# zhirui-gao/PoseProbe

Measured on AMD Instinct MI355X. Metric: rays_per_sec_train_step, higher is better.
Workload: dtype f32 (3xf16-split products); 1 GPU; DTU-scan1-like 3-view 400x400, object-branch train step (ray select, render, losses, backward, TV+Adam), 160^3 grid, 186 samples/ray, N_rand=1024/GPU; per-step ray permutation + jitter pre-generated on the host and resident in HBM (the reference draws randperm inside the step); grid=160, n_rand_per_gpu=1024, samples_in_bbox_last_step=57637, parallelism=single GPU

## Files before the change

include/poseprobe_hip.h:

```cpp
#ifndef POSEPROBE_HIP_H
#define POSEPROBE_HIP_H

#include <stdint.h>

#ifdef __cplusplus
extern "C" {
#endif

typedef enum {
  PP_OK = 0,
  PP_ERR_INVALID_ARG = -1,
  PP_ERR_LAUNCH = -2,
  PP_ERR_UNSUPPORTED = -3
} pp_status;

const char* pp_last_error(void);
#define PP_ABI_VERSION 4
int pp_abi_version(void);

typedef struct {
  float xyz_min[3];
  float xyz_max[3];
  int32_t size[3];
  float voxel_size;
// ... 49 lines not shown
                 const float* alphainv_last, const int32_t* ray_start, const int32_t* i_end, int32_t n_rays,
                 float bg, const float* rgb_pre, const float* g_rgb_marched, const float* g_cum_weights,
                 const float* g_alphainv_last, const float* g_depth_acc, const float* g_weights ,
                 float* grad_alpha, float* grad_rgb, void* stream);

int pp_geometry_fwd(const pp_scene* sc, const float* sdf_grid, const float* sdf_ab ,
                    const float* pts, const float* warp_out, const float* viewdirs, const int32_t* ray_id,
                    const int32_t* count, int32_t capacity, float inv_s, float* alpha, float* gradient,
                    float* sdf_final, float* sdf_deform, float* grad_deform, void* stream);
int pp_geometry_bwd(const pp_scene* sc, const float* sdf_grid, const float* sdf_ab, const float* pts,
                    const float* warp_out, const float* viewdirs, const int32_t* ray_id, const int32_t* count,
                    int32_t capacity, float inv_s, const float* g_alpha, const float* g_gradient,
                    const float* g_sdf_final, const float* g_sdf_deform, const float* g_grad_deform,
                    const float* g_correction, int32_t accumulate, float* warp_out_grad, float* pts_grad,
                    float* viewdir_grad_s, float* sdf_ab_grad, void* stream);

int pp_geometry_bwd_priors(const pp_scene* sc, const float* sdf_grid, const float* sdf_ab, const float* pts,
                           const float* warp_out, const float* viewdirs, const int32_t* ray_id, const int32_t* count,
                           int32_t capacity, float inv_s, const float* g_alpha, const float* g_gradient, float w_eikonal,
                           float w_deform, float loss_scale, int32_t accumulate, float* warp_out_grad, float* pts_grad,
                           float* viewdir_grad_s, float* sdf_ab_grad, float* loss_out, const float* batch_norm,
                           void* stream);

int pp_k0_pack_samples(const float* pts, const float* feat_grad, const int32_t* count, int32_t capacity, int32_t k0_dim,
                       float* packed, void* stream);
int pp_k0_scatter_packed(const pp_scene* sc, const float* packed, int32_t n_shards, int32_t capacity, float* k0_grad_cl,
                         uint8_t* touched , void* stream);
int pp_k0_scatter_samples(const pp_scene* sc, const float* pts, const int32_t* count, int32_t capacity,
                          const float* feat_grad, float* k0_grad_cl, uint8_t* touched , void* stream);

int pp_k0_scatter_sorted_workspace(int64_t n_samples, int64_t* bytes);
int pp_k0_scatter_samples_sorted(const pp_scene* sc, const float* pts, const int32_t* count, int32_t capacity,
                                 const float* feat_grad, float* k0_grad_cl, uint8_t* touched , void* work,
                                 int64_t work_bytes, void* stream);
int pp_k0_scatter_packed_sorted(const pp_scene* sc, const float* packed, int32_t n_shards, int32_t capacity, float* k0_grad_cl,
                                uint8_t* touched , void* work, int64_t work_bytes, void* stream);

int pp_color_feat_fwd(const pp_scene* sc, const float* k0_cl, const float* pts, const float* viewdirs,
                      const int32_t* ray_id, const float* gradient, const float* pe_w, const int32_t* count,
                      int32_t capacity, float* feat, void* stream);
int pp_color_feat_bwd(const pp_scene* sc, const float* k0_cl, const float* pts, const float* viewdirs,
                      const int32_t* ray_id, const float* gradient, const float* pe_w, const int32_t* count,
                      int32_t capacity, const float* feat_grad, float* k0_grad_cl, float* pts_grad,
                      float* gradient_grad, float* viewdir_grad_s, void* stream);

int pp_context_create(void** ctx);
int pp_context_destroy(void* ctx);
int pp_context_set_option(void* ctx, const char* name, int32_t value);
int pp_context_get_option(const void* ctx, const char* name, int32_t* value);

#define PP_RGBNET_PARAMS (128 * 64 + 128 + 2 * (128 * 128 + 128) + 3 * 128 + 3)
int pp_rgbnet_fwd(const float* params, const float* feat, const int32_t* count, int32_t capacity, float* acts,
                  float* rgb, void* ctx, void* stream);
int pp_rgbnet_bwd(const float* params, const float* feat, const float* acts, const float* rgb,
                  const float* rgb_grad, const int32_t* count, int32_t capacity, float* scratch ,
                  float* params_grad , float* feat_grad, void* ctx , void* stream);

#define PP_WARP_PARAMS (128 * 3 + 128 + 3 * (128 * 128 + 128) + 4 * 128 + 4)
int pp_warp_fwd(const float* params, const float* pts, const int32_t* count, int32_t capacity, float out_range,
                float* acts, float* out, void* ctx, void* stream);
int pp_warp_bwd(const float* params, const float* pts, const float* acts, const float* out_grad,
                const int32_t* count, int32_t capacity, float out_range, float* scratch ,
                float* params_grad , float* pts_grad , void* ctx ,
                void* stream);

int pp_rgbnet_workspace(int32_t capacity, int64_t* acts_floats, int64_t* scratch_floats);
int pp_warp_workspace(int32_t capacity, int64_t* acts_floats, int64_t* scratch_floats);
int pp_mlp_workspace(int32_t in_ld, int32_t n_gemm, int32_t capacity, int64_t* acts_floats, int64_t* scratch_floats);

int pp_warp_bwd_data(const float* params, const float* pts, const float* acts, const float* out_grad,
                     const int32_t* count, int32_t capacity, float out_range, float* scratch, float* params_grad,
                     float* pts_grad, int32_t* stage2_host, void* ctx, void* stream);
int pp_warp_bwd_weights(const float* acts, const float* scratch, const int32_t* count, int32_t capacity,
                        float* params_grad, int32_t stage2, void* ctx, void* stream);
int pp_rgbnet_bwd_data(const float* params, const float* acts, const float* rgb, const float* rgb_grad,
                       const int32_t* count, int32_t capacity, float* scratch, float* params_grad, float* feat_grad,
                       int32_t* stage2_host, void* ctx, void* stream);
int pp_rgbnet_bwd_weights(const float* feat, const float* acts, const float* scratch, const int32_t* count,
                          int32_t capacity, float* params_grad, int32_t stage2, void* ctx, void* stream);

int pp_mlp_pack_workspace(int64_t* pack_floats);
int pp_mlp_pack(const float* warp_params, const float* rgbnet_params, float* pack, void* ctx, void* stream);
int pp_mlp_pack_invalidate(void* ctx);

int pp_warp_lean_begin(const float* acts, const float* scratch, const float* params, void* ctx);
int pp_warp_lean_end(void* ctx);

int pp_ordered_workspace(int32_t work_groups, int32_t capacity, int32_t n_rays, int64_t* bytes);
int pp_ordered_attach(void* ctx, void* work, int64_t work_bytes, int32_t work_groups, int32_t capacity, int32_t n_rays);
int pp_geometry_color_feat_fwd(const pp_scene* sc, const float* sdf_grid, const float* sdf_ab, const float* pts,
                               const float* warp_out, const float* viewdirs, const int32_t* ray_id, const int32_t* count,
                               int32_t capacity, float inv_s, float* alpha, float* gradient, float* sdf_final,
                               float* sdf_deform, float* grad_deform, const float* k0_cl, const float* pe_w, float* feat,
                               void* stream);
int pp_geometry_bwd_priors_ordered(const pp_scene* sc, const float* sdf_grid, const float* sdf_ab, const float* pts,
                                   const float* warp_out, const float* viewdirs, const int32_t* ray_id, const int32_t* count,
                                   int32_t capacity, float inv_s, const float* g_alpha, const float* g_gradient, float w_eikonal,
                                   float w_deform, float loss_scale, int32_t accumulate, float* warp_out_grad, float* pts_grad,
                                   float* viewdir_grad_s, float* sdf_ab_grad, float* loss_out, const float* batch_norm,
                                   void* ctx, void* stream);
int pp_raygen_select_bwd_ordered(const pp_scene* sc, const int32_t* ray_idx, int32_t n_rays, const float* c2w,
                                 const float* intr, int32_t n_views, int32_t H, int32_t W, int32_t inverse_y,
                                 const float* rays_o, const float* rays_d, const float* t_min,
                                 const int32_t* ray_start, const float* pts_grad, const float* step,
                                 const float* viewdir_grad_s, const float* rays_o_grad, const float* rays_d_grad,
                                 const float* viewdirs_grad, const float* depth_grad, float* rays_o_grad_out,
                                 float* rays_d_grad_out, float* viewdirs_grad_out, float* c2w_grad, void* ctx, void* stream);

int pp_loss_rays(const float* rgb_marched, const float* alphainv_last, const float* cum_weights,
                 const float* target, const float* mask_px, float* mask_sum, int32_t n_rays, float w_main,
                 float w_entropy, float w_mask, float loss_scale, float* g_rgb_marched, float* g_alphainv_last,
                 float* g_cum_weights, float* loss_out, const float* batch_norm, void* stream);
int pp_loss_samples(const float* gradient, const float* grad_deform, const float* warp_out,
                    const float* sdf_deform, const int32_t* count, int32_t capacity, float w_eikonal,
                    float w_deform, float loss_scale, float* g_gradient, float* g_grad_deform,
                    float* g_correction, float* g_sdf_deform, float* loss_out, const float* batch_norm, void* stream);

int pp_grid_tv_adam_step(const float* p_in, float* p_out, float* grad, float* exp_avg, float* exp_avg_sq,
                         int32_t size_x, int32_t size_y, int32_t size_z, int32_t channels, int32_t x_begin,
                         int32_t x_end, float tv_scale, float grad_scale, float lr, float beta1, float beta2,
                         float eps, int32_t step, float* tv_out, void* ctx, void* stream);
int pp_grid_tv_adam_step_sparse(const float* p_in, float* p_out, float* grad, float* exp_avg, float* exp_avg_sq,
                                int32_t size_x, int32_t size_y, int32_t size_z, int32_t channels, int32_t x_begin,
                                int32_t x_end, float tv_scale, float grad_scale, float lr, float beta1, float beta2,
                                float eps, int32_t step, float* tv_out, const uint8_t* touched, uint8_t* touched_clear,
                                void* ctx, void* stream);
int pp_grid_tv_adam_step_tail(const float* p_in, float* p_out, float* grad, float* exp_avg, float* exp_avg_sq,
                              int32_t size_x, int32_t size_y, int32_t size_z, int32_t channels, int32_t x_begin,
                              int32_t x_end, float tv_scale, float grad_scale, float lr, float beta1, float beta2,
                              float eps, int32_t step, float* tv_out, const uint8_t* touched, uint8_t* touched_clear,
                              float* flat_p, float* flat_grad, float* flat_m, float* flat_v, int32_t flat_n,
                              const int32_t* flat_seg_end, const float* flat_seg_lr, int32_t flat_n_seg, float flat_beta1,
                              float flat_beta2, float flat_eps, float* se3, float* se3_grad, float* se3_m, float* se3_v,
                              int32_t n_views, const float* pose_lr, float pose_beta1, float pose_beta2, float pose_eps,
                              int32_t se3_update, const pp_scene* sc, const int32_t* ray_idx, int32_t n_rays,
                              const float* c2w, const float* intr, int32_t H, int32_t W, int32_t inverse_y,
                              const float* rays_o, const float* rays_d, const float* t_min, const int32_t* ray_start,
                              const float* pts_grad, const float* step_len, const float* viewdir_grad_s, const float* jac,
                              float* c2w_grad, int32_t* arrive, void* ctx, void* stream);
int pp_adam_flat(float* p, float* grad, float* exp_avg, float* exp_avg_sq, int32_t n, const int32_t* seg_end,
                 const float* seg_lr, int32_t n_seg, float grad_scale, float beta1, float beta2, float eps,
                 int32_t step, int32_t zero_grad, void* stream);
int pp_grid_tv_value(const float* p, int32_t size_x, int32_t size_y, int32_t size_z, int32_t channels, float* out,
                     void* stream);

int pp_grid_sample_fwd(const pp_scene* sc, const float* grid_cl, int32_t channels, const float* pts, int32_t n_pts,
                       int32_t border, float* out, void* stream);
int pp_grid_sample_bwd(const pp_scene* sc, const float* grid_cl, int32_t channels, const float* pts, int32_t n_pts,
                       int32_t border, const float* out_grad, float* grid_grad_cl, float* pts_grad, void* stream);
int pp_grid_tv_grad(const float* p, int32_t size_x, int32_t size_y, int32_t size_z, int32_t channels, float scale,
                    const float* g_scalar, float* grad, void* stream);

int pp_sdf_first_crossing(const float* sdf, const int32_t* ray_start, const int32_t* step_k, int32_t n_rays,
                          int32_t n_samples, float dist, const float* t_min, const float* rays_o,
                          const float* rays_d, float* sdf_dense, float* pts, uint8_t* mask, float* zval,
                          void* stream);

int pp_sdf_crossing_dense_bwd(const pp_scene* sc, const float* sdf_grid, const float* rays_o, const float* rays_d,
                              const float* t_min, const float* jitter, int32_t n_rays, int32_t n_samples, float dist,
                              const float* sdf_dense, const float* g_pts, const float* g_sdf_dense, float* g_rays_o,
                              float* g_rays_d, float* g_t_min, void* stream);

int pp_raw2alpha_fwd(const float* density, float shift, float interval, const float* interval_v, int32_t n,
                     float* exp_d, float* alpha, void* stream);
int pp_raw2alpha_bwd(const float* exp_d, const float* grad_back, float interval, const float* interval_v, int32_t n,
                     float* grad, void* stream);
int pp_maskcache_lookup(const uint8_t* world, const float* xyz, int32_t size_x, int32_t size_y, int32_t size_z,
                        float scale_x, float scale_y, float scale_z, float shift_x, float shift_y, float shift_z,
                        int32_t n, uint8_t* out, void* stream);
int pp_sample_ndc(const pp_scene* sc, const float* rays_o, const float* rays_d, int32_t n_rays, int32_t n_samples,
                  float* pts, uint8_t* mask_outbbox, void* stream);
int pp_sample_bg(const float* rays_o, const float* rays_d, const float* t_max, float bg_preserve, int32_t n_rays,
                 int32_t n_samples, float* pts, void* stream);
int pp_adam_upd(float* param, const float* grad, float* exp_avg, float* exp_avg_sq, const float* perlr, int32_t n,
                int32_t step, float beta1, float beta2, float lr, float eps, int32_t mode, void* stream);
int pp_adam_upd_multi(float* const* params_host, const float* const* grads_host, float* const* exp_avg_host,
                      float* const* exp_avg_sq_host, const int32_t* sizes_host, int32_t n_tensors, int32_t step, float beta1,
                      float beta2, float lr, float eps, void* stream);
int pp_tv_add_grad(const float* param_cl, float* grad_cl, const float* mask_cl, int32_t size_x, int32_t size_y,
                   int32_t size_z, int32_t channels, float wx, float wy, float wz, int32_t dense_mode, void* stream);
int pp_cumdist_thres(const float* dist, float thres, int32_t n_rays, int32_t n_pts, uint8_t* mask, void* stream);

int pp_feat_generic_fwd(const pp_scene* sc, const float* k0_cl, const float* pts, const float* viewdirs,
                        const int32_t* ray_id, const float* gradient, const float* pe_w, const uint8_t* sel,
                        int32_t k0_skip, int32_t ld, const int32_t* count, int32_t capacity, float* feat,
                        float* k0_raw, void* stream);
int pp_feat_generic_bwd_k0(const pp_scene* sc, const float* pts, const uint8_t* sel, int32_t k0_skip, int32_t ld,
                           const int32_t* count, int32_t capacity, const float* feat_grad,
                           const float* k0_raw_grad, float* k0_grad_cl, void* stream);
int pp_mlp_fwd(const float* params, const float* feat, int32_t in_ld, int32_t n_gemm, const int32_t* count,
               int32_t capacity, const float* logit_add, int32_t logit_add_ld, float* acts, float* out,
               void* ctx, void* stream);
int pp_mlp_bwd(const float* params, const float* feat, int32_t in_ld, int32_t n_gemm, const float* acts,
               const float* out, const float* out_grad, const int32_t* count, int32_t capacity, float* scratch,
               float* params_grad, float* feat_grad, float* logit_add_grad, int32_t logit_add_ld, void* ctx,
// ... 87 lines not shown
```

poseprobe_amd/csrc/pp_loss.hip:

```cpp
#include "pp_common.h"

__device__ __forceinline__ float block_sum256(float v, float* sm) {
  v = pp_wave_sum(v);
  int lane = threadIdx.x & 63, wid = threadIdx.x >> 6;
  __syncthreads();
  if (lane == 0) sm[wid] = v;
  __syncthreads();
  return sm[0] + sm[1] + sm[2] + sm[3];
}

__global__ __launch_bounds__(256) void k_loss_rays(const float* __restrict__ rgbm, const float* __restrict__ alast,
                                                   const float* __restrict__ cw, const float* __restrict__ target,
                                                   const float* __restrict__ mask_px, float* __restrict__ mask_sum,
                                                   int n_rays, float w_main, float w_ent, float w_mask, float ls,
                                                   float* __restrict__ g_rgbm, float* __restrict__ g_alast,
                                                   float* __restrict__ g_cw, float* __restrict__ loss_out,
                                                   const float* __restrict__ batch_norm) {
  __shared__ float sm[4];
  int r = blockIdx.x * blockDim.x + threadIdx.x;
  float l_mse = 0.f, l_ent = 0.f, l_bce = 0.f;
  float part = 0.f;
  for (int i = threadIdx.x; i < n_rays; i += 256) part += mask_px[i];
  const float msum_local = block_sum256(part, sm);
  if (blockIdx.x == 0 && threadIdx.x == 0) mask_sum[0] = msum_local;
  const float msum = batch_norm ? batch_norm[0] : msum_local;
  const float invN = 1.f / (float)n_rays;
  if (r < n_rays) {
    float y = mask_px[r];
    for (int k = 0; k < 3; ++k) {
      float d = rgbm[r * 3 + k] * y - target[r * 3 + k] * y;
      l_mse += d * d;
      g_rgbm[r * 3 + k] = ls * w_main * 2.f * d * y / (msum * 3.f);
    }
    float a = alast[r];
    float p = fminf(fmaxf(a, 1e-6f), 1.f - 1e-6f);
    float lp = logf(p), lq = logf(1.f - p);
    l_ent = -(p * lp + (1.f - p) * lq);
    g_alast[r] = (a >= 1e-6f && a <= 1.f - 1e-6f) ? ls * w_ent * (-(lp - lq)) * invN : 0.f;
    float c0 = cw[r];
    float c = fminf(fmaxf(c0, 1e-3f), 1.f - 1e-3f);
    l_bce = -(y * logf(c) + (1.f - y) * logf(1.f - c));
    g_cw[r] = (c0 >= 1e-3f && c0 <= 1.f - 1e-3f) ? ls * w_mask * (-(y / c) + (1.f - y) / (1.f - c)) * invN : 0.f;
  }
  l_mse = block_sum256(l_mse, sm);
  l_ent = block_sum256(l_ent, sm);
  l_bce = block_sum256(l_bce, sm);
  if (threadIdx.x == 0 && loss_out) {
    atomicAdd(&loss_out[0], l_mse / (msum * 3.f));
    atomicAdd(&loss_out[1], l_ent * invN);
    atomicAdd(&loss_out[6], l_bce * invN);
    atomicAdd(&loss_out[7], w_main * (l_mse / (msum * 3.f)) + w_ent * (l_ent * invN) + w_mask * (l_bce * invN));
  }
}

__global__ __launch_bounds__(256) void k_loss_samples(const float* __restrict__ gradient, const float* __restrict__ gdef,
                                                      const float* __restrict__ warp_out, const float* __restrict__ sdef,
                                                      const int32_t* __restrict__ count, int capacity, float w_eik,
                                                      float w_dyn, float ls, float* __restrict__ g_gradient,
                                                      float* __restrict__ g_gdef, float* __restrict__ g_corr,
                                                      float* __restrict__ g_sdef, float* __restrict__ loss_out,
                                                      const float* __restrict__ batch_norm) {
  __shared__ float sm[4];
  int m = blockIdx.x * blockDim.x + threadIdx.x;
  int M = min(count[0], capacity);
  float invM = M > 0 ? 1.f / (float)M : 0.f;
  if (batch_norm) invM = batch_norm[1] > 0.f ? 1.f / batch_norm[1] : 0.f;
  float l_eik = 0.f, l_gd = 0.f, l_c = 0.f, l_sd = 0.f;
  if (m < M) {
    float g[3] = {gradient[m * 3], gradient[m * 3 + 1], gradient[m * 3 + 2]};
    float gn = sqrtf(g[0] * g[0] + g[1] * g[1] + g[2] * g[2]);
    float e = gn - 1.f;
    l_eik = fabsf(e);
    float sg = (e > 0.f) ? 1.f : (e < 0.f ? -1.f : 0.f);
    for (int k = 0; k < 3; ++k) g_gradient[m * 3 + k] += (gn > 0.f) ? ls * w_eik * sg * g[k] / gn * invM : 0.f;
    for (int i = 0; i < 3; ++i) {
      float a0 = gdef[m * 9 + i * 3], a1 = gdef[m * 9 + i * 3 + 1], a2 = gdef[m * 9 + i * 3 + 2];
      float an = sqrtf(a0 * a0 + a1 * a1 + a2 * a2);
      l_gd += an;
      float s = (an > 0.f) ? ls * w_dyn * invM / (3.f * an) : 0.f;
      g_gdef[m * 9 + i * 3] = a0 * s; g_gdef[m * 9 + i * 3 + 1] = a1 * s; g_gdef[m * 9 + i * 3 + 2] = a2 * s;
    }
    float c = warp_out[(size_t)m * 16 + 3];
    l_c = fabsf(c);
    g_corr[m] = ls * w_dyn * invM * ((c > 0.f) ? 1.f : (c < 0.f ? -1.f : 0.f));
    float sd = sdef[m];
    l_sd = fabsf(sd);
    g_sdef[m] = ls * w_dyn * invM * ((sd > 0.f) ? 1.f : (sd < 0.f ? -1.f : 0.f));
  }
  l_eik = block_sum256(l_eik, sm);
  l_gd = block_sum256(l_gd, sm);
  l_c = block_sum256(l_c, sm);
  l_sd = block_sum256(l_sd, sm);
  if (threadIdx.x == 0 && loss_out && m - (int)threadIdx.x < M) {
    atomicAdd(&loss_out[2], l_eik * invM);
    atomicAdd(&loss_out[3], l_gd * invM / 3.f);
    atomicAdd(&loss_out[4], l_c * invM);
    atomicAdd(&loss_out[5], l_sd * invM);
    atomicAdd(&loss_out[7], w_eik * (l_eik * invM) + w_dyn * ((l_gd * invM / 3.f + l_c * invM) + l_sd * invM));
  }
}

extern "C" int pp_loss_rays(const float* rgb_marched, const float* alphainv_last, const float* cum_weights,
                            const float* target, const float* mask_px, float* mask_sum, int32_t n_rays, float w_main,
                            float w_entropy, float w_mask, float loss_scale, float* g_rgb_marched,
                            float* g_alphainv_last, float* g_cum_weights, float* loss_out, const float* batch_norm,
                            void* stream) {
  PP_REQUIRE(rgb_marched && alphainv_last && cum_weights && target && mask_px && mask_sum && g_rgb_marched &&
                 g_alphainv_last && g_cum_weights,
             "null pointer");
  PP_REQUIRE(n_rays > 0, "n_rays<=0");
  hipStream_t st = pp_stream(stream);
  hipLaunchKernelGGL(k_loss_rays, dim3(pp_div_up(n_rays, 256)), dim3(256), 0, st, rgb_marched, alphainv_last,
                     cum_weights, target, mask_px, mask_sum, n_rays, w_main, w_entropy, w_mask, loss_scale,
                     g_rgb_marched, g_alphainv_last, g_cum_weights, loss_out, batch_norm);
  PP_CHECK_LAUNCH();
  return PP_OK;
}

extern "C" int pp_loss_samples(const float* gradient, const float* grad_deform, const float* warp_out,
                               const float* sdf_deform, const int32_t* count, int32_t capacity, float w_eikonal,
                               float w_deform, float loss_scale, float* g_gradient, float* g_grad_deform,
                               float* g_correction, float* g_sdf_deform, float* loss_out, const float* batch_norm,
                               void* stream) {
  PP_REQUIRE(gradient && grad_deform && warp_out && sdf_deform && count && g_gradient && g_grad_deform &&
                 g_correction && g_sdf_deform,
             "null pointer");
  PP_REQUIRE(capacity > 0, "capacity<=0");
  hipLaunchKernelGGL(k_loss_samples, dim3(pp_div_up(capacity, 256)), dim3(256), 0, pp_stream(stream), gradient,
                     grad_deform, warp_out, sdf_deform, count, capacity, w_eikonal, w_deform, loss_scale, g_gradient,
                     g_grad_deform, g_correction, g_sdf_deform, loss_out, batch_norm);
  PP_CHECK_LAUNCH();
  return PP_OK;
}
```

poseprobe_amd/csrc/pp_march.hip:

```cpp
#include "pp_common.h"

__device__ __forceinline__ float lane_value(float v, int j) {
  return __int_as_float(__builtin_amdgcn_readlane(__float_as_int(v), j));
}
__device__ __forceinline__ double lane_value(double v, int j) {
  return __hiloint2double(__builtin_amdgcn_readlane(__double2hiint(v), j), __builtin_amdgcn_readlane(__double2loint(v), j));
}

template <bool FUSED, bool DVGO>
__global__ __launch_bounds__(256) void k_march_fwd(const float* __restrict__ alpha, const float* __restrict__ rgb,
                                                   const float* __restrict__ step_w, const float* __restrict__ nrm_in,
                                                   const int32_t* __restrict__ ray_start, int n_rays, float bg,
                                                   float* __restrict__ weights, float* __restrict__ Tout,
                                                   float* __restrict__ alphainv_last, int32_t* __restrict__ i_end,
                                                   float* __restrict__ rgb_marched, float* __restrict__ rgb_pre,
                                                   float* __restrict__ cum_weights, float* __restrict__ depth_acc,
                                                   float* __restrict__ normal_marched) {
  const int r = blockIdx.x * 4 + __builtin_amdgcn_readfirstlane(threadIdx.x >> 6);
  int lane = threadIdx.x & 63;
  if (r >= n_rays) return;
  const int b = ray_start[r], e = ray_start[r + 1];
  float Tc = 1.f;
  int stop = e;
  bool stopped = false;
  float acc_rgb[3] = {0, 0, 0}, acc_w = 0.f, acc_d = 0.f, acc_n[3] = {0, 0, 0};
  float a_next = (b + lane < e) ? alpha[b + lane] : 0.f;
  for (int c0 = b; c0 < e; c0 += 64) {
    int i = c0 + lane;
    const float a = a_next;
    a_next = (i + 64 < e) ? alpha[i + 64] : 0.f;
    float cr[3] = {0.f, 0.f, 0.f}, cs = 0.f, cn[3] = {0.f, 0.f, 0.f};
    if (FUSED && i < e) {
      if (rgb) for (int k = 0; k < 3; ++k) cr[k] = rgb[i * 3 + k];
      if (step_w) cs = step_w[i];
      if (nrm_in) for (int k = 0; k < 3; ++k) cn[k] = nrm_in[i * 3 + k];
    }
    float myT = 1.f, myw = 0.f;
    if (!stopped) {
      int n = e - c0 < 64 ? e - c0 : 64;
      const double omd = 1.0 - (double)a;
      const float omf = fmaxf(1.f - a, 1e-10f);
      bool reached = false;
      for (int j = 0; j < n; ++j) {
        if (lane == j) { myT = Tc; reached = true; }
        if (DVGO) {
          Tc = Tc * lane_value(omf, j);
        } else {
          Tc = (float)((double)Tc * lane_value(omd, j));
          if (Tc < 1e-3f) { stop = c0 + j + 1; stopped = true; break; }
        }
      }
      if (reached) myw = myT * a;
    }
    if (i < e) {
      weights[i] = myw;
      if (Tout) Tout[i] = myT;
      if (FUSED) {
        acc_w += myw;
        if (rgb) for (int k = 0; k < 3; ++k) acc_rgb[k] += myw * cr[k];
        if (step_w) acc_d += myw * cs;
        if (nrm_in) for (int k = 0; k < 3; ++k) acc_n[k] += myw * cn[k];
      }
    }
  }
  if (FUSED) {
    acc_w = pp_wave_sum(acc_w);
    acc_d = pp_wave_sum(acc_d);
    for (int k = 0; k < 3; ++k) { acc_rgb[k] = pp_wave_sum(acc_rgb[k]); acc_n[k] = pp_wave_sum(acc_n[k]); }
  }
  if (lane == 0) {
    alphainv_last[r] = Tc;
    i_end[r] = stop;
    if (FUSED) {
      cum_weights[r] = acc_w;
      if (depth_acc) depth_acc[r] = acc_d;
      for (int k = 0; k < 3; ++k) {
        float pre = acc_rgb[k] + (1.f - acc_w) * bg;
        if (rgb_pre) rgb_pre[r * 3 + k] = pre;
        if (rgb_marched) rgb_marched[r * 3 + k] = fminf(fmaxf(pre, 0.f), 1.f);
        if (normal_marched) normal_marched[r * 3 + k] = acc_n[k];
      }
    }
  }
}

template <bool FUSED>
__global__ __launch_bounds__(256) void k_march_bwd(const float* __restrict__ alpha, const float* __restrict__ rgb,
                                                   const float* __restrict__ step_w, const float* __restrict__ weights,
                                                   const float* __restrict__ Tin, const float* __restrict__ alphainv_last,
                                                   const int32_t* __restrict__ ray_start, const int32_t* __restrict__ i_end,
                                                   int n_rays, float bg, const float* __restrict__ rgb_pre,
                                                   const float* __restrict__ g_rgbm, const float* __restrict__ g_cw,
                                                   const float* __restrict__ g_last, const float* __restrict__ g_depth,
                                                   const float* __restrict__ g_w_in, float* __restrict__ g_alpha,
                                                   float* __restrict__ g_rgb) {
  const int r = blockIdx.x * 4 + __builtin_amdgcn_readfirstlane(threadIdx.x >> 6);
  int lane = threadIdx.x & 63;
  if (r >= n_rays) return;
  const int b = ray_start[r], e = ray_start[r + 1], stop = i_end[r];
  float gm[3] = {0, 0, 0}, gcw = 0.f, gd = 0.f;
  if (FUSED) {
    for (int k = 0; k < 3; ++k) {
      float pre = rgb_pre ? rgb_pre[r * 3 + k] : 0.5f;
      float g = g_rgbm ? g_rgbm[r * 3 + k] : 0.f;
      gm[k] = (pre >= 0.f && pre <= 1.f) ? g : 0.f;
    }
    gcw = (g_cw ? g_cw[r] : 0.f) - bg * (gm[0] + gm[1] + gm[2]);
    gd = g_depth ? g_depth[r] : 0.f;
  }
  float back = (g_last ? g_last[r] : 0.f) * alphainv_last[r];
  int nchunk = (e - b + 63) / 64;
  struct Chunk { float a, w, T, gw, v[3], sw; };
  auto fetch = [&](int c) {
    Chunk k;
    const int i = b + c * 64 + lane;
    const bool live = i < e;
    k.a = live ? alpha[i] : 0.f;
    k.w = live ? weights[i] : 0.f;
    k.T = live ? Tin[i] : 1.f;
    k.gw = (live && g_w_in) ? g_w_in[i] : 0.f;
    k.v[0] = k.v[1] = k.v[2] = 0.f; k.sw = 0.f;
    if (FUSED && live) {
      if (rgb) for (int q = 0; q < 3; ++q) k.v[q] = rgb[i * 3 + q];
      if (step_w) k.sw = step_w[i];
    }
    return k;
  };
  Chunk nx = fetch(nchunk > 0 ? nchunk - 1 : 0);
  for (int c = nchunk - 1; c >= 0; --c) {
    int c0 = b + c * 64;
    int i = c0 + lane;
    bool live = i < e;
    const Chunk ck = nx;
    if (c > 0) nx = fetch(c - 1);
    const float a = ck.a, w = ck.w, T = ck.T;
    float gw = ck.gw;
    if (FUSED && live) {
      float wr = 0.f;
      if (rgb) for (int k = 0; k < 3; ++k) { wr += gm[k] * ck.v[k]; if (g_rgb) g_rgb[i * 3 + k] = w * gm[k]; }
      gw += wr + gcw + (step_w ? gd * ck.sw : 0.f);
    }
    int hi = stop - c0;
    if (hi > 64) hi = 64;
    const float gww = gw * w;
    float myback = 0.f;
    for (int j = hi - 1; j >= 0; --j) {
      if (lane == j) myback = back;
      back += lane_value(gww, j);
    }
    float ga = 0.f;
    if (lane < hi) {
      const float gwT = gw * T;
      const double denom = (double)(1.f - a) + 1e-10;
      ga = (float)((double)gwT - (double)myback / denom);
    }
    if (live) g_alpha[i] = ga;
  }
}

extern "C" int pp_alpha2weight_fwd(const float* alpha, const int32_t* ray_start, int32_t n_rays, float* weights,
                                   float* T, float* alphainv_last, int32_t* i_end, void* stream) {
  PP_REQUIRE(alpha && ray_start && weights && T && alphainv_last && i_end, "null pointer");
  PP_REQUIRE(n_rays > 0, "n_rays<=0");
  hipLaunchKernelGGL((k_march_fwd<false, false>), dim3(pp_div_up(n_rays, 4)), dim3(256), 0, pp_stream(stream), alpha, nullptr,
                     nullptr, nullptr, ray_start, n_rays, 0.f, weights, T, alphainv_last, i_end, nullptr, nullptr,
                     nullptr, nullptr, nullptr);
  PP_CHECK_LAUNCH();
  return PP_OK;
}

extern "C" int pp_alpha2weight_bwd(const float* alpha, const float* weights, const float* T, const float* alphainv_last,
                                   const int32_t* ray_start, const int32_t* i_end, int32_t n_rays,
                                   const float* grad_weights, const float* grad_last, float* grad_alpha, void* stream) {
  PP_REQUIRE(alpha && weights && T && alphainv_last && ray_start && i_end && grad_weights && grad_last && grad_alpha,
             "null pointer");
  PP_REQUIRE(n_rays > 0, "n_rays<=0");
  hipLaunchKernelGGL((k_march_bwd<false>), dim3(pp_div_up(n_rays, 4)), dim3(256), 0, pp_stream(stream), alpha, nullptr,
                     nullptr, weights, T, alphainv_last, ray_start, i_end, n_rays, 0.f, nullptr, nullptr, nullptr,
                     grad_last, nullptr, grad_weights, grad_alpha, nullptr);
  PP_CHECK_LAUNCH();
  return PP_OK;
}

extern "C" int pp_march_fwd(const float* alpha, const float* rgb, const float* step_w, const float* nrm_in,
                            const int32_t* ray_start, int32_t n_rays, float bg, float* weights, float* T,
                            float* alphainv_last, int32_t* i_end, float* rgb_marched, float* rgb_pre,
                            float* cum_weights, float* depth_acc, float* normal_marched, void* stream) {
  PP_REQUIRE(alpha && rgb && ray_start && weights && T && alphainv_last && i_end && cum_weights, "null pointer");
  PP_REQUIRE(n_rays > 0, "n_rays<=0");
  hipLaunchKernelGGL((k_march_fwd<true, false>), dim3(pp_div_up(n_rays, 4)), dim3(256), 0, pp_stream(stream), alpha, rgb,
                     step_w, nrm_in, ray_start, n_rays, bg, weights, T, alphainv_last, i_end, rgb_marched, rgb_pre,
                     cum_weights, depth_acc, normal_marched);
  PP_CHECK_LAUNCH();
  return PP_OK;
}

extern "C" int pp_march_bwd(const float* alpha, const float* rgb, const float* step_w, const float* weights,
                            const float* T, const float* alphainv_last, const int32_t* ray_start,
                            const int32_t* i_end, int32_t n_rays, float bg, const float* rgb_pre,
                            const float* g_rgb_marched, const float* g_cum_weights, const float* g_alphainv_last,
                            const float* g_depth_acc, const float* g_weights, float* grad_alpha, float* grad_rgb,
                            void* stream) {
  PP_REQUIRE(alpha && rgb && weights && T && alphainv_last && ray_start && i_end && grad_alpha, "null pointer");
  PP_REQUIRE(n_rays > 0, "n_rays<=0");
  hipLaunchKernelGGL((k_march_bwd<true>), dim3(pp_div_up(n_rays, 4)), dim3(256), 0, pp_stream(stream), alpha, rgb,
                     step_w, weights, T, alphainv_last, ray_start, i_end, n_rays, bg, rgb_pre, g_rgb_marched,
                     g_cum_weights, g_alphainv_last, g_depth_acc, g_weights, grad_alpha, grad_rgb);
  PP_CHECK_LAUNCH();
  return PP_OK;
}

#define PP_MAX_S 1024
__global__ __launch_bounds__(256) void k_first_crossing(const float* __restrict__ sdf, const int32_t* __restrict__ ray_start,
                                                        const int32_t* __restrict__ step_k, int n_rays, int S, float dist,
                                                        const float* __restrict__ t_min, const float* __restrict__ rays_o,
                                                        const float* __restrict__ rays_d, float* __restrict__ sdf_dense,
                                                        float* __restrict__ pts, uint8_t* __restrict__ mask,
                                                        float* __restrict__ zval) {
  __shared__ float rows[4][PP_MAX_S];
  int wid = threadIdx.x >> 6, lane = threadIdx.x & 63;
  int r = blockIdx.x * 4 + wid;
  if (r >= n_rays) return;
  float* row = rows[wid];
  if (ray_start) {
    for (int k = lane; k < S; k += 64) row[k] = 1.f;
    __builtin_amdgcn_wave_barrier();
    for (int i = ray_start[r] + lane; i < ray_start[r + 1]; i += 64) row[step_k[i]] = sdf[i];
  } else {
    for (int k = lane; k < S; k += 64) row[k] = sdf[(size_t)r * S + k];
  }
  __builtin_amdgcn_wave_barrier();
  if (sdf_dense) for (int k = lane; k < S; k += 64) sdf_dense[(size_t)r * S + k] = row[k];
  int prev = 0;
  for (int k0 = 0; k0 < S - 1; k0 += 64) {
    int k = k0 + lane;
    bool hit = (k < S - 1) && (row[k] * row[k + 1] <= 0.f);
    unsigned long long bal = __ballot(hit);
    if (bal) { prev = k0 + __ffsll((long long)bal) - 1; break; }
  }
  if (lane == 0) {
    float s1 = row[prev], s2 = row[prev + 1];
    float z1 = (float)prev * dist + dist * 0.5f, z2 = (float)(prev + 1) * dist + dist * 0.5f;
    float z0 = (s1 * z2 - s2 * z1) / (s1 - s2 + 1e-10f);
    if (z0 < z1) z0 = 0.f;
    if (z0 > z2) z0 = 0.f;
    bool ok = (z0 > 1e-10f) && (s1 * s2 < 0.f);
    float dx = rays_d[r * 3], dy = rays_d[r * 3 + 1], dz = rays_d[r * 3 + 2];
    float nrm = sqrtf(fmaf(dz, dz, fmaf(dy, dy, dx * dx)));
    float interpx = t_min[r] + z0 / nrm;
    pts[r * 3] = rays_o[r * 3] + dx * interpx;
    pts[r * 3 + 1] = rays_o[r * 3 + 1] + dy * interpx;
    pts[r * 3 + 2] = rays_o[r * 3 + 2] + dz * interpx;
    mask[r] = ok ? 1 : 0;
    if (zval) zval[r] = z0;
  }
}

extern "C" int pp_sdf_first_crossing(const float* sdf, const int32_t* ray_start, const int32_t* step_k, int32_t n_rays,
                                     int32_t n_samples, float dist, const float* t_min, const float* rays_o,
                                     const float* rays_d, float* sdf_dense, float* pts, uint8_t* mask, float* zval,
                                     void* stream) {
  PP_REQUIRE(sdf && t_min && rays_o && rays_d && pts && mask, "null pointer");
  PP_REQUIRE((ray_start == nullptr) == (step_k == nullptr), "ray_start and step_k go together");
  PP_REQUIRE(n_rays > 0 && n_samples >= 2 && n_samples <= PP_MAX_S, "need n_rays>0 and 2<=n_samples<=1024");
  hipLaunchKernelGGL(k_first_crossing, dim3(pp_div_up(n_rays, 4)), dim3(256), 0, pp_stream(stream), sdf, ray_start, step_k,
                     n_rays, n_samples, dist, t_min, rays_o, rays_d, sdf_dense, pts, mask, zval);
  PP_CHECK_LAUNCH();
  return PP_OK;
}

extern "C" int pp_march_dvgo_fwd(const float* alpha, const float* rgb, const float* step_w, const int32_t* ray_start,
                                 int32_t n_rays, float* weights, float* T, float* alphainv_last, int32_t* i_end,
                                 float* rgb_acc, float* cum_weights, float* depth_acc, void* stream) {
  PP_REQUIRE(alpha && ray_start && weights && T && alphainv_last && i_end && cum_weights, "null pointer");
  PP_REQUIRE(n_rays > 0, "n_rays<=0");
  hipLaunchKernelGGL((k_march_fwd<true, true>), dim3(pp_div_up(n_rays, 4)), dim3(256), 0, pp_stream(stream), alpha, rgb,
                     step_w, nullptr, ray_start, n_rays, 0.f, weights, T, alphainv_last, i_end, nullptr, rgb_acc,
                     cum_weights, depth_acc, nullptr);
  PP_CHECK_LAUNCH();
  return PP_OK;
}
```

poseprobe_amd/csrc/pp_mlp.hip:

```cpp
#include "pp_common.h"
#include "pp_mlp_fused.h"
#include "pp_mlp_pack.h"
#include "pp_ordered.h"
#include <stdlib.h>

struct MlpRoute {
  const PPContext* c;
  bool fused;
  int split;
  bool pack;
  int wgs;
  explicit MlpRoute(const void* ctx) : c(static_cast<const PPContext*>(ctx)) {
    const int* o = pp_options(ctx);
    fused = o[PP_OPT_MLP_FUSED] == 1; split = o[PP_OPT_MLP_SPLIT]; pack = o[PP_OPT_MLP_PACK] == 1;
    wgs = o[PP_OPT_MLP_WGS] > 0 ? (o[PP_OPT_MLP_WGS] < 16 ? 16 : o[PP_OPT_MLP_WGS]) : pp_num_cus();
  }
  bool runs_split(int bits) const { return fused && (split & bits) == bits; }
};

static const float* mlp_pack_for(const MlpRoute& rt, const float* params, int net) {
  if (!rt.c || !rt.pack || !rt.c->pack || rt.c->pack_params[net] != params) return nullptr;
  return rt.c->pack;
}

static const float* warp_lean_for(const MlpRoute& rt, const float* acts, const float* scratch) {
  const PPContext* c = rt.c;
  if (!c || !c->lean_acts || c->lean_acts != acts || (scratch && c->lean_scratch != scratch) || !rt.runs_split(1 | 2 | 16)) return nullptr;
  return c->lean_params;
}

extern "C" int pp_warp_lean_end(void* ctx) {
  PP_REQUIRE(ctx, "null context");
  PPContext* c = static_cast<PPContext*>(ctx);
  c->lean_acts = c->lean_scratch = c->lean_params = nullptr;
  return PP_OK;
}

extern "C" int pp_warp_lean_begin(const float* acts, const float* scratch, const float* params, void* ctx) {
  PP_REQUIRE(ctx, "null context (the scope is recorded in a context: create one)");
  PP_REQUIRE(acts && scratch && params, "null pointer");
  pp_warp_lean_end(ctx);
  if (pp_options(ctx)[PP_OPT_WARP_LEAN] != 1 || !MlpRoute(ctx).runs_split(1 | 2 | 16)) return PP_OK;
  PPContext* c = static_cast<PPContext*>(ctx);
  c->lean_acts = acts;
  c->lean_scratch = scratch;
  c->lean_params = params;
  return PP_OK;
}

static const char* ordered_refusal(const MlpRoute& rt, int capacity, int bits, bool fused_shape = true) {
  const PPContext* c = rt.c;
  if (!c || !c->ord) return nullptr;
  if (!fused_shape || !rt.runs_split(bits))
    return "an ordered-flush workspace is attached to the context: only the split-precision layer-fused kernels have ordered "
           "flushes (options mlp_fused = 1, mlp_split bits 2, 8 and 16; the Voxurf network shapes)";
  if (capacity > c->ord_cap || rt.wgs > c->ord_wgs)
    return "the attached ordered-flush workspace is too small for this capacity / work-group count";
  return nullptr;
}
#define PP_REQUIRE_ORDERED(rt, capacity, ...)                                   \
  do {                                                                          \
    const char* why__ = ordered_refusal(rt, capacity, __VA_ARGS__);             \
    PP_REQUIRE(why__ == nullptr, why__);                                        \
  } while (0)
static float* ordered_part(const MlpRoute& rt, int region) {
  const PPContext* c = rt.c;
  if (!c || !c->ord) return nullptr;
  const OrdLayout L = pp_ord_layout(c->ord_wgs, c->ord_cap, c->ord_rays);
  return c->ord + (region < 2 ? L.wgrad[region] : L.thin[region - 2]);
}

extern "C" int pp_mlp_pack_workspace(int64_t* pack_floats) {
  PP_REQUIRE(pack_floats, "null pointer");
  *pack_floats = PK_FLOATS;
  return PP_OK;
}

extern "C" int pp_mlp_pack_invalidate(void* ctx) {
  PP_REQUIRE(ctx, "null context");
  PPContext* c = static_cast<PPContext*>(ctx);
  c->pack = nullptr;
  c->pack_params[0] = c->pack_params[1] = nullptr;
  return PP_OK;
}

extern "C" int pp_mlp_pack(const float* warp_params, const float* rgbnet_params, float* pack, void* ctx, void* stream) {
  PP_REQUIRE(ctx, "null context (the pack is recorded in a context: create one)");
  PP_REQUIRE(pack && (warp_params || rgbnet_params), "null pointer");
  PP_REQUIRE((reinterpret_cast<uintptr_t>(pack) & 15) == 0, "pack must be 16-byte aligned");
  pp_mlp_pack_invalidate(ctx);
  const MlpRoute rt(ctx);
  if (!rt.pack || !rt.fused || (rt.split & 15) == 0) return PP_OK;
  pp_launch_mlp_pack(warp_params, rgbnet_params, pack, pp_stream(stream));
  PP_CHECK_LAUNCH();
  PPContext* c = static_cast<PPContext*>(ctx);
  c->pack = pack;
  c->pack_params[0] = warp_params;
  c->pack_params[1] = rgbnet_params;
  return PP_OK;
}

extern "C" int pp_mlp_fwd(const float* params, const float* feat, int32_t in_ld, int32_t n_gemm, const int32_t* count,
                          int32_t capacity, const float* logit_add, int32_t logit_add_ld, float* acts, float* out,
                          void* ctx, void* stream) {
  const MlpRoute rt(ctx);
  PP_REQUIRE(params && feat && count && out, "null pointer");
  PP_REQUIRE(capacity > 0 && in_ld % 32 == 0 && in_ld <= 128 && n_gemm >= 1 && n_gemm <= 8, "bad sizes");
  PP_REQUIRE(acts || (in_ld == 64 && n_gemm == 3 && rt.runs_split(4)),
             "acts may be NULL only for the rgbnet shape with the split-precision forward kernel (option mlp_split bit 4)");
  hipStream_t st = pp_stream(stream);
  if (in_ld == 64 && n_gemm == 3 && rt.fused) {
    if (rt.runs_split(4)) pp_launch_rgb_fused_fwd_s(params, feat, count, capacity, logit_add, logit_add_ld, acts, out, st, rt.wgs, mlp_pack_for(rt, params, 1));
    else pp_launch_rgb_fused_fwd(params, feat, count, capacity, logit_add, logit_add_ld, acts, out, st, rt.wgs);
  } else
    pp_launch_mlp_layered_fwd(params, feat, in_ld, n_gemm, count, capacity, logit_add, logit_add_ld, acts, out, st);
  PP_CHECK_LAUNCH();
  return PP_OK;
}

static bool warp_bwd_stage1(const MlpRoute& rt, const float* params, const float* pts, const float* acts, const float* out_grad,
                            const int32_t* count, int capacity, float out_range, float* scratch, float* params_grad, float* pts_grad,
                            hipStream_t st) {
  const bool sb = rt.runs_split(2);
  if (sb) pp_launch_warp_fused_bwd_s(params, pts, acts, out_grad, count, capacity, out_range, scratch, params_grad, pts_grad, st, rt.wgs,
                                     mlp_pack_for(rt, params, 0), ordered_part(rt, 2), warp_lean_for(rt, acts, scratch) != nullptr);
  else pp_launch_warp_fused_bwd(params, pts, acts, out_grad, count, capacity, out_range, scratch, params_grad, pts_grad, st, rt.wgs);
  return sb;
}
static void warp_bwd_stage2(const MlpRoute& rt, const float* acts, const float* scratch, const int32_t* count, int capacity,
                            float* params_grad, bool sb, hipStream_t st) {
  const int rcap = capacity * 4;
  const size_t LS = (size_t)rcap * 128;
  float *pg = params_grad, *b3 = sb ? pg + WPF_B3 : nullptr, *b2 = sb ? pg + WPF_B2 : nullptr, *b1 = sb ? pg + WPF_B1 : nullptr;
  const float* lp = warp_lean_for(rt, acts, scratch);
  const WgradLean lean{acts + 3 * LS, lp ? lp + WPF_W4 : nullptr, lp ? lp + WPF_W0 : nullptr};
  if (rt.runs_split(16))
    pp_launch_wgrad_chain_s(scratch, acts + 2 * LS, pg + WPF_W3, scratch + LS, acts + LS, pg + WPF_W2, scratch + 2 * LS, acts, pg + WPF_W1,
                            128, count, 4, rcap, st, rt.wgs, b3, b2, b1, ordered_part(rt, 0), lp ? &lean : nullptr);
  else
    pp_launch_wgrad_chain(scratch, acts + 2 * LS, pg + WPF_W3, scratch + LS, acts + LS, pg + WPF_W2, scratch + 2 * LS, acts, pg + WPF_W1,
                          128, count, 4, rcap, st, rt.wgs, b3, b2, b1);
}
static bool rgb_bwd_stage1(const MlpRoute& rt, const float* params, const float* acts, const float* rgb, const float* rgb_grad,
                           const int32_t* count, int capacity, float* scratch, float* params_grad, float* feat_grad, float* logit_grad,
                           int lg_ld, hipStream_t st) {
  const bool sb = rt.runs_split(8);
  if (sb) pp_launch_rgb_fused_bwd_s(params, acts, rgb, rgb_grad, count, capacity, scratch, params_grad, feat_grad, logit_grad, lg_ld,
                                    st, rt.wgs, mlp_pack_for(rt, params, 1), ordered_part(rt, 3));
  else pp_launch_rgb_fused_bwd(params, acts, rgb, rgb_grad, count, capacity, scratch, params_grad, feat_grad, logit_grad, lg_ld, st, rt.wgs);
  return sb;
}
static void rgb_bwd_stage2(const MlpRoute& rt, const float* feat, const float* acts, const float* scratch, const int32_t* count,
                           int capacity, float* params_grad, bool sb, hipStream_t st) {
  const size_t FLS = (size_t)capacity * 128;
  float *pg = params_grad, *b2 = sb ? pg + RGF_B2 : nullptr, *b1 = sb ? pg + RGF_B1 : nullptr, *b0 = sb ? pg + RGF_B0 : nullptr;
  if (rt.runs_split(16))
    pp_launch_wgrad_chain_s(scratch, acts + FLS, pg + RGF_W2, scratch + FLS, acts, pg + RGF_W1, scratch + 2 * FLS, feat, pg + RGF_W0,
                            64, count, 1, capacity, st, rt.wgs, b2, b1, b0, ordered_part(rt, 1), nullptr);
  else
    pp_launch_wgrad_chain(scratch, acts + FLS, pg + RGF_W2, scratch + FLS, acts, pg + RGF_W1, scratch + 2 * FLS, feat, pg + RGF_W0,
                          64, count, 1, capacity, st, rt.wgs, b2, b1, b0);
}

extern "C" int pp_mlp_bwd(const float* params, const float* feat, int32_t in_ld, int32_t n_gemm, const float* acts,
                          const float* out, const float* out_grad, const int32_t* count, int32_t capacity,
                          float* scratch, float* params_grad, float* feat_grad, float* logit_add_grad,
                          int32_t logit_add_ld, void* ctx, void* stream) {
  const MlpRoute rt(ctx);
  PP_REQUIRE(params && feat && acts && out && out_grad && count && scratch && params_grad, "null pointer");
  PP_REQUIRE(capacity > 0 && in_ld % 32 == 0 && in_ld <= 128 && n_gemm >= 1 && n_gemm <= 8, "bad sizes");
  PP_REQUIRE_ORDERED(rt, capacity, 8 | 16, in_ld == 64 && n_gemm == 3 && feat_grad != nullptr);
  hipStream_t st = pp_stream(stream);
  if (in_ld == 64 && n_gemm == 3 && feat_grad && rt.fused) {
    const bool sb = rgb_bwd_stage1(rt, params, acts, out, out_grad, count, capacity, scratch, params_grad, feat_grad, logit_add_grad,
                                   logit_add_ld, st);
    rgb_bwd_stage2(rt, feat, acts, scratch, count, capacity, params_grad, sb, st);
  } else
    pp_launch_mlp_layered_bwd(params, feat, in_ld, n_gemm, acts, out, out_grad, count, capacity, scratch, params_grad, feat_grad,
                              logit_add_grad, logit_add_ld, st);
  PP_CHECK_LAUNCH();
  return PP_OK;
}

extern "C" int pp_rgbnet_fwd(const float* params, const float* feat, const int32_t* count, int32_t capacity,
// ... 120 lines not shown
```

poseprobe_amd/csrc/pp_mlp_fused.h:

```cpp
#pragma once
#include <hip/hip_runtime.h>
#include <stdint.h>

#define WPF_W0 0
#define WPF_B0 (128 * 3)
#define WPF_W1 (WPF_B0 + 128)
#define WPF_B1 (WPF_W1 + 128 * 128)
#define WPF_W2 (WPF_B1 + 128)
#define WPF_B2 (WPF_W2 + 128 * 128)
#define WPF_W3 (WPF_B2 + 128)
#define WPF_B3 (WPF_W3 + 128 * 128)
#define WPF_W4 (WPF_B3 + 128)
#define WPF_B4 (WPF_W4 + 4 * 128)

static inline int pp_fused_grid(int units, int wgs) { return units < wgs ? units : wgs; }

int pp_launch_warp_fused_fwd(const float* params, const float* pts, const int32_t* count, int capacity, float out_range,
                             float* acts, float* out, hipStream_t st, int wgs);
int pp_launch_warp_fused_bwd(const float* params, const float* pts, const float* acts, const float* out_grad,
                             const int32_t* count, int capacity, float out_range, float* ybar, float* params_grad,
                             float* pts_grad, hipStream_t st, int wgs);
struct WgradOperands {
  const float* Y;
  const float* X;
  float* Wbar;
  float* bbar;
};
struct WgradLean {
  const float* gate3;
  const float* w4;
  const float* w0;
};
int pp_launch_wgrad_chain_s(const float* YA, const float* XA, float* WA, const float* YB, const float* XB, float* WB,
                            const float* YC, const float* XC, float* WC, int kxc, const int32_t* count, int rmul, int rcap,
                            hipStream_t st, int wgs, float* bA, float* bB, float* bC, float* part, const WgradLean* lean);
int pp_launch_warp_fused_fwd_s(const float* params, const float* pts, const int32_t* count, int capacity, float out_range,
                               float* acts, float* out, hipStream_t st, int wgs, const float* pack, bool lean);
int pp_launch_warp_fused_bwd_s(const float* params, const float* pts, const float* acts, const float* out_grad,
                               const int32_t* count, int capacity, float out_range, float* ybar, float* params_grad,
                               float* pts_grad, hipStream_t st, int wgs, const float* pack, float* part, bool lean);
int pp_launch_mlp_pack(const float* warp_params, const float* rgbnet_params, float* pack, hipStream_t st);
int pp_launch_wgrad_chain(const float* YA, const float* XA, float* WA, const float* YB, const float* XB, float* WB,
                          const float* YC, const float* XC, float* WC, int kxc, const int32_t* count, int rmul, int rcap,
                          hipStream_t st, int wgs, float* bA, float* bB, float* bC);

#define RGF_W0 0
#define RGF_B0 (128 * 64)
#define RGF_W1 (RGF_B0 + 128)
#define RGF_B1 (RGF_W1 + 128 * 128)
#define RGF_W2 (RGF_B1 + 128)
#define RGF_B2 (RGF_W2 + 128 * 128)
#define RGF_W3 (RGF_B2 + 128)
#define RGF_B3 (RGF_W3 + 3 * 128)

int pp_launch_rgb_fused_fwd(const float* params, const float* feat, const int32_t* count, int capacity,
                            const float* logit_add, int add_ld, float* acts, float* rgb, hipStream_t st, int wgs);
int pp_launch_rgb_fused_fwd_s(const float* params, const float* feat, const int32_t* count, int capacity,
                              const float* logit_add, int add_ld, float* acts, float* rgb, hipStream_t st, int wgs, const float* pack);
int pp_launch_rgb_fused_bwd_s(const float* params, const float* acts, const float* rgb, const float* rgb_grad,
                              const int32_t* count, int capacity, float* ybar, float* params_grad, float* feat_grad,
                              float* logit_grad, int lg_ld, hipStream_t st, int wgs, const float* pack, float* part);
int pp_launch_rgb_fused_bwd(const float* params, const float* acts, const float* rgb, const float* rgb_grad,
                            const int32_t* count, int capacity, float* ybar, float* params_grad, float* feat_grad,
                            float* logit_grad, int lg_ld, hipStream_t st, int wgs);

void pp_launch_mlp_layered_fwd(const float* params, const float* feat, int in_ld, int n_gemm, const int32_t* count, int capacity,
                               const float* logit_add, int logit_add_ld, float* acts, float* out, hipStream_t st);
void pp_launch_mlp_layered_bwd(const float* params, const float* feat, int in_ld, int n_gemm, const float* acts, const float* out,
                               const float* out_grad, const int32_t* count, int capacity, float* scratch, float* params_grad,
                               float* feat_grad, float* logit_add_grad, int logit_add_ld, hipStream_t st);
void pp_launch_warp_layered_fwd(const float* params, const float* pts, const int32_t* count, int capacity, float out_range,
                                float* acts, float* out, hipStream_t st);
void pp_launch_warp_layered_bwd(const float* params, const float* pts, const float* acts, const float* out_grad, const int32_t* count,
                                int capacity, float out_range, float* scratch, float* params_grad, float* pts_grad, hipStream_t st);
```

poseprobe_amd/csrc/pp_mlp_split.hip:

```cpp
#include "pp_common.h"
#include "pp_mlp_fused.h"
#include "pp_gemm_split.h"
#include "pp_split_image.h"
#include "pp_mlp_pack.h"
#include "pp_ordered.h"

typedef float f32x4 __attribute__((ext_vector_type(4)));

#define LDA 132
#define TILE_ROWS 64
#define LDH2 136
#define PLANE (TILE_ROWS * LDH2)
#define PP_WAIT_VMEM() do { __builtin_amdgcn_s_waitcnt(0x0F70); asm volatile("" ::: "memory"); } while (0)

namespace {

struct SplitW { pp_half8 h[8], l[8]; };

__device__ __forceinline__ float wave_max(float v) {
#pragma unroll
  for (int o = 32; o > 0; o >>= 1) v = fmaxf(v, __shfl_xor(v, o, 64));
  return v;
}
template <int CTRL>
__device__ __forceinline__ float dpp_f(float v) {
  return __int_as_float(__builtin_amdgcn_update_dpp(0, __float_as_int(v), CTRL, 0xf, 0xf, true));
}
__device__ __forceinline__ float row_max16(float v) {
  v = fmaxf(v, dpp_f<0xB1>(v));
  v = fmaxf(v, dpp_f<0x4E>(v));
  v = fmaxf(v, dpp_f<0x141>(v));
  v = fmaxf(v, dpp_f<0x140>(v));
  return v;
}
__device__ __forceinline__ float block_max(float v, float* red, int tid, int& phase) {
  float* set = red + 16 * (phase & 1);
  ++phase;
  v = row_max16(v);
  if ((tid & 15) == 0) set[tid >> 4] = v;
  __syncthreads();
  const float4 a = *reinterpret_cast<const float4*>(set), b = *reinterpret_cast<const float4*>(set + 4),
               c = *reinterpret_cast<const float4*>(set + 8), d = *reinterpret_cast<const float4*>(set + 12);
  return fmaxf(fmaxf(fmaxf(fmaxf(a.x, a.y), fmaxf(a.z, a.w)), fmaxf(fmaxf(b.x, b.y), fmaxf(b.z, b.w))),
               fmaxf(fmaxf(fmaxf(c.x, c.y), fmaxf(c.z, c.w)), fmaxf(fmaxf(d.x, d.y), fmaxf(d.z, d.w))));
}
__device__ __forceinline__ int scale_exp(float mx) {
  if (!(mx > 0.f) || !(mx < 3.0e38f)) return 0;
  int e;
  frexpf(mx, &e);
  return min(max(15 - e, -60), 60);
}
__device__ __forceinline__ float pow2(int e) { return ldexpf(1.f, e); }
__device__ __forceinline__ float tile_scale(float mx) { return pow2(scale_exp(mx)); }
__device__ __forceinline__ void split1(float x, _Float16& h, _Float16& l) {
  h = (_Float16)x;
  l = (_Float16)(x - (float)h);
}
__device__ __forceinline__ void split8(const float4& a, const float4& b, float s, pp_half8& h, pp_half8& l) {
  const float v[8] = {a.x * s, a.y * s, a.z * s, a.w * s, b.x * s, b.y * s, b.z * s, b.w * s};
#pragma unroll
  for (int i = 0; i < 8; ++i) {
    _Float16 hh, ll;
    split1(v[i], hh, ll);
    h[i] = hh; l[i] = ll;
  }
}
__device__ __forceinline__ float amax4(const float4& v) { return fmaxf(fmaxf(fabsf(v.x), fabsf(v.y)), fmaxf(fabsf(v.z), fabsf(v.w))); }
__device__ __forceinline__ float asum4(const float4& v) { return (fabsf(v.x) + fabsf(v.y)) + (fabsf(v.z) + fabsf(v.w)); }

__device__ __forceinline__ int load_w_rows_split(SplitW& w, float& l1, const float* __restrict__ W, int n, int lh, float* red,
                                                   int tid, int& phase) {
  float4 v[16];
  float mx = 0.f, sum = 0.f;
#pragma unroll
  for (int ks = 0; ks < 8; ++ks) {
    v[2 * ks] = *reinterpret_cast<const float4*>(W + (size_t)n * 128 + 16 * ks + 8 * lh);
    v[2 * ks + 1] = *reinterpret_cast<const float4*>(W + (size_t)n * 128 + 16 * ks + 8 * lh + 4);
    mx = fmaxf(mx, fmaxf(amax4(v[2 * ks]), amax4(v[2 * ks + 1])));
    sum += asum4(v[2 * ks]) + asum4(v[2 * ks + 1]);
  }
  sum += __shfl_xor(sum, 32, 64);
  const int e = scale_exp(block_max(mx, red, tid, phase));
  const float s = pow2(e);
  l1 = block_max(sum, red, tid, phase) * 1.0001f;
#pragma unroll
  for (int ks = 0; ks < 8; ++ks) split8(v[2 * ks], v[2 * ks + 1], s, w.h[ks], w.l[ks]);
  return e;
// ... 1095 lines not shown
    mma_half(Aa, w2, acc0, l31, lh);
    PP_WAIT_VMEM();
    __syncthreads();
    const int e10 = scale_exp(slot_get(&Mx[par][0]) * l1_2), e11 = scale_exp(slot_get(&Mx[par][1]) * l1_2);
    zero16(acc1);
    eb.begin(&GT[l31 * 128 + fb]);
    mma_half(Aa + 32 * LDH2, w2, acc1, l31, lh, [&](int ks) {
      eb.step(ks, acc0, pow2(-(e2 + ew2)), pow2(e10), ok0, crow + LS, Ab + l31 * LDH2 + fb);
    });
    slot_max(&Mx[par][2], eb.vmax(pow2(-e10)), lane);
    __syncthreads();
    zero16(acc0);
    eb.begin(&GT[(32 + l31) * 128 + fb]);
    mma_half(Ab, w1, acc0, l31, lh, [&](int ks) {
      eb.step(ks, acc1, pow2(-(e2 + ew2)), pow2(e11), ok1, crow + LS + 32 * 128, Ab + (32 + l31) * LDH2 + fb);
    });
    slot_max(&Mx[par][3], eb.vmax(pow2(-e11)), lane);
    __syncthreads();
    stage_tile(H0, r0, GT);
    zero16(acc1);
    mma_half(Ab + 32 * LDH2, w1, acc1, l31, lh);
    PP_WAIT_VMEM();
    __syncthreads();
    const int e00 = scale_exp(slot_get(&Mx[par][2]) * l1_1), e01 = scale_exp(slot_get(&Mx[par][3]) * l1_1);
    eb.begin(&GT[l31 * 128 + fb]);
    eb.all(acc0, pow2(-(e10 + ew1)), pow2(e00), ok0, crow + 2 * LS, Aa + l31 * LDH2 + fb);
    eb.begin(&GT[(32 + l31) * 128 + fb]);
    eb.all(acc1, pow2(-(e11 + ew1)), pow2(e01), ok1, crow + 2 * LS + 32 * 128, Aa + (32 + l31) * LDH2 + fb);
    if (more) logit_grads(tnext, par ^ 1);
    __syncthreads();
    {
      f32x16 fa;
      zero16(fa);
      mma_half(Aa + rb * 32 * LDH2, w0, fa, l31, lh);
      const float inv = pow2(-((rb ? e01 : e00) + ew0));
      const int row = r0 + rb * 32 + l31;
      if (row < R) {
        float* __restrict__ ft = feat_grad + (size_t)row * 64 + (wid & 1) * 32 + 4 * lh;
#pragma unroll
        for (int q = 0; q < 4; ++q)
          *reinterpret_cast<float4*>(ft + 8 * q) = make_float4(fa[4 * q] * inv, fa[4 * q + 1] * inv, fa[4 * q + 2] * inv, fa[4 * q + 3] * inv);
      }
    }
    if (more) {
      w3_accumulate();
      out_layer_bwd(tnext, par ^ 1, Ab);
    }
    __syncthreads();
  }

  float* red = reinterpret_cast<float*>(At[0]);
  __syncthreads();
  if (h0 == 1) {
#pragma unroll
    for (int o = 0; o < 3; ++o) red[o * 128 + j0] = wacc3[o];
    if (j0 < 3) red[4 * 128 + j0] = bacc3;
  }
  __syncthreads();
  if (h0 == 0 && part != nullptr) {
    float* __restrict__ row = part + (size_t)blockIdx.x * ORD_RGB_THIN;
#pragma unroll
    for (int o = 0; o < 3; ++o) row[o * 128 + j0] = wacc3[o] + red[o * 128 + j0];
    if (j0 < 3) row[384 + j0] = bacc3 + red[4 * 128 + j0];
  } else if (h0 == 0) {
#pragma unroll
    for (int o = 0; o < 3; ++o) atomicAdd(&params_grad[RGF_W3 + o * 128 + j0], wacc3[o] + red[o * 128 + j0]);
    if (j0 < 3) atomicAdd(&params_grad[RGF_B3 + j0], bacc3 + red[4 * 128 + j0]);
  }
}

int pp_launch_rgb_fused_bwd_s(const float* params, const float* acts, const float* rgb, const float* rgb_grad,
                              const int32_t* count, int capacity, float* ybar, float* params_grad, float* feat_grad,
                              float* logit_grad, int lg_ld, hipStream_t st, int wgs, const float* pack, float* part) {
  const int grid = pp_fused_grid(pp_div_up(capacity, TILE_ROWS), wgs);
  launch_pack_variant(k_rgb_fused_bwd_s<true>, k_rgb_fused_bwd_s<false>, grid, st, pack, params, acts, rgb, rgb_grad, count, capacity, ybar,
                      params_grad, feat_grad, logit_grad, lg_ld, part);
  if (part) {
    const OrdSegs segs{2, {384, ORD_RGB_THIN_N, 0, 0}, {RGF_W3, RGF_B3, 0, 0}};
    pp_launch_ordered_flush(part, ORD_RGB_THIN, grid, count, capacity, TILE_ROWS, segs, params_grad, st);
  }
  return 0;
}

__global__ __launch_bounds__(256) void k_mlp_pack(const float* __restrict__ warp, const float* __restrict__ rgb, float* __restrict__ pack) {
  __shared__ __attribute__((aligned(16))) float red4[32];
  const int task = blockIdx.x;
  const float* __restrict__ params = task < PK_TASKS_WARP ? warp : rgb;
  if (params == nullptr) return;
  const int tid = threadIdx.x, lane = tid & 63, wid = tid >> 6;
  const int l31 = lane & 31, lh = lane >> 5;
  const int col = wid * 32 + l31;
  int phase = 0;
  SplitW w;
  float l1 = 0.f;
  float* __restrict__ S = pack + PK_SCAL;
  auto put = [&](int se, int e, int sl, float v) {
    if (tid == 0) { S[se] = __int_as_float(e); if (sl >= 0) S[sl] = v; }
  };
  if (task < 3) {
    const int off = task == 0 ? WPF_W1 : (task == 1 ? WPF_W2 : WPF_W3);
    const int e = load_w_rows_split(w, l1, params + off, col, lh, red4, tid, phase);
    store_w_packed<8>(pack + PK_WARP + task * PK_IMG, w, tid);
    put(PKW_EW1 + 2 * task, e, PKW_L1_1 + 2 * task, l1);
  } else if (task < 6) {
    const int t = task - 3;
    const int off = t == 0 ? WPF_W3 : (t == 1 ? WPF_W2 : WPF_W1);
    const int e = load_w_cols_split(w, l1, params + off, col, lh, red4, tid, phase);
    store_w_packed<8>(pack + PK_WARP + task * PK_IMG, w, tid);
    put(PKW_EW3C + 2 * t, e, PKW_L1_3C + 2 * t, l1);
  } else if (task == 6) {
    const float b1mx = block_max(fabsf(params[WPF_B1 + col]), red4, tid, phase), b2mx = block_max(fabsf(params[WPF_B2 + col]), red4, tid, phase);
    const float w0x = params[WPF_W0 + col * 3], w0y = params[WPF_W0 + col * 3 + 1], w0z = params[WPF_W0 + col * 3 + 2];
    const float b0 = params[WPF_B0 + col];
    const float w0l1 = block_max((fabsf(w0x) + fabsf(w0y)) + fabsf(w0z), red4, tid, phase) * 1.0001f;
    const float w0mx = block_max(fmaxf(fmaxf(fabsf(w0x), fabsf(w0y)), fabsf(w0z)), red4, tid, phase);
    const float b0mx = block_max(fabsf(b0), red4, tid, phase);
    if (tid == 0) { S[PKW_B1MX] = b1mx; S[PKW_B2MX] = b2mx; S[PKW_W0L1] = w0l1; S[PKW_W0MX] = w0mx; S[PKW_B0MX] = b0mx; }
    put(PKW_EW0, scale_exp(fmaxf(w0mx, b0mx)), -1, 0.f);
  } else if (task == 7) {
    const int e = load_w0_rows_split(w, l1, params + RGF_W0, col, lh, red4, tid, phase);
    store_w_packed<4>(pack + PK_RGB, w, tid);
    put(PKR_EW0, e, PKR_L1_0, l1);
  } else if (task < 10) {
    const int t = task - 8;
    const int e = load_w_rows_split(w, l1, params + (t == 0 ? RGF_W1 : RGF_W2), col, lh, red4, tid, phase);
    store_w_packed<8>(pack + PK_RGB_W1 + t * PK_IMG, w, tid);
    put(PKR_EW1 + 2 * t, e, PKR_L1_1 + 2 * t, l1);
  } else if (task < 12) {
    const int t = task - 10;
    const int e = load_w_cols_split(w, l1, params + (t == 0 ? RGF_W2 : RGF_W1), col, lh, red4, tid, phase);
    store_w_packed<8>(pack + PK_RGB_W1 + (2 + t) * PK_IMG, w, tid);
    put(PKR_EW2C + 2 * t, e, PKR_L1_2C + 2 * t, l1);
  } else if (task == 12) {
    const int e = load_w0_cols_split(w, params + RGF_W0, (wid & 1) * 32 + l31, lh, red4, tid, phase);
    store_w_packed<8>(pack + PK_RGB_W1 + 4 * PK_IMG, w, tid);
    put(PKR_EW0T, e, -1, 0.f);
  } else {
    const float b0mx = block_max(fabsf(params[RGF_B0 + col]), red4, tid, phase), b1mx = block_max(fabsf(params[RGF_B1 + col]), red4, tid, phase);
    const float w3a = params[RGF_W3 + col], w3b = params[RGF_W3 + 128 + col], w3c = params[RGF_W3 + 256 + col];
    const float w3l1 = block_max((fabsf(w3a) + fabsf(w3b)) + fabsf(w3c), red4, tid, phase) * 1.0001f;
    const int ew3 = scale_exp(block_max(fmaxf(fmaxf(fabsf(w3a), fabsf(w3b)), fabsf(w3c)), red4, tid, phase));
    if (tid == 0) { S[PKR_B0MX] = b0mx; S[PKR_B1MX] = b1mx; }
    put(PKR_EW3, ew3, PKR_W3L1, w3l1);
  }
}

int pp_launch_mlp_pack(const float* warp_params, const float* rgbnet_params, float* pack, hipStream_t st) {
  hipLaunchKernelGGL(k_mlp_pack, dim3(PK_TASKS), dim3(256), 0, st, warp_params, rgbnet_params, pack);
  return 0;
}

namespace {

struct WgsUnit { int r0, rend; };

__device__ __forceinline__ WgsUnit wgs_unit(int k, int full, int wg, int nwg, int ntiles, int R, int rem_rows, int q) {
  if (k < full) {
    const int t = ntiles - 1 - wg - k * nwg;
    return {t * TILE_ROWS, R};
  }
  const int hi = rem_rows - wg * q;
  return {max(hi - q, 0), hi};
}

__device__ __forceinline__ void wgs_active(int ntiles, int& nwg_ab, int& nwg_c) {
  if (ntiles < 8 * nwg_ab) {
    nwg_ab = max(nwg_ab / 2, 1);
    nwg_c = max(nwg_c / 2, 1);
  }
}

template <int KX, int CSTEP, bool LEAN>
__device__ __forceinline__ void wgs_layer(const WgradOperands& L, const float* __restrict__ gate3, const float* __restrict__ wls,
                                          int layer, int R, int ntiles, int wg, int nwg, unsigned char* __restrict__ img,
                                          float2* __restrict__ flags, float* __restrict__ slot) {
  static_assert(!LEAN || KX == 128, "the lean form is the warp net's");
  constexpr int NB = KX / 64;
  constexpr int XR = KX / 16;
  constexpr int XC = KX / 4;
  const int full = ntiles / nwg;
  const int rem_rows = min((ntiles - full * nwg) * TILE_ROWS, R);
  const int q = ((rem_rows + nwg - 1) / nwg + 15) & ~15;
  const int nunits = full + (rem_rows - wg * q > 0 ? 1 : 0);
  if (nunits == 0) {
    if (slot != nullptr)
      for (int i = threadIdx.x; i < ORD_WGRAD_SLOT / 4; i += 256) reinterpret_cast<float4*>(slot)[i] = make_float4(0.f, 0.f, 0.f, 0.f);
    return;
  }
  unsigned char* const Yh = img;
  unsigned char* const Yl = img + TILE_ROWS * 256;
  unsigned char* const Xh = img + 2 * TILE_ROWS * 256;
  unsigned char* const Xl = img + 3 * TILE_ROWS * 256;
  const int tid = threadIdx.x, lane = tid & 63, wid = tid >> 6;
  const int wr = wid >> 1, wc = wid & 1, l31 = lane & 31, lh = lane >> 5;
  const int c4 = tid & 31, rblk = tid >> 5;
  const int xc4 = c4 % XC, xrow = 8 * rblk + (c4 / XC) * XR;
  const bool bias = L.bbar != nullptr;
  const bool lean_y = LEAN && layer == 0, lean_x = LEAN && layer == 2;
  float4 rg[2];
  f32x16 acc[2][NB];
#pragma unroll
  for (int t = 0; t < 2; ++t)
#pragma unroll
    for (int u = 0; u < NB; ++u) zero16(acc[t][u]);
  float bsum[4] = {0.f, 0.f, 0.f, 0.f};
  int eY = 60, eX = 60;
  float sY = pow2(eY), sX = pow2(eX), limY = pow2(15 - eY), limX = pow2(15 - eX);

  float4 ry[8], rx[XR];
  auto load_rows = [&](int r0, int i0, int i1) {
#pragma unroll
    for (int i = 0; i < 8; ++i) {
      if (i < i0 || i >= i1) continue;
      if (lean_y) {
        const size_t row = (size_t)min(r0 + 8 * rblk + i, R - 1);
        ry[i] = *reinterpret_cast<const float4*>(L.Y + row * 4);
        if ((i & 3) == 0) rg[i >> 2] = *reinterpret_cast<const float4*>(gate3 + row * 128 + c4 * 4);
      } else {
        ry[i] = *reinterpret_cast<const float4*>(L.Y + (size_t)min(r0 + 8 * rblk + i, R - 1) * 128 + c4 * 4);
      }
      if (i < XR && !(lean_x && (i & 3) != 0))
        rx[i] = *reinterpret_cast<const float4*>(L.X + (size_t)min(r0 + xrow + i, R - 1) * KX + xc4 * 4);
    }
  };
  auto rebuild = [&]() {
    if (lean_y) {
      const float4 w0 = *reinterpret_cast<const float4*>(wls + c4 * 4), w1 = *reinterpret_cast<const float4*>(wls + 128 + c4 * 4),
                   w2 = *reinterpret_cast<const float4*>(wls + 256 + c4 * 4), w3 = *reinterpret_cast<const float4*>(wls + 384 + c4 * 4);
#pragma unroll
// ... 258 lines not shown
```

poseprobe_amd/csrc/pp_rays.hip:

```cpp
#include "pp_common.h"
#include "pp_ordered.h"
#include "pp_ray_bwd.h"

struct D6 {
  float v;
  float d;
};
__device__ __forceinline__ D6 d6c(float c) { D6 r; r.v = c; r.d = 0.f; return r; }
__device__ __forceinline__ D6 operator+(const D6& a, const D6& b) { D6 r; r.v = a.v + b.v; r.d = a.d + b.d; return r; }
__device__ __forceinline__ D6 operator-(const D6& a, const D6& b) { D6 r; r.v = a.v - b.v; r.d = a.d - b.d; return r; }
__device__ __forceinline__ D6 operator-(const D6& a) { D6 r; r.v = -a.v; r.d = -a.d; return r; }
__device__ __forceinline__ D6 operator*(const D6& a, const D6& b) { D6 r; r.v = a.v * b.v; r.d = a.d * b.v + a.v * b.d; return r; }
__device__ __forceinline__ D6 operator*(const D6& a, float s) { D6 r; r.v = a.v * s; r.d = a.d * s; return r; }

__device__ D6 taylor_t(const D6& t, int kind) {
  D6 ans = d6c(0.f);
  D6 pw = d6c(1.f);
  double denom = 1.0;
  for (int i = 0; i <= 10; ++i) {
    if (kind == 0) { if (i > 0) denom *= (double)((2 * i) * (2 * i + 1)); }
    else if (kind == 1) denom *= (double)((2 * i + 1) * (2 * i + 2));
    else denom *= (double)((2 * i + 2) * (2 * i + 3));
    float c = (float)(((i & 1) ? -1.0 : 1.0) / denom);
    ans = ans + pw * c;
    pw = pw * t;
  }
  return ans;
}

__global__ void k_pose_fwd(const float* __restrict__ se3, const float* __restrict__ w2c_init,
                           const int32_t* __restrict__ refine_mask, int n_views, float* __restrict__ w2c,
                           float* __restrict__ c2w, float* __restrict__ jac) {
  int tidx = blockIdx.x * blockDim.x + threadIdx.x;
  int v = tidx / 6, kd = tidx - (tidx / 6) * 6;
  if (v >= n_views) return;
  const float* P0 = w2c_init + v * 12;
  D6 Rn[3][3], tn[3];
  bool refine = (refine_mask == nullptr) || refine_mask[v] != 0;
  if (!refine) {
    for (int i = 0; i < 3; ++i) { for (int j = 0; j < 3; ++j) Rn[i][j] = d6c(P0[i * 4 + j]); tn[i] = d6c(P0[i * 4 + 3]); }
  } else {
    D6 w[3], u[3];
    for (int k = 0; k < 3; ++k) {
      w[k] = d6c(se3[v * 6 + k]); w[k].d = (kd == k) ? 1.f : 0.f;
      u[k] = d6c(se3[v * 6 + 3 + k]); u[k].d = (kd == 3 + k) ? 1.f : 0.f;
    }
    D6 t = w[0] * w[0] + w[1] * w[1] + w[2] * w[2];
    D6 A = taylor_t(t, 0), B = taylor_t(t, 1), C = taylor_t(t, 2);
    D6 z = d6c(0.f);
    D6 wx[3][3] = {{z, -w[2], w[1]}, {w[2], z, -w[0]}, {-w[1], w[0], z}};
    D6 wx2[3][3];
    for (int i = 0; i < 3; ++i) for (int j = 0; j < 3; ++j) wx2[i][j] = wx[i][0] * wx[0][j] + wx[i][1] * wx[1][j] + wx[i][2] * wx[2][j];
    D6 R[3][3], Vm[3][3], tr[3];
    for (int i = 0; i < 3; ++i) for (int j = 0; j < 3; ++j) {
      D6 eye = d6c(i == j ? 1.f : 0.f);
      R[i][j] = eye + A * wx[i][j] + B * wx2[i][j];
      Vm[i][j] = eye + B * wx[i][j] + C * wx2[i][j];
    }
    for (int i = 0; i < 3; ++i) tr[i] = Vm[i][0] * u[0] + Vm[i][1] * u[1] + Vm[i][2] * u[2];
    for (int i = 0; i < 3; ++i) {
      for (int j = 0; j < 3; ++j) Rn[i][j] = R[0][j] * P0[i * 4 + 0] + R[1][j] * P0[i * 4 + 1] + R[2][j] * P0[i * 4 + 2];
      tn[i] = tr[0] * P0[i * 4 + 0] + tr[1] * P0[i * 4 + 1] + tr[2] * P0[i * 4 + 2] + d6c(P0[i * 4 + 3]);
    }
  }
  for (int i = 0; i < 3; ++i) {
    for (int j = 0; j < 3; ++j) {
      if (kd == 0) { w2c[v * 12 + i * 4 + j] = Rn[i][j].v; c2w[v * 12 + i * 4 + j] = Rn[j][i].v; }
      jac[(v * 12 + i * 4 + j) * 6 + kd] = Rn[j][i].d;
    }
    D6 ti = -(Rn[0][i] * tn[0] + Rn[1][i] * tn[1] + Rn[2][i] * tn[2]);
    if (kd == 0) { w2c[v * 12 + i * 4 + 3] = tn[i].v; c2w[v * 12 + i * 4 + 3] = ti.v; }
    jac[(v * 12 + i * 4 + 3) * 6 + kd] = ti.d;
  }
}

__global__ void k_pose_bwd(const float* __restrict__ jac, const float* __restrict__ c2w_grad, int n_views,
                           float* __restrict__ se3_grad) {
  int t = blockIdx.x * blockDim.x + threadIdx.x;
  if (t >= n_views * 6) return;
  se3_grad[t] = pose_bwd_elem<false>(jac, c2w_grad, t);
}

extern "C" int pp_pose_fwd(const float* se3, const float* w2c_init, const int32_t* refine_mask, int32_t n_views,
                           float* w2c, float* c2w, float* jac, void* stream) {
  PP_REQUIRE(se3 && w2c_init && w2c && c2w && jac && n_views > 0, "null pointer or n_views<=0");
  hipLaunchKernelGGL(k_pose_fwd, dim3(pp_div_up(n_views * 6, 64)), dim3(64), 0, pp_stream(stream), se3, w2c_init,
                     refine_mask, n_views, w2c, c2w, jac);
  PP_CHECK_LAUNCH();
  return PP_OK;
}
extern "C" int pp_pose_bwd(const float* jac, const float* c2w_grad, int32_t n_views, float* se3_grad, void* stream) {
  PP_REQUIRE(jac && c2w_grad && se3_grad && n_views > 0, "null pointer or n_views<=0");
  hipLaunchKernelGGL(k_pose_bwd, dim3(pp_div_up(n_views * 6, 64)), dim3(64), 0, pp_stream(stream), jac, c2w_grad,
                     n_views, se3_grad);
  PP_CHECK_LAUNCH();
  return PP_OK;
}


__global__ void k_raygen_fwd(const int32_t* __restrict__ ray_idx, int n_rays, const float* __restrict__ c2w,
                             const float* __restrict__ intr, int H, int W, int inverse_y, int normalize,
                             const float* __restrict__ images, const float* __restrict__ masks,
                             float* __restrict__ rays_o, float* __restrict__ rays_d, float* __restrict__ viewdirs,
                             float* __restrict__ target, float* __restrict__ mask_px) {
  int r = blockIdx.x * blockDim.x + threadIdx.x;
  if (r >= n_rays) return;
  int idx = ray_idx[r], view;
  float dirs[3];
  pixel_dir(idx, H, W, intr, inverse_y, view, dirs);
  const float* P = c2w + view * 12;
  float d[3];
  for (int k = 0; k < 3; ++k)
    d[k] = pp_add(pp_add(pp_mul(dirs[0], P[k * 4 + 0]), pp_mul(dirs[1], P[k * 4 + 1])), pp_mul(dirs[2], P[k * 4 + 2]));
  float nrm = pp_norm3(d[0], d[1], d[2]);
  for (int k = 0; k < 3; ++k) {
    float vd = pp_div(d[k], nrm);
    rays_o[r * 3 + k] = P[k * 4 + 3];
    rays_d[r * 3 + k] = normalize ? vd : d[k];
    viewdirs[r * 3 + k] = vd;
  }
  if (target) for (int k = 0; k < 3; ++k) target[r * 3 + k] = images[(size_t)idx * 3 + k];
  if (mask_px) mask_px[r] = masks[idx];
}

extern "C" int pp_raygen_select_fwd(const pp_scene* sc, const int32_t* ray_idx, int32_t n_rays, const float* c2w,
                                    const float* intr, int32_t n_views, int32_t H, int32_t W, int32_t inverse_y,
                                    int32_t normalize, const float* images, const float* masks, float* rays_o,
                                    float* rays_d, float* viewdirs, float* target, float* mask_px, void* stream) {
  (void)sc; (void)n_views;
  PP_REQUIRE(ray_idx && c2w && intr && rays_o && rays_d && viewdirs && n_rays > 0, "null pointer or n_rays<=0");
  PP_REQUIRE((!target || images) && (!mask_px || masks), "target/mask requested without images/masks");
  hipLaunchKernelGGL(k_raygen_fwd, dim3(pp_div_up(n_rays, 256)), dim3(256), 0, pp_stream(stream), ray_idx, n_rays,
                     c2w, intr, H, W, inverse_y, normalize, images, masks, rays_o, rays_d, viewdirs, target, mask_px);
  PP_CHECK_LAUNCH();
  return PP_OK;
}

struct RaySlab {
  float o[3], d[3], t_min, t_max, nrm;
  bool miss;
};

__device__ __forceinline__ RaySlab ray_slab(const SceneDev& sc, const float* __restrict__ rays_o,
                                            const float* __restrict__ rays_d, int r) {
  RaySlab s;
  float lo = -INFINITY, hi = INFINITY;
  for (int k = 0; k < 3; ++k) {
    s.o[k] = rays_o[r * 3 + k];
    s.d[k] = rays_d[r * 3 + k];
    float vec = (s.d[k] == 0.f) ? 1e-6f : s.d[k];
    float a = pp_div(pp_sub(sc.mx[k], s.o[k]), vec);
    float b = pp_div(pp_sub(sc.mn[k], s.o[k]), vec);
    lo = fmaxf(lo, fminf(a, b));
    hi = fminf(hi, fmaxf(a, b));
  }
  s.t_min = fminf(fmaxf(lo, sc.near_), sc.far_);
// ... 339 lines not shown
```

poseprobe_amd/engine.py:

```python
import contextlib
import math
from dataclasses import dataclass

import numpy as np
import torch

from . import ops

PAD = 64


def _pad(n):
    return (n + PAD - 1) // PAD * PAD


@dataclass
class SceneConfig:
    xyz_min: np.ndarray
    xyz_max: np.ndarray
    num_voxels: int
    stepsize: float = 1.5
    near: float = 0.24
    far: float = 4.8
    bg: float = 0.0
    N_iters: int = 10000
    s_ratio: float = 50.0
    s_start: float = 0.2
    step_start: float = 0.0
    barf_c2f: tuple = (0.6, 1.0)
    posbase_pe: int = 5
    viewbase_pe: int = 1
    k0_dim: int = 12
    out_range: float = 1.0
    inverse_y: bool = True
    sdf_index_exact: bool = False

    def __post_init__(self):
        lo = torch.tensor(np.asarray(self.xyz_min, dtype=np.float32))
        hi = torch.tensor(np.asarray(self.xyz_max, dtype=np.float32))
        vs = ((hi - lo).prod() / self.num_voxels).pow(1 / 3)
        self.voxel_size = float(vs)
        self.world_size = [int(v) for v in ((hi - lo) / vs).long().tolist()]
        self.pp = ops.make_scene(lo.tolist(), hi.tolist(), self.world_size, self.voxel_size, self.stepsize, self.near,
                                 self.far, self.bg, self.out_range, self.k0_dim, self.posbase_pe, self.viewbase_pe,
                                 sdf_index_exact=True if self.sdf_index_exact else None)
        self.n_samples = self.pp.n_samples

    def s_val(self, global_step):
        return 1. / (global_step + self.s_ratio / self.s_start - self.step_start) * self.s_ratio

    def inv_s(self, global_step):
        return float(np.float32(1.0) / np.float32(self.s_val(global_step)))

    @property
    def step_dist(self):
        return float(np.float32(self.stepsize) * np.float32(self.voxel_size))

    def pe_weights(self, progress):
        out = []
        for L in (self.posbase_pe, self.viewbase_pe):
            if self.barf_c2f is None:
                out.append(np.ones(L, dtype=np.float32))
                continue
            start, end = self.barf_c2f
            alpha = (torch.tensor(progress, dtype=torch.float32) - start) / (end - start) * L
            k = torch.arange(L, dtype=torch.float32)
            w = (1 - (alpha - k).clamp_(min=0, max=1).mul_(np.pi).cos_()) / 2
            out.append(w.numpy())
        return np.concatenate(out).astype(np.float32)


def dynamic_weight(w0, w1, it, total):
    return w0 * math.exp(math.log(w1 / w0) / total * it)


class Workspace:
    SAMPLER = ('t_min', 't_max', 'ray_start', 'count', 'pts', 'ray_id', 'step_k', 'step')

    def __init__(self, N, capacity, device, sample_capacity=None, backward=True, keep_activations=True, ctx=None, samples=None):
        f = dict(dtype=torch.float32, device=device)
        i = dict(dtype=torch.int32, device=device)
        self.N, self.cap, self.device = N, capacity, device
        e = torch.empty
        self.rays_o, self.rays_d, self.viewdirs = e(N, 3, **f), e(N, 3, **f), e(N, 3, **f)
# ... 49 lines not shown

    def __init__(self, device, moments=True):
        self.off, o = {}, 0
        for name, n in self.SEG:
            self.off[name] = (o, n)
            o += _pad(n)
        self.n = o
        z = lambda: torch.zeros(o, dtype=torch.float32, device=device)
        self.data, self.grad = z(), z()
        self.m, self.v = (z(), z()) if moments else (None, None)

    def view(self, name, which='data'):
        o, n = self.off[name]
        return getattr(self, which)[o:o + n]

    def load_reference(self, sdf_alpha, sdf_beta, rgbnet, warp):
        with torch.no_grad():
            self.view('sdf_ab').copy_(torch.cat([sdf_alpha.reshape(1), sdf_beta.reshape(1)]))
            self.view('rgbnet').copy_(pack_rgbnet(rgbnet).to(self.data.device))
            self.view('warp').copy_(pack_warp(warp).to(self.data.device))

    def export_grads(self):
        g = {'sdf_alpha': self.view('sdf_ab', 'grad')[0:1].clone(), 'sdf_beta': self.view('sdf_ab', 'grad')[1:2].clone()}
        g['rgbnet'] = unpack_rgbnet(self.view('rgbnet', 'grad'))
        g['warp'] = unpack_warp(self.view('warp', 'grad'))
        return g


_WARP_PREFIX = 'warp_network.deform_net.net.net.{}.0'
MLP_LAYOUT = {
    'rgbnet': ((128, 57, 64, 'rgbnet.0'), (128, 128, 128, 'rgbnet.2.0'), (128, 128, 128, 'rgbnet.3.0'), (3, 128, 128, 'rgbnet.4')),
    'warp': tuple((o, i, i, _WARP_PREFIX.format(l)) for l, (o, i) in enumerate(((128, 3), (128, 128), (128, 128), (128, 128), (4, 128)))),
}


def _pack(net, layers):
    parts = []
    for (o, i, ld, _), (W, b) in zip(MLP_LAYOUT[net], layers):
        if ld != i:
            Wp = torch.zeros(o, ld, dtype=torch.float32, device=W.device)
            Wp[:, :W.shape[1]] = W
            W = Wp
        parts += [W.reshape(-1), b]
    return torch.cat([p.detach().float() for p in parts])


def _unpack(net, flat):
    at, out = 0, []
    for o, i, ld, _ in MLP_LAYOUT[net]:
        W = flat[at:at + o * ld].reshape(o, ld)[:, :i]; at += o * ld
        b = flat[at:at + o]; at += o
        out.append((W, b))
    return out


def pack_rgbnet(layers, in_dim=57):
    assert in_dim == MLP_LAYOUT['rgbnet'][0][1]
    return _pack('rgbnet', layers)


def unpack_rgbnet(flat, in_dim=57):
    assert in_dim == MLP_LAYOUT['rgbnet'][0][1]
    return _unpack('rgbnet', flat)


def pack_warp(layers):
    return _pack('warp', layers)


def unpack_warp(flat):
    return _unpack('warp', flat)


class RenderCore:

    def __init__(self, cfg: SceneConfig, ctx=None, ordered=False):
        self.cfg = cfg
        self.ctx = ctx
        self.ordered = bool(ordered)
        if self.ordered and ctx is None:
            raise ValueError('an ordered RenderCore needs its own context (the workspace is attached to it)')

    @contextlib.contextmanager
    def pass_scope(self, flat, pack, lean_ws=None):
        lean = lean_ws is not None and lean_ws.warp_acts is not None
        try:
            ops.mlp_pack(flat.view('warp'), flat.view('rgbnet'), pack, self.ctx)
            if lean:
                ops.warp_lean_begin(lean_ws.warp_acts, lean_ws.scratch, flat.view('warp'), self.ctx)
            yield
        finally:
            ops.mlp_pack_invalidate(self.ctx)
            if lean:
                ops.warp_lean_end(self.ctx)

    def sample(self, ws, jitter):
        ops.sample_dense(self.cfg.pp, ws.rays_o, ws.rays_d, jitter, ws.sample_cap, ws.t_min, ws.t_max, ws.ray_start, ws.count,
                         ws.pts, ws.ray_id, ws.step_k, ws.step)

    def forward(self, ws, k0_cl, sdf, sdf_ab, rgbnet_p, warp_p, inv_s, pe_w, step_w=None, before_k0_use=None, normals=None,
                side_by_side=False):
        cfg, sc = self.cfg, self.cfg.pp
        nrm, normal_marched = (None, None) if normals is None else normals
        ops.warp_fwd(warp_p, ws.pts, ws.count, ws.cap, cfg.out_range, ws.warp_acts, ws.warp_out, self.ctx)
        if side_by_side and before_k0_use is None and (sc.k0_dim, sc.pos_pe, sc.view_pe) == (12, 5, 1):
            ops.geometry_color_feat_fwd(sc, sdf, sdf_ab, ws.pts, ws.warp_out, ws.viewdirs, ws.ray_id, ws.count, ws.cap, inv_s,
                                        ws.alpha, ws.gradient, ws.sdf_final, ws.sdf_deform, ws.grad_deform, k0_cl, pe_w, ws.feat)
        else:
            ops.geometry_fwd(sc, sdf, sdf_ab, ws.pts, ws.warp_out, ws.viewdirs, ws.ray_id, ws.count, ws.cap, inv_s,
                             ws.alpha, ws.gradient, ws.sdf_final, ws.sdf_deform, ws.grad_deform)
            if before_k0_use is not None:
                before_k0_use()
            ops.color_feat_fwd(sc, k0_cl, ws.pts, ws.viewdirs, ws.ray_id, ws.gradient, pe_w, ws.count, ws.cap, ws.feat)
        ops.rgbnet_fwd(rgbnet_p, ws.feat, ws.count, ws.cap, ws.rgb_acts, ws.rgb, self.ctx)
        if nrm is not None:
            torch.div(ws.gradient, ws.gradient.norm(2, -1, keepdim=True) + 1e-6, out=nrm)
        ops.march_fwd(ws.alpha, ws.rgb, ws.step if step_w is None else step_w, nrm, ws.ray_start, ws.N, cfg.bg,
                      ws.weights, ws.T, ws.alphainv_last, ws.i_end, ws.rgb_marched, ws.rgb_pre, ws.cum_weights,
                      ws.depth_acc, normal_marched)

    def backward(self, ws, k0_cl, sdf, sdf_ab, rgbnet_p, warp_p, inv_s, pe_w, k0_grad_cl, sdf_ab_grad, rgbnet_grad,
                 warp_grad, g_depth=None, g_weights=None, g_gradient_ext=None, g_sdf_deform=None, g_grad_deform=None,
                 g_correction=None, g_alpha_ext=None, g_rgb_ext=None, after_k0_grad=None, priors=None):
        cfg, sc = self.cfg, self.cfg.pp
        ops.march_bwd(ws.alpha, ws.rgb, ws.step, ws.weights, ws.T, ws.alphainv_last, ws.ray_start, ws.i_end, ws.N, cfg.bg,
                      ws.rgb_pre, ws.g_rgbm, ws.g_cw, ws.g_last, g_depth, g_weights, ws.g_alpha, ws.g_rgb)
        if g_alpha_ext is not None:
            ws.g_alpha.add_(g_alpha_ext)
        if g_rgb_ext is not None:
            ws.g_rgb.add_(g_rgb_ext)
        ctx = self.ctx
        ops.rgbnet_bwd(rgbnet_p, ws.feat, ws.rgb_acts, ws.rgb, ws.g_rgb, ws.count, ws.cap, ws.scratch_rgb,
                       rgbnet_grad, ws.g_feat, ctx)
        ops.color_feat_bwd(sc, k0_cl, ws.pts, ws.viewdirs, ws.ray_id, ws.gradient, pe_w, ws.count, ws.cap, ws.g_feat,
                           k0_grad_cl, ws.g_pts, ws.g_gradient, ws.g_view_s)
        if after_k0_grad is not None:
            after_k0_grad()
        if priors is not None:
            w_eik, w_dyn, ls, loss_out, batch_norm = priors
            if self.ordered:
                ops.geometry_bwd_priors_ordered(sc, sdf, sdf_ab, ws.pts, ws.warp_out, ws.viewdirs, ws.ray_id, ws.count, ws.cap,
                                                inv_s, ws.g_alpha, ws.g_gradient, w_eik, w_dyn, ls, 1, ws.g_warp_out, ws.g_pts,
                                                ws.g_view_s, sdf_ab_grad, loss_out, batch_norm, self.ctx)
            else:
                ops.geometry_bwd_priors(sc, sdf, sdf_ab, ws.pts, ws.warp_out, ws.viewdirs, ws.ray_id, ws.count, ws.cap, inv_s,
                                        ws.g_alpha, ws.g_gradient, w_eik, w_dyn, ls, 1, ws.g_warp_out, ws.g_pts, ws.g_view_s,
                                        sdf_ab_grad, loss_out, batch_norm)
        else:
            if self.ordered:
                raise ValueError('an ordered RenderCore differentiates the fused step only (priors=...): the separate '
                                 'geometry backward keeps its float atomics')
            if g_gradient_ext is not None:
                g_gradient_ext(ws)
            ops.geometry_bwd(sc, sdf, sdf_ab, ws.pts, ws.warp_out, ws.viewdirs, ws.ray_id, ws.count, ws.cap, inv_s,
                             ws.g_alpha, ws.g_gradient, None, g_sdf_deform, g_grad_deform, g_correction, 1, ws.g_warp_out,
                             ws.g_pts, ws.g_view_s, sdf_ab_grad)
        ops.warp_bwd(warp_p, ws.pts, ws.warp_acts, ws.g_warp_out, ws.count, ws.cap, cfg.out_range, ws.scratch, warp_grad,
                     ws.g_pts, ctx)


class TrainEngine:

    LR = {'k0': 1e-1, 'rgbnet': 1e-3, 'warp': 1e-3, 'sdf_ab': 1e-2}

    def __init__(self, cfg: SceneConfig, n_views, H, W, n_rand, device='cuda', lr_pose=1e-3, lr_pose_end=1e-4,
                 pose_iters=1, lrate_decay=10, loss_scale=0.1, weight_main=1.0, weight_tv_k0=0.01, weight_mask=0.1,
                 fix_first=True, capacity=None, x_slab=None, dist_ctx=None, deterministic_scatter=False, options=None,
                 deterministic=False, reproj_rows=0):
        self.cfg, self.dev = cfg, torch.device(device)
        self.deterministic = bool(deterministic)
        if self.deterministic:
            from . import _lib
            opts = dict(_lib.default_context().options(), **(options or {}))
            refused = [('mlp_fused = 0: the layer-by-layer kernels', opts['mlp_fused'] != 1),
                       (f"mlp_split = {opts['mlp_split']} (bits 2, 8 and 16 are needed): the fp32-instruction kernels",
                        opts['mlp_split'] & 26 != 26)]
            for what, bad in refused:
                if bad:
                    raise ValueError(f'deterministic=True with {what} have no ordered gradient flush (they keep float atomics)')
            options = opts
            deterministic_scatter = True
        self.ctx = ops.Context(**options) if options else None
        self.deterministic_scatter = bool(deterministic_scatter)
        self._scatter_work = None
        self._ordered_work = None
        self.V, self.H, self.W, self.N = n_views, H, W, n_rand
        cap = capacity or n_rand * cfg.n_samples
        self.ws = Workspace(n_rand, cap, self.dev, ctx=self.ctx)
        self.core = RenderCore(cfg, ctx=self.ctx, ordered=self.deterministic)
        X, Y, Z = cfg.world_size
        f = dict(dtype=torch.float32, device=self.dev)
        self.k0 = [torch.zeros(X, Y, Z, cfg.k0_dim, **f), torch.zeros(X, Y, Z, cfg.k0_dim, **f)]
        self.k0_cur = 0
        self.k0_grad, self.k0_m, self.k0_v = (torch.zeros(X, Y, Z, cfg.k0_dim, **f) for _ in range(3))
        self.sdf = torch.zeros(X, Y, Z, **f)
        self.k0_touched = torch.zeros(2, X * Y * Z, dtype=torch.uint8, device=self.dev)
        self.touch_par = 0
        self._k0_marked = False
        self.flat = FlatParams(self.dev)
        self.mlp_pack = torch.empty(ops.mlp_pack_workspace(), **f)
        self.se3 = torch.zeros(n_views, 6, **f)
        self.se3_grad, self.se3_m, self.se3_v = (torch.zeros(n_views, 6, **f) for _ in range(3))
        self.w2c_init = torch.zeros(n_views, 3, 4, **f)
        self.w2c, self.c2w = torch.zeros(n_views, 3, 4, **f), torch.zeros(n_views, 3, 4, **f)
        self.jac = torch.zeros(n_views, 12, 6, **f)
        self.c2w_grad = torch.zeros(n_views, 3, 4, **f)
        self.tail_arrive = torch.zeros(1, dtype=torch.int32, device=self.dev)
        self._c2w_clean = True
        self._deferred_rays = None
        mask = torch.ones(n_views, dtype=torch.int32)
        if fix_first:
            mask[0] = 0
        self.refine_mask = mask.to(self.dev)
        self.intr = torch.zeros(n_views, 4, **f)
        self.images = self.masks = None
        self.lr = dict(self.LR)
        self.lr_pose = lr_pose
        self.pose_gamma = (lr_pose_end / (1e-10 + lr_pose)) ** (1. / pose_iters)
        self.decay = 0.1 ** (1 / (lrate_decay * 1000))
        self.loss_scale, self.w_main, self.w_tv, self.w_mask = loss_scale, weight_main, weight_tv_k0, weight_mask
        self.n_step = 0
        self.x_slab = x_slab or (0, X)
        self.dist = dist_ctx
        segs = [self.flat.off[n][0] + _pad(self.flat.off[n][1]) for n, _ in FlatParams.SEG]
        self.seg_end = torch.tensor(segs, dtype=torch.int32, device=self.dev)
        self.pose_seg_end = torch.tensor([n_views * 6], dtype=torch.int32, device=self.dev)
        self.npe = cfg.posbase_pe + cfg.viewbase_pe
        self.step_host = torch.zeros(256, self.npe + 4, dtype=torch.float32)
        if self.dev.type == 'cuda':
            self.step_host = self.step_host.pin_memory()
        self._slot = 0
        self.step_dev = torch.zeros(self.npe + 4, **f)
        self.pe_w = self.step_dev[:self.npe]
        self.seg_lr = self.step_dev[self.npe:self.npe + 3]
        self.pose_seg_lr = self.step_dev[self.npe + 3:self.npe + 4]
        self.reproj_rows = int(reproj_rows)
        self.ws_reproj = None
        self.last_reproj_terms = None
        if self.reproj_rows > 0:
            self._alloc_reproj()

    def _alloc_reproj(self):
        R, S, cfg = self.reproj_rows, self.cfg.n_samples, self.cfg
        f = dict(dtype=torch.float32, device=self.dev)
        ws = self.ws_reproj = Workspace(R, R * S, self.dev, ctx=self.ctx)
        for t in (ws.g_rgbm, ws.g_last, ws.g_cw):
            t.zero_()
        z = lambda *shape: torch.zeros(*shape, **f)
        self._rp = dict(g_p=z(R, 3), g_depth=z(R), g_o=z(R, 3), g_d=z(R, 3), go=z(R, 3), gd=z(R, 3), gv=z(R, 3), g_t=z(R),
                        p=z(R, 3), hit=torch.zeros(R, dtype=torch.uint8, device=self.dev), terms=z(3),
                        g_w2c=z(self.V, 3, 4), g_c2w=z(self.V, 3, 4), se3=z(self.V, 6))
        lo, hi = (torch.tensor(np.asarray(a, dtype=np.float32)) for a in (cfg.xyz_min, cfg.xyz_max))
        self._rp_centre = [float(x) for x in (lo + hi)]
        self._rp_half_diag = float(torch.sqrt(torch.sum(hi - lo ** 2)) / 2.)
        if not math.isfinite(self._rp_half_diag):
            raise ValueError('reproj_rows > 0: Voxurf.diagonal_length is not finite for this box (sum(xyz_max - xyz_min ** 2) < 0)')

    def set_views(self, images, masks, Ks, w2c_init):
        t = lambda a: torch.as_tensor(np.asarray(a), dtype=torch.float32).to(self.dev).contiguous()
        self.images, self.masks = t(images), t(masks).reshape(self.V, self.H, self.W).contiguous()
        K = torch.as_tensor(np.asarray(Ks), dtype=torch.float32)
        self.intr.copy_(torch.stack([K[:, 0, 0], K[:, 1, 1], K[:, 0, 2], K[:, 1, 2]], -1))
        self.w2c_init.copy_(t(w2c_init))

    @property
    def k0_cl(self):
        return self.k0[self.k0_cur]

    def load_reference_params(self, k0, sdf, sdf_alpha, sdf_beta, rgbnet, warp, se3=None):
        with torch.no_grad():
            self.k0_cl.copy_(k0[0].permute(1, 2, 3, 0).to(self.dev))
            self.sdf.copy_(sdf[0, 0].to(self.dev))
            d = lambda x: x.detach().to(self.dev)
            self.flat.load_reference(d(sdf_alpha), d(sdf_beta), [(d(W), d(b)) for W, b in rgbnet],
                                     [(d(W), d(b)) for W, b in warp])
            if se3 is not None:
                self.se3.copy_(se3.to(self.dev))

    def k0_reference_layout(self, t=None):
        t = self.k0_cl if t is None else t
        return t.permute(3, 0, 1, 2)[None]

    def scatter_work(self, n_samples):
        need = ops.k0_scatter_sorted_workspace(n_samples)
        if self._scatter_work is None or self._scatter_work.numel() < need:
            self._scatter_work = torch.empty(need, dtype=torch.uint8, device=self.dev)
        return self._scatter_work

    def ordered_work(self):
        mlp_wgs = self.ctx.get('mlp_wgs')
        wgs = max(16, mlp_wgs) if mlp_wgs > 0 else torch.cuda.get_device_properties(self.dev).multi_processor_count
        need = ops.ordered_workspace(wgs, self.ws.cap, self.N)
        if self._ordered_work is None or self._ordered_work.numel() < need:
            self._ordered_work = torch.empty(need, dtype=torch.uint8, device=self.dev)
            ops.ordered_attach(self.ctx, self._ordered_work, wgs, self.ws.cap, self.N)
        return self._ordered_work

    def zero_grads(self):
        self.k0_grad.zero_()
        self.k0_touched.zero_()
        self._k0_marked = False
        self.flat.grad.zero_()
        self.se3_grad.zero_()
        self.c2w_grad.zero_()
        self.tail_arrive.zero_()
        self._c2w_clean = True
        self._deferred_rays = None

    @property
    def side_by_side(self):
        return self.dist is None and not self.deterministic

    def render_and_grads(self, ray_idx, jitter, global_step, defer_pose_bwd=False):
        defer_pose_bwd = defer_pose_bwd and self.side_by_side
        self._deferred_rays = None
        cfg, ws, sc = self.cfg, self.ws, self.cfg.pp
        if self.deterministic:
            self.ordered_work()
        ops.pose_fwd(self.se3, self.w2c_init, self.refine_mask, self.w2c, self.c2w, self.jac)
        ops.raygen_select_fwd(sc, ray_idx, self.c2w, self.intr, self.H, self.W, cfg.inverse_y, True, self.images, self.masks,
                              ws.rays_o, ws.rays_d, ws.viewdirs, ws.target, ws.mask_px)
        self.core.sample(ws, jitter)
        if self.dist is not None:
            self.dist.start_batch_stats(ws.count, ws.mask_px)
        progress = global_step / cfg.N_iters
        self._upload_step_scalars(progress)
        s_val, inv_s = cfg.s_val(global_step), cfg.inv_s(global_step)
        P = self.flat
        with self.core.pass_scope(P, self.mlp_pack, ws):
            self.core.forward(ws, self.k0_cl, self.sdf, P.view('sdf_ab'), P.view('rgbnet'), P.view('warp'), inv_s, self.pe_w,
                              before_k0_use=None if self.dist is None else (lambda: self.dist.wait_parameters(self)),
                              side_by_side=self.side_by_side)
            ws.zero_block.zero_()
            w_dyn = dynamic_weight(1e-1, 1e-3, global_step, cfg.N_iters)
            ls = self.loss_scale
            batch_norm = None if self.dist is None else self.dist.wait_batch_stats()
            ops.loss_rays(ws.rgb_marched, ws.alphainv_last, ws.cum_weights, ws.target, ws.mask_px, ws.mask_sum, self.w_main,
                          0.01, self.w_mask, ls, ws.g_rgbm, ws.g_last, ws.g_cw, ws.loss_out, batch_norm)

            dense_exchange = self.dist is not None and self.dist.local_scatter
            k0_grad = self.k0_grad if dense_exchange else None
            self._k0_marked = not dense_exchange
            touched = self.k0_touched[self.touch_par]

            def after_k0():
                if self.dist is None:
                    if self.deterministic_scatter:
                        ops.k0_scatter_samples_sorted(sc, ws.pts, ws.count, ws.cap, ws.g_feat, self.k0_grad, self.scatter_work(ws.cap), touched)
                    else:
                        ops.k0_scatter_samples(sc, ws.pts, ws.count, ws.cap, ws.g_feat, self.k0_grad, touched)
                else:
                    self.dist.start_grid_reduce(self)
            self.core.backward(ws, self.k0_cl, self.sdf, P.view('sdf_ab'), P.view('rgbnet'), P.view('warp'), inv_s, self.pe_w,
                               k0_grad, P.view('sdf_ab', 'grad'), P.view('rgbnet', 'grad'), P.view('warp', 'grad'),
                               priors=(1.0, w_dyn, ls, ws.loss_out, batch_norm),
                               after_k0_grad=after_k0)
            if defer_pose_bwd:
                self._deferred_rays = ray_idx
            elif self.deterministic:
                ops.raygen_select_bwd_ordered(sc, ray_idx, self.c2w, self.intr, self.H, self.W, cfg.inverse_y, ws.rays_o, ws.rays_d,
                                              ws.t_min, ws.ray_start, ws.g_pts, ws.step, ws.g_view_s, None, None, None, None, None,
                                              None, None, self.c2w_grad, self.ctx)
            else:
                ops.raygen_select_bwd(sc, ray_idx, self.c2w, self.intr, self.H, self.W, cfg.inverse_y, ws.rays_o, ws.rays_d,
                                      ws.t_min, ws.ray_start, ws.g_pts, ws.step, ws.g_view_s, None, None, None, None, None, None,
                                      None, self.c2w_grad)
            if not defer_pose_bwd:
                self._c2w_clean = False
                ops.pose_bwd(self.jac, self.c2w_grad, self.se3_grad)
        return s_val, w_dyn

    def reprojection_grads(self, rows, mode, global_step, jitter=None, weight_projection=1.0, weight_near_surface=1.0, nl=0.0,
                           pixel_thre=None, scale=None):
        if self.ws_reproj is None:
            raise ValueError('reprojection_grads needs an engine built with reproj_rows > 0')
        if self.deterministic:
            raise ValueError('the reprojection pass is out of the scope of deterministic=True: its render backward uses the separate '
                             'geometry backward, which keeps float atomics')
        if self.dist is not None:
            raise NotImplementedError('the reprojection pass is not sharded across ranks')
        if not self.cfg.inverse_y:
            raise NotImplementedError('the reprojection pass implements inverse_y=True without flips (the DTU setting)')
        if mode not in ('crossing', 'render'):
            raise ValueError(f"mode must be 'crossing' or 'render', got {mode!r}")
        cfg, ws, sc, rp, P = self.cfg, self.ws_reproj, self.cfg.pp, self._rp, self.flat
        R = rows['own'].shape[0]
        n = int(rows.get('n_rows', R))
        if not 0 < n <= R <= self.reproj_rows:
            raise ValueError(f'{n} of {R} rows with reproj_rows = {self.reproj_rows}')
        cap = self.reproj_rows
        if jitter is None:
            jitter = torch.rand(cap, device=self.dev)
        elif jitter.shape[0] < cap:
            jitter = torch.cat([jitter, jitter.new_zeros(cap - jitter.shape[0])])
        render = mode == 'render'
        scale = self.loss_scale if scale is None else scale
        ops.reproj_rays(sc, rows['own'], rows['pix'], n, self.intr, self.c2w, ws.rays_o, ws.rays_d, ws.viewdirs)
        self.core.sample(ws, jitter)
        loss_args = (self.intr, self.w2c, self._rp_centre, self._rp_half_diag, nl, pixel_thre, weight_near_surface,
                     weight_projection, scale, rp['terms'], rp['g_p'], rp['g_depth'], rp['g_o'], rp['g_d'], rp['g_w2c'])
        if render:
            par = (self.k0_cl, self.sdf, P.view('sdf_ab'), P.view('rgbnet'), P.view('warp'), cfg.inv_s(global_step), self.pe_w)
            with self.core.pass_scope(P, self.mlp_pack, ws):
                self.core.forward(ws, *par)
                ops.reproj_loss(True, n, rows['other'], rows['match'], rows['conf'], ws.rays_o, ws.rays_d, None, None, ws.t_min,
                                ws.depth_acc, *loss_args)
                self.core.backward(ws, *par, None, P.view('sdf_ab', 'grad'), P.view('rgbnet', 'grad'), P.view('warp', 'grad'),
                                   g_depth=rp['g_depth'])
                ops.raygen_select_bwd(sc, None, None, None, 0, 0, True, ws.rays_o, ws.rays_d, ws.t_min, ws.ray_start, ws.g_pts,
                                      ws.step, ws.g_view_s, rp['g_o'], rp['g_d'], None, rp['g_depth'], rp['go'], rp['gd'], rp['gv'],
                                      None)
            g_o, g_d, g_v, g_t = rp['go'], rp['gd'], rp['gv'], None
        else:
            S = cfg.n_samples
            dist = cfg.step_dist
            dense, sdf_d = ws.alpha, ws.sdf_final
            ops.reproj_dense_pts(sc, ws.rays_o, ws.rays_d, ws.t_min, jitter, ws.pts)
            ops.grid_sample_fwd(sc, self.sdf, 1, ws.pts, 1, dense)
            ops.sdf_first_crossing(dense, None, None, cap, S, dist, ws.t_min, ws.rays_o, ws.rays_d, sdf_d, rp['p'], rp['hit'], None)
            ops.reproj_loss(False, n, rows['other'], rows['match'], rows['conf'], ws.rays_o, ws.rays_d, rp['p'], rp['hit'], None,
                            None, *loss_args)
            ops.sdf_crossing_dense_bwd(sc, self.sdf, ws.rays_o, ws.rays_d, ws.t_min, jitter, cap, S, dist, sdf_d, rp['g_p'], None,
                                       rp['go'], rp['gd'], rp['g_t'])
            rp['go'].add_(rp['g_o'])
            rp['gd'].add_(rp['g_d'])
            g_o, g_d, g_v, g_t = rp['go'], rp['gd'], None, rp['g_t']
        ops.reproj_pose_fold(sc, rows['own'], rows['pix'], n, self.intr, self.c2w, self.w2c, ws.rays_o, ws.rays_d, g_o, g_d, g_v,
                             g_t, rp['g_w2c'], rp['g_c2w'])
        ops.pose_bwd(self.jac, rp['g_c2w'], rp['se3'])
        self.se3_grad += rp['se3']
        t = rp['terms']
        self.last_reproj_terms = dict(err=t[0], near=t[1], n_valid=t[2])
        return self.last_reproj_terms

    def _upload_step_scalars(self, progress):
        h = self.step_host[self._slot]
        self._slot = (self._slot + 1) % self.step_host.shape[0]
        h[:self.npe] = torch.from_numpy(self.cfg.pe_weights(progress))
        d = self.decay
        h[self.npe + 0], h[self.npe + 1], h[self.npe + 2] = self.lr['sdf_ab'] * d, self.lr['rgbnet'] * d, self.lr['warp'] * d
        h[self.npe + 3] = self.lr_pose
        self.step_dev.copy_(h, non_blocking=True)

    def optimizer_step(self, optimize_pose=True, grad_scale=1.0):
        cfg = self.cfg
        self.n_step += 1
        for k in self.lr:
            self.lr[k] *= self.decay
        if self.side_by_side:
            self._k0_step(self.lr['k0'], self.n_step, grad_scale, tail=self._optimizer_tail(optimize_pose))
            if optimize_pose:
                self.lr_pose *= self.pose_gamma
            return
        self._k0_step(self.lr['k0'], self.n_step, grad_scale)
        if self.dist is not None:
            self.dist.wait_small()
        ops.adam_flat(self.flat.data, self.flat.grad, self.flat.m, self.flat.v, self.seg_end, self.seg_lr, grad_scale, 0.9,
                      0.99, 1e-8, self.n_step, 1)
        if optimize_pose:
            ops.adam_flat(self.se3.view(-1), self.se3_grad.view(-1), self.se3_m.view(-1), self.se3_v.view(-1),
                          self.pose_seg_end, self.pose_seg_lr, grad_scale, 0.9, 0.999, 1e-8, self.n_step, 1)
            self.lr_pose *= self.pose_gamma

    def _optimizer_tail(self, optimize_pose):
        ws, cfg, rays = self.ws, self.cfg, None
        if self._deferred_rays is not None:
            if not self._c2w_clean:
                self.c2w_grad.zero_()
                self.tail_arrive.zero_()
                self._c2w_clean = True
            rays = (cfg.pp, self._deferred_rays, self.c2w, self.intr, self.H, self.W, cfg.inverse_y, ws.rays_o, ws.rays_d, ws.t_min,
                    ws.ray_start, ws.g_pts, ws.step, ws.g_view_s, self.jac, self.c2w_grad, self.tail_arrive)
            self._deferred_rays = None
        pose = None
        if optimize_pose or rays is not None:
            pose = (self.se3.view(-1), self.se3_grad.view(-1), self.se3_m.view(-1), self.se3_v.view(-1), self.pose_seg_lr, 0.9, 0.999,
                    1e-8, optimize_pose)
        return dict(flat=(self.flat.data, self.flat.grad, self.flat.m, self.flat.v, self.seg_end, self.seg_lr, 0.9, 0.99, 1e-8),
                    pose=pose, rays=rays)

    def _k0_step(self, lr_k0, n_step, grad_scale, tail=None):
        kw = {} if tail is None else dict(tail=tail)
        cfg = self.cfg
        X, Y, Z = cfg.world_size
        tv_scale = self.loss_scale * self.w_tv / (3.0 * X * Y * Z * cfg.k0_dim)
        src, dst = self.k0[self.k0_cur], self.k0[1 - self.k0_cur]
        xb, xe = self.x_slab
        if self._k0_marked and (xb, xe) == (0, X):
            cur = self.touch_par
            ops.grid_tv_adam_step_sparse(src, dst, self.k0_grad, self.k0_m, self.k0_v, cfg.world_size, cfg.k0_dim, xb, xe,
                                         tv_scale, grad_scale, lr_k0, 0.9, 0.99, 1e-8, n_step, self.ws.tv_out,
                                         self.k0_touched[cur], self.k0_touched[1 - cur], self.ctx, **kw)
            self.touch_par = 1 - cur
            self._k0_marked = False
        else:
            ops.grid_tv_adam_step(src, dst, self.k0_grad, self.k0_m, self.k0_v, cfg.world_size, cfg.k0_dim, xb, xe, tv_scale,
                                  grad_scale, lr_k0, 0.9, 0.99, 1e-8, n_step, self.ws.tv_out, self.ctx, **kw)
        self.k0_cur = 1 - self.k0_cur

    def train_step(self, ray_idx, jitter, global_step, optimize_pose=True):
        out = self.render_and_grads(ray_idx, jitter, global_step, defer_pose_bwd=True)
        self.grad_scale = 1.0
        if self.dist is not None:
            self.dist.reduce_gradients(self)
        self.optimizer_step(optimize_pose, grad_scale=self.grad_scale)
        if self.dist is not None:
            self.dist.gather_parameters(self)
        return out

    def _mlp_state(self, which='data'):
        for net in ('rgbnet', 'warp'):
            for (*_, key), (W, b) in zip(MLP_LAYOUT[net], _unpack(net, self.flat.view(net, which))):
                yield key, W, b

    def model_state_dict(self):
        c = lambda t: t.detach().clone().cpu()
        cfg, P = self.cfg, self.flat
        sd = {'sdf_alpha': c(P.view('sdf_ab')[0:1]), 'sdf_beta': c(P.view('sdf_ab')[1:2]),
              'xyz_min': torch.tensor(np.asarray(cfg.xyz_min, dtype=np.float32)),
              'xyz_max': torch.tensor(np.asarray(cfg.xyz_max, dtype=np.float32)),
              'sdf.grid': c(self.sdf)[None, None], 'k0.grid': c(self.k0_reference_layout()).contiguous()}
        for name in ('sdf', 'k0'):
            sd[name + '.xyz_min'], sd[name + '.xyz_max'] = sd['xyz_min'].clone(), sd['xyz_max'].clone()
        for key, W, b in self._mlp_state():
            sd[key + '.weight'], sd[key + '.bias'] = c(W).contiguous(), c(b)
# ... 175 lines not shown
```

poseprobe_amd/ops.py:

```python
import ctypes

import numpy as np
import torch

from . import _lib
from ._lib import pp_scene


def _ptr(t, dtype=None, name='tensor'):
    if t is None:
        return None
    if not isinstance(t, torch.Tensor):
        raise TypeError(f'{name} must be a torch.Tensor')
    if not t.is_cuda:
        raise RuntimeError(f'{name} must be a CUDA tensor')
    if not t.is_contiguous():
        raise RuntimeError(f'{name} must be contiguous')
    if dtype is not None and t.dtype != dtype:
        raise RuntimeError(f'{name} must be {dtype}, got {t.dtype}')
    return ctypes.c_void_p(t.data_ptr())


def _f(t, name='tensor'):
    return _ptr(t, torch.float32, name)


def _i(t, name='tensor'):
    return _ptr(t, torch.int32, name)


def _u8(t, name='tensor'):
    return _ptr(t, torch.uint8, name)


def _stream():
    return ctypes.c_void_p(torch.cuda.current_stream().cuda_stream)


def make_scene(xyz_min, xyz_max, world_size, voxel_size, stepsize, near, far, bg, out_range=1.0, k0_dim=12,
               pos_pe=5, view_pe=1, sdf_index_exact=None):
    sc = pp_scene()
    for i in range(3):
        sc.xyz_min[i] = float(xyz_min[i])
        sc.xyz_max[i] = float(xyz_max[i])
        sc.size[i] = int(world_size[i])
    sc.voxel_size = float(np.float32(voxel_size))
    sc.stepsize = float(stepsize)
    sc.near_clip = float(near)
    sc.far_clip = float(far)
    sc.bg = float(bg)
    sc.n_samples = int(np.linalg.norm(np.array([int(w) for w in world_size]) + 1) / stepsize) + 1
    sc.out_range = float(out_range)
    sc.k0_dim, sc.pos_pe, sc.view_pe = int(k0_dim), int(pos_pe), int(view_pe)
    if sdf_index_exact is None:
        import os
        sdf_index_exact = os.environ.get('PP_SDF_INDEX_EXACT') == '1'
    sc.sdf_index_exact = int(bool(sdf_index_exact))
    return sc


RGBNET_PARAMS = 128 * 64 + 128 + 2 * (128 * 128 + 128) + 3 * 128 + 3
WARP_PARAMS = 128 * 3 + 128 + 3 * (128 * 128 + 128) + 4 * 128 + 4
FEAT_LD = 64


def pose_fwd(se3, w2c_init, refine_mask, w2c, c2w, jac):
    V = se3.shape[0]
    _lib.call('pp_pose_fwd', _f(se3), _f(w2c_init), _i(refine_mask), V, _f(w2c), _f(c2w), _f(jac), _stream())


def pose_bwd(jac, c2w_grad, se3_grad):
    _lib.call('pp_pose_bwd', _f(jac), _f(c2w_grad), se3_grad.shape[0], _f(se3_grad), _stream())


def raygen_select_fwd(sc, ray_idx, c2w, intr, H, W, inverse_y, normalize, images, masks, rays_o, rays_d, viewdirs,
                      target, mask_px):
    _lib.call('pp_raygen_select_fwd', ctypes.byref(sc), _i(ray_idx), ray_idx.shape[0], _f(c2w), _f(intr),
              c2w.shape[0], H, W, int(inverse_y), int(normalize), _f(images), _f(masks), _f(rays_o), _f(rays_d),
              _f(viewdirs), _f(target), _f(mask_px), _stream())


def raygen_select_bwd(sc, ray_idx, c2w, intr, H, W, inverse_y, rays_o, rays_d, t_min, ray_start, pts_grad, step,
                      vgrad_s, g_o, g_d, g_v, g_depth, g_o_out, g_d_out, g_v_out, c2w_grad):
    n_views = c2w.shape[0] if c2w is not None else 0
    _lib.call('pp_raygen_select_bwd', ctypes.byref(sc), _i(ray_idx), rays_o.shape[0], _f(c2w), _f(intr), n_views,
              H, W, int(inverse_y), _f(rays_o), _f(rays_d), _f(t_min), _i(ray_start), _f(pts_grad), _f(step),
              _f(vgrad_s), _f(g_o), _f(g_d), _f(g_v), _f(g_depth), _f(g_o_out), _f(g_d_out), _f(g_v_out),
              _f(c2w_grad), _stream())


def sample_dense(sc, rays_o, rays_d, jitter, capacity, t_min, t_max, ray_start, count, pts, ray_id, step_k, step,
                 mask_keep=None):
    _lib.call('pp_sample_dense', ctypes.byref(sc), _f(rays_o), _f(rays_d), _f(jitter), rays_o.shape[0], capacity,
              _f(t_min), _f(t_max), _i(ray_start), _i(count), _f(pts), _i(ray_id), _i(step_k), _f(step),
              _ptr(mask_keep, torch.uint8), _stream())


def sample_var(sc, rays_o, rays_d, capacity, t_min, t_max, n_steps, ray_start, count, pts, ray_id, step_id):
    _lib.call('pp_sample_var', ctypes.byref(sc), _f(rays_o), _f(rays_d), rays_o.shape[0], capacity, _f(t_min),
              _f(t_max), _i(n_steps), _i(ray_start), _i(count), _f(pts), _i(ray_id), _i(step_id), _stream())


def alpha2weight_fwd(alpha, ray_start, n_rays, weights, T, alphainv_last, i_end):
    _lib.call('pp_alpha2weight_fwd', _f(alpha), _i(ray_start), n_rays, _f(weights), _f(T), _f(alphainv_last),
              _i(i_end), _stream())


def alpha2weight_bwd(alpha, weights, T, alphainv_last, ray_start, i_end, n_rays, grad_weights, grad_last, grad_alpha):
    _lib.call('pp_alpha2weight_bwd', _f(alpha), _f(weights), _f(T), _f(alphainv_last), _i(ray_start), _i(i_end),
              n_rays, _f(grad_weights), _f(grad_last), _f(grad_alpha), _stream())


def march_fwd(alpha, rgb, step_w, nrm_in, ray_start, n_rays, bg, weights, T, alphainv_last, i_end, rgb_marched,
              rgb_pre, cum_weights, depth_acc, normal_marched):
    _lib.call('pp_march_fwd', _f(alpha), _f(rgb), _f(step_w), _f(nrm_in), _i(ray_start), n_rays, float(bg),
              _f(weights), _f(T), _f(alphainv_last), _i(i_end), _f(rgb_marched), _f(rgb_pre), _f(cum_weights),
              _f(depth_acc), _f(normal_marched), _stream())


def march_bwd(alpha, rgb, step_w, weights, T, alphainv_last, ray_start, i_end, n_rays, bg, rgb_pre, g_rgbm, g_cw,
              g_last, g_depth, g_weights, grad_alpha, grad_rgb):
    _lib.call('pp_march_bwd', _f(alpha), _f(rgb), _f(step_w), _f(weights), _f(T), _f(alphainv_last), _i(ray_start),
              _i(i_end), n_rays, float(bg), _f(rgb_pre), _f(g_rgbm), _f(g_cw), _f(g_last), _f(g_depth),
              _f(g_weights), _f(grad_alpha), _f(grad_rgb), _stream())


def geometry_fwd(sc, sdf_grid, sdf_ab, pts, warp_out, viewdirs, ray_id, count, capacity, inv_s, alpha, gradient,
                 sdf_final, sdf_deform, grad_deform):
    _lib.call('pp_geometry_fwd', ctypes.byref(sc), _f(sdf_grid), _f(sdf_ab), _f(pts), _f(warp_out), _f(viewdirs),
              _i(ray_id), _i(count), capacity, float(inv_s), _f(alpha), _f(gradient), _f(sdf_final), _f(sdf_deform),
              _f(grad_deform), _stream())


def geometry_bwd(sc, sdf_grid, sdf_ab, pts, warp_out, viewdirs, ray_id, count, capacity, inv_s, g_alpha, g_gradient,
                 g_sdf_final, g_sdf_deform, g_grad_deform, g_correction, accumulate, warp_out_grad, pts_grad, vgrad_s,
                 sdf_ab_grad):
    _lib.call('pp_geometry_bwd', ctypes.byref(sc), _f(sdf_grid), _f(sdf_ab), _f(pts), _f(warp_out), _f(viewdirs),
              _i(ray_id), _i(count), capacity, float(inv_s), _f(g_alpha), _f(g_gradient), _f(g_sdf_final),
              _f(g_sdf_deform), _f(g_grad_deform), _f(g_correction), int(accumulate), _f(warp_out_grad),
              _f(pts_grad), _f(vgrad_s), _f(sdf_ab_grad), _stream())


def color_feat_fwd(sc, k0_cl, pts, viewdirs, ray_id, gradient, pe_w, count, capacity, feat):
    _lib.call('pp_color_feat_fwd', ctypes.byref(sc), _f(k0_cl), _f(pts), _f(viewdirs), _i(ray_id), _f(gradient),
              _f(pe_w), _i(count), capacity, _f(feat), _stream())


def color_feat_bwd(sc, k0_cl, pts, viewdirs, ray_id, gradient, pe_w, count, capacity, feat_grad, k0_grad_cl, pts_grad,
                   gradient_grad, vgrad_s):
    _lib.call('pp_color_feat_bwd', ctypes.byref(sc), _f(k0_cl), _f(pts), _f(viewdirs), _i(ray_id), _f(gradient),
              _f(pe_w), _i(count), capacity, _f(feat_grad), _f(k0_grad_cl), _f(pts_grad), _f(gradient_grad),
              _f(vgrad_s), _stream())


def geometry_bwd_priors(sc, sdf_grid, sdf_ab, pts, warp_out, viewdirs, ray_id, count, capacity, inv_s, g_alpha, g_gradient,
                        w_eikonal, w_deform, loss_scale, accumulate, warp_out_grad, pts_grad, vgrad_s, sdf_ab_grad, loss_out,
                        batch_norm=None):
    _lib.call('pp_geometry_bwd_priors', ctypes.byref(sc), _f(sdf_grid), _f(sdf_ab), _f(pts), _f(warp_out), _f(viewdirs),
              _i(ray_id), _i(count), capacity, float(inv_s), _f(g_alpha), _f(g_gradient), float(w_eikonal), float(w_deform),
              float(loss_scale), int(accumulate), _f(warp_out_grad), _f(pts_grad), _f(vgrad_s), _f(sdf_ab_grad),
              _f(loss_out), _f(batch_norm), _stream())


def geometry_color_feat_fwd(sc, sdf_grid, sdf_ab, pts, warp_out, viewdirs, ray_id, count, capacity, inv_s, alpha, gradient,
                           sdf_final, sdf_deform, grad_deform, k0_cl, pe_w, feat):
    _lib.call('pp_geometry_color_feat_fwd', ctypes.byref(sc), _f(sdf_grid), _f(sdf_ab), _f(pts), _f(warp_out), _f(viewdirs),
              _i(ray_id), _i(count), capacity, float(inv_s), _f(alpha), _f(gradient), _f(sdf_final), _f(sdf_deform),
              _f(grad_deform), _f(k0_cl), _f(pe_w), _f(feat), _stream())


def ordered_workspace(work_groups, capacity, n_rays):
    b = ctypes.c_int64()
    _lib.call('pp_ordered_workspace', int(work_groups), int(capacity), int(n_rays), ctypes.byref(b))
    return b.value


def ordered_attach(ctx, work, work_groups, capacity, n_rays):
    if ctx is None:
        raise ValueError('ordered_attach needs a context of its own (the default context is shared by everybody)')
    _lib.call('pp_ordered_attach', ctx.handle, _u8(work), 0 if work is None else int(work.numel()), int(work_groups),
              int(capacity), int(n_rays))


def geometry_bwd_priors_ordered(sc, sdf_grid, sdf_ab, pts, warp_out, viewdirs, ray_id, count, capacity, inv_s, g_alpha, g_gradient,
                                w_eikonal, w_deform, loss_scale, accumulate, warp_out_grad, pts_grad, vgrad_s, sdf_ab_grad, loss_out,
                                batch_norm, ctx):
    _lib.call('pp_geometry_bwd_priors_ordered', ctypes.byref(sc), _f(sdf_grid), _f(sdf_ab), _f(pts), _f(warp_out), _f(viewdirs),
              _i(ray_id), _i(count), capacity, float(inv_s), _f(g_alpha), _f(g_gradient), float(w_eikonal), float(w_deform),
              float(loss_scale), int(accumulate), _f(warp_out_grad), _f(pts_grad), _f(vgrad_s), _f(sdf_ab_grad),
              _f(loss_out), _f(batch_norm), ctx.handle, _stream())


def raygen_select_bwd_ordered(sc, ray_idx, c2w, intr, H, W, inverse_y, rays_o, rays_d, t_min, ray_start, pts_grad, step,
                              vgrad_s, g_o, g_d, g_v, g_depth, g_o_out, g_d_out, g_v_out, c2w_grad, ctx):
    _lib.call('pp_raygen_select_bwd_ordered', ctypes.byref(sc), _i(ray_idx), rays_o.shape[0], _f(c2w), _f(intr), c2w.shape[0],
              H, W, int(inverse_y), _f(rays_o), _f(rays_d), _f(t_min), _i(ray_start), _f(pts_grad), _f(step),
              _f(vgrad_s), _f(g_o), _f(g_d), _f(g_v), _f(g_depth), _f(g_o_out), _f(g_d_out), _f(g_v_out),
              _f(c2w_grad), ctx.handle, _stream())


def k0_pack_samples(pts, feat_grad, count, capacity, k0_dim, packed):
    _lib.call('pp_k0_pack_samples', _f(pts), _f(feat_grad), _i(count), capacity, int(k0_dim), _f(packed), _stream())


def k0_scatter_packed(sc, packed, n_shards, capacity, k0_grad_cl, touched=None):
    _lib.call('pp_k0_scatter_packed', ctypes.byref(sc), _f(packed), int(n_shards), capacity, _f(k0_grad_cl), _u8(touched),
              _stream())


# ... 15 lines not shown

def k0_scatter_packed_sorted(sc, packed, n_shards, capacity, k0_grad_cl, work, touched=None):
    _lib.call('pp_k0_scatter_packed_sorted', ctypes.byref(sc), _f(packed), int(n_shards), capacity, _f(k0_grad_cl), _u8(touched),
              _u8(work), int(work.numel()), _stream())


Context = _lib.Context
_h = _lib.handle


def mlp_pack_workspace():
    n = ctypes.c_int64()
    _lib.call('pp_mlp_pack_workspace', ctypes.byref(n))
    return n.value


def mlp_pack(warp_params, rgbnet_params, pack, ctx=None):
    _lib.call('pp_mlp_pack', _f(warp_params), _f(rgbnet_params), _f(pack), _h(ctx), _stream())


def mlp_pack_invalidate(ctx=None):
    _lib.call('pp_mlp_pack_invalidate', _h(ctx))


def warp_lean_begin(acts, scratch, params, ctx=None):
    _lib.call('pp_warp_lean_begin', _f(acts), _f(scratch), _f(params), _h(ctx))


def warp_lean_end(ctx=None):
    _lib.call('pp_warp_lean_end', _h(ctx))


def rgbnet_fwd(params, feat, count, capacity, acts, rgb, ctx=None):
    _lib.call('pp_rgbnet_fwd', _f(params), _f(feat), _i(count), capacity, _f(acts), _f(rgb), _h(ctx), _stream())


def rgbnet_bwd(params, feat, acts, rgb, rgb_grad, count, capacity, scratch, params_grad, feat_grad, ctx=None):
    _lib.call('pp_rgbnet_bwd', _f(params), _f(feat), _f(acts), _f(rgb), _f(rgb_grad), _i(count), capacity,
              _f(scratch), _f(params_grad), _f(feat_grad), _h(ctx), _stream())


def warp_fwd(params, pts, count, capacity, out_range, acts, out, ctx=None):
    _lib.call('pp_warp_fwd', _f(params), _f(pts), _i(count), capacity, float(out_range), _f(acts), _f(out), _h(ctx), _stream())


def warp_bwd(params, pts, acts, out_grad, count, capacity, out_range, scratch, params_grad, pts_grad, ctx=None):
    _lib.call('pp_warp_bwd', _f(params), _f(pts), _f(acts), _f(out_grad), _i(count), capacity, float(out_range),
              _f(scratch), _f(params_grad), _f(pts_grad), _h(ctx), _stream())


def mlp_workspaces(capacity):
    out = {}
    for name in ('rgbnet', 'warp'):
        a, s = ctypes.c_int64(), ctypes.c_int64()
        _lib.call(f'pp_{name}_workspace', int(capacity), ctypes.byref(a), ctypes.byref(s))
        out[name] = (a.value, s.value)
    return out


def warp_bwd_data(params, pts, acts, out_grad, count, capacity, out_range, scratch, params_grad, pts_grad, ctx=None):
    stage2 = ctypes.c_int32()
    _lib.call('pp_warp_bwd_data', _f(params), _f(pts), _f(acts), _f(out_grad), _i(count), capacity, float(out_range),
              _f(scratch), _f(params_grad), _f(pts_grad), ctypes.byref(stage2), _h(ctx), _stream())
    return stage2.value


def warp_bwd_weights(acts, scratch, count, capacity, params_grad, stage2, ctx=None):
    _lib.call('pp_warp_bwd_weights', _f(acts), _f(scratch), _i(count), capacity, _f(params_grad), int(stage2), _h(ctx), _stream())


def rgbnet_bwd_data(params, acts, rgb, rgb_grad, count, capacity, scratch, params_grad, feat_grad, ctx=None):
    stage2 = ctypes.c_int32()
    _lib.call('pp_rgbnet_bwd_data', _f(params), _f(acts), _f(rgb), _f(rgb_grad), _i(count), capacity, _f(scratch),
              _f(params_grad), _f(feat_grad), ctypes.byref(stage2), _h(ctx), _stream())
    return stage2.value


def rgbnet_bwd_weights(feat, acts, scratch, count, capacity, params_grad, stage2, ctx=None):
    _lib.call('pp_rgbnet_bwd_weights', _f(feat), _f(acts), _f(scratch), _i(count), capacity, _f(params_grad), int(stage2),
              _h(ctx), _stream())


def loss_rays(rgb_marched, alphainv_last, cum_weights, target, mask_px, mask_sum, w_main, w_entropy, w_mask,
              loss_scale, g_rgbm, g_last, g_cw, loss_out, batch_norm=None):
    _lib.call('pp_loss_rays', _f(rgb_marched), _f(alphainv_last), _f(cum_weights), _f(target), _f(mask_px),
              _f(mask_sum), rgb_marched.shape[0], float(w_main), float(w_entropy), float(w_mask), float(loss_scale),
              _f(g_rgbm), _f(g_last), _f(g_cw), _f(loss_out), _f(batch_norm), _stream())


def loss_samples(gradient, grad_deform, warp_out, sdf_deform, count, capacity, w_eik, w_deform, loss_scale, g_gradient,
                 g_grad_deform, g_correction, g_sdf_deform, loss_out, batch_norm=None):
    _lib.call('pp_loss_samples', _f(gradient), _f(grad_deform), _f(warp_out), _f(sdf_deform), _i(count), capacity,
              float(w_eik), float(w_deform), float(loss_scale), _f(g_gradient), _f(g_grad_deform), _f(g_correction),
              _f(g_sdf_deform), _f(loss_out), _f(batch_norm), _stream())


def _tail_args(tail):
    fp, fg, fm, fv, seg_end, seg_lr, b1, b2, eps = tail['flat']
    out = [_f(fp), _f(fg), _f(fm), _f(fv), fp.numel(), _i(seg_end), _f(seg_lr), seg_end.numel(), float(b1), float(b2), float(eps)]
    pose, rays = tail.get('pose'), tail.get('rays')
    if pose is None:
        out += [None, None, None, None, 0, None, 0., 0., 0., 0]
    else:
        se3, g, m, v, lr, b1, b2, eps, update = pose
        out += [_f(se3), _f(g), _f(m), _f(v), se3.numel() // 6, _f(lr), float(b1), float(b2), float(eps), int(bool(update))]
    if rays is None:
        out += [None, None, 0, None, None, 0, 0, 0] + [None] * 10
    else:
        sc, ray_idx, c2w, intr, H, W, inverse_y, rays_o, rays_d, t_min, ray_start, pts_grad, step, vgrad_s, jac, c2w_grad, arrive = rays
        out += [ctypes.byref(sc), _i(ray_idx), rays_o.shape[0], _f(c2w), _f(intr), H, W, int(inverse_y), _f(rays_o), _f(rays_d),
                _f(t_min), _i(ray_start), _f(pts_grad), _f(step), _f(vgrad_s), _f(jac), _f(c2w_grad), _i(arrive)]
    return out


def grid_tv_adam_step(p_in, p_out, grad, exp_avg, exp_avg_sq, size, channels, x_begin, x_end, tv_scale, grad_scale, lr,
                      beta1, beta2, eps, step, tv_out, ctx=None, tail=None):
    if tail is not None:
        _lib.call('pp_grid_tv_adam_step_tail', _f(p_in), _f(p_out), _f(grad), _f(exp_avg), _f(exp_avg_sq),
                  int(size[0]), int(size[1]), int(size[2]), channels, x_begin, x_end, float(tv_scale), float(grad_scale),
                  float(lr), float(beta1), float(beta2), float(eps), int(step), _f(tv_out), None, None, *_tail_args(tail),
                  _h(ctx), _stream())
        return
    _lib.call('pp_grid_tv_adam_step', _f(p_in), _f(p_out), _f(grad), _f(exp_avg), _f(exp_avg_sq),
              int(size[0]), int(size[1]), int(size[2]), channels, x_begin, x_end, float(tv_scale), float(grad_scale),
              float(lr), float(beta1), float(beta2), float(eps), int(step), _f(tv_out), _h(ctx), _stream())


def grid_tv_adam_step_sparse(p_in, p_out, grad, exp_avg, exp_avg_sq, size, channels, x_begin, x_end, tv_scale, grad_scale,
                             lr, beta1, beta2, eps, step, tv_out, touched, touched_clear, ctx=None, tail=None):
    grid = (_f(p_in), _f(p_out), _f(grad), _f(exp_avg), _f(exp_avg_sq),
            int(size[0]), int(size[1]), int(size[2]), channels, x_begin, x_end, float(tv_scale), float(grad_scale),
            float(lr), float(beta1), float(beta2), float(eps), int(step), _f(tv_out), _u8(touched), _u8(touched_clear))
    if tail is None:
        _lib.call('pp_grid_tv_adam_step_sparse', *grid, _h(ctx), _stream())
    else:
        _lib.call('pp_grid_tv_adam_step_tail', *grid, *_tail_args(tail), _h(ctx), _stream())


def grid_tv_value(p, size, channels, out):
    _lib.call('pp_grid_tv_value', _f(p), int(size[0]), int(size[1]), int(size[2]), channels, _f(out), _stream())


def adam_flat(p, grad, exp_avg, exp_avg_sq, seg_end, seg_lr, grad_scale, beta1, beta2, eps, step, zero_grad):
    _lib.call('pp_adam_flat', _f(p), _f(grad), _f(exp_avg), _f(exp_avg_sq), p.numel(), _i(seg_end), _f(seg_lr),
              seg_end.numel(), float(grad_scale), float(beta1), float(beta2), float(eps), int(step), int(zero_grad),
              _stream())


def grid_sample_fwd(sc, grid_cl, channels, pts, border, out):
    _lib.call('pp_grid_sample_fwd', ctypes.byref(sc), _f(grid_cl), channels, _f(pts), pts.shape[0], int(border), _f(out),
              _stream())


def grid_sample_bwd(sc, grid_cl, channels, pts, border, out_grad, grid_grad_cl, pts_grad):
    _lib.call('pp_grid_sample_bwd', ctypes.byref(sc), _f(grid_cl), channels, _f(pts), pts.shape[0], int(border),
              _f(out_grad), _f(grid_grad_cl), _f(pts_grad), _stream())


def grid_tv_grad(p, size, channels, scale, g_scalar, grad):
    _lib.call('pp_grid_tv_grad', _f(p), int(size[0]), int(size[1]), int(size[2]), channels, float(scale), _f(g_scalar),
              _f(grad), _stream())


def sdf_first_crossing(sdf, ray_start, step_k, n_rays, n_samples, dist, t_min, rays_o, rays_d, sdf_dense, pts, mask, zval):
    _lib.call('pp_sdf_first_crossing', _f(sdf), _i(ray_start), _i(step_k), n_rays, n_samples, float(dist), _f(t_min),
              _f(rays_o), _f(rays_d), _f(sdf_dense), _f(pts), _ptr(mask, torch.uint8), _f(zval), _stream())

# ... 321 lines not shown
```

Baseline: 1.056 million rays/s.

## Fuse ray compositing, ray losses and march backward; fuse step head launches

Adds a fused march+loss+backward kernel that composites each ray, computes the ray losses and their gradients, and runs the march backward in one launch with a workspace. This replaces the separate composite, loss_rays and march_bwd kernels and their intermediate global round-trips. It also adds a pp_step_begin entry that combines pose forward, step-scalar upload, zeroing and the MLP pack into one call. The loss and march math is moved into shared device helpers. The fused path requires a sample cap and is refused when batch normalisation across devices is used.

```diff
diff --git a/include/poseprobe_hip.h b/include/poseprobe_hip.h
--- a/include/poseprobe_hip.h
+++ b/include/poseprobe_hip.h
@@ -155,6 +155,10 @@
 int pp_mlp_pack_workspace(int64_t* pack_floats);
 int pp_mlp_pack(const float* warp_params, const float* rgbnet_params, float* pack, void* ctx, void* stream);
 int pp_mlp_pack_invalidate(void* ctx);
+int pp_step_begin(const float* se3, const float* w2c_init, const int32_t* refine_mask, int32_t n_views, float* w2c,
+                  float* c2w, float* jac, const float* step_scalars, int32_t n_scalars, float* step_dev,
+                  float* zero_block, int32_t n_zero, const float* warp_params, const float* rgbnet_params, float* pack,
+                  void* ctx, void* stream);
 
 int pp_warp_lean_begin(const float* acts, const float* scratch, const float* params, void* ctx);
 int pp_warp_lean_end(void* ctx);
@@ -184,6 +188,14 @@
                  const float* target, const float* mask_px, float* mask_sum, int32_t n_rays, float w_main,
                  float w_entropy, float w_mask, float loss_scale, float* g_rgb_marched, float* g_alphainv_last,
                  float* g_cum_weights, float* loss_out, const float* batch_norm, void* stream);
+int pp_march_loss_workspace(int32_t n_rays, int32_t sample_cap, int64_t* bytes);
+int pp_march_loss_bwd(const float* alpha, const float* rgb, const float* step_w, const int32_t* ray_start,
+                      int32_t n_rays, int32_t sample_cap, float bg, float* weights, float* T, float* alphainv_last,
+                      int32_t* i_end, float* rgb_marched, float* rgb_pre, float* cum_weights, float* depth_acc,
+                      const float* target, const float* mask_px, float* mask_sum, float w_main, float w_entropy,
+                      float w_mask, float loss_scale, float* g_rgb_marched, float* g_alphainv_last,
+                      float* g_cum_weights, float* loss_out, const float* g_depth_acc, const float* g_weights,
+                      float* grad_alpha, float* grad_rgb, void* work, int64_t work_bytes, void* stream);
 int pp_loss_samples(const float* gradient, const float* grad_deform, const float* warp_out,
                     const float* sdf_deform, const int32_t* count, int32_t capacity, float w_eikonal,
                     float w_deform, float loss_scale, float* g_gradient, float* g_grad_deform,
diff --git a/poseprobe_amd/csrc/pp_loss.hip b/poseprobe_amd/csrc/pp_loss.hip
--- a/poseprobe_amd/csrc/pp_loss.hip
+++ b/poseprobe_amd/csrc/pp_loss.hip
@@ -1,13 +1,5 @@
 #include "pp_common.h"
-
-__device__ __forceinline__ float block_sum256(float v, float* sm) {
-  v = pp_wave_sum(v);
-  int lane = threadIdx.x & 63, wid = threadIdx.x >> 6;
-  __syncthreads();
-  if (lane == 0) sm[wid] = v;
-  __syncthreads();
-  return sm[0] + sm[1] + sm[2] + sm[3];
-}
+#include "pp_loss_body.h"
 
 __global__ __launch_bounds__(256) void k_loss_rays(const float* __restrict__ rgbm, const float* __restrict__ alast,
                                                    const float* __restrict__ cw, const float* __restrict__ target,
@@ -19,38 +11,23 @@
   __shared__ float sm[4];
   int r = blockIdx.x * blockDim.x + threadIdx.x;
   float l_mse = 0.f, l_ent = 0.f, l_bce = 0.f;
-  float part = 0.f;
-  for (int i = threadIdx.x; i < n_rays; i += 256) part += mask_px[i];
-  const float msum_local = block_sum256(part, sm);
+  const float msum_local = loss_mask_sum(mask_px, n_rays, sm);
   if (blockIdx.x == 0 && threadIdx.x == 0) mask_sum[0] = msum_local;
   const float msum = batch_norm ? batch_norm[0] : msum_local;
   const float invN = 1.f / (float)n_rays;
   if (r < n_rays) {
-    float y = mask_px[r];
-    for (int k = 0; k < 3; ++k) {
-      float d = rgbm[r * 3 + k] * y - target[r * 3 + k] * y;
-      l_mse += d * d;
-      g_rgbm[r * 3 + k] = ls * w_main * 2.f * d * y / (msum * 3.f);
-    }
-    float a = alast[r];
-    float p = fminf(fmaxf(a, 1e-6f), 1.f - 1e-6f);
-    float lp = logf(p), lq = logf(1.f - p);
-    l_ent = -(p * lp + (1.f - p) * lq);
-    g_alast[r] = (a >= 1e-6f && a <= 1.f - 1e-6f) ? ls * w_ent * (-(lp - lq)) * invN : 0.f;
-    float c0 = cw[r];
-    float c = fminf(fmaxf(c0, 1e-3f), 1.f - 1e-3f);
-    l_bce = -(y * logf(c) + (1.f - y) * logf(1.f - c));
-    g_cw[r] = (c0 >= 1e-3f && c0 <= 1.f - 1e-3f) ? ls * w_mask * (-(y / c) + (1.f - y) / (1.f - c)) * invN : 0.f;
+    const float pix[3] = {rgbm[r * 3], rgbm[r * 3 + 1], rgbm[r * 3 + 2]};
+    const float tgt[3] = {target[r * 3], target[r * 3 + 1], target[r * 3 + 2]};
+    const RayLoss L = loss_ray_terms(pix, alast[r], cw[r], tgt, mask_px[r], msum, invN, w_main, w_ent, w_mask, ls);
+    for (int k = 0; k < 3; ++k) g_rgbm[r * 3 + k] = L.g_rgbm[k];
+    g_alast[r] = L.g_last;
+    g_cw[r] = L.g_cw;
+    l_mse = L.l_mse; l_ent = L.l_ent; l_bce = L.l_bce;
   }
   l_mse = block_sum256(l_mse, sm);
   l_ent = block_sum256(l_ent, sm);
   l_bce = block_sum256(l_bce, sm);
-  if (threadIdx.x == 0 && loss_out) {
-    atomicAdd(&loss_out[0], l_mse / (msum * 3.f));
-    atomicAdd(&loss_out[1], l_ent * invN);
-    atomicAdd(&loss_out[6], l_bce * invN);
-    atomicAdd(&loss_out[7], w_main * (l_mse / (msum * 3.f)) + w_ent * (l_ent * invN) + w_mask * (l_bce * invN));
-  }
+  if (threadIdx.x == 0 && loss_out) loss_rays_add(loss_out, l_mse, l_ent, l_bce, msum, invN, w_main, w_ent, w_mask);
 }
 
 __global__ __launch_bounds__(256) void k_loss_samples(const float* __restrict__ gradient, const float* __restrict__ gdef,
diff --git a/poseprobe_amd/csrc/pp_loss_body.h b/poseprobe_amd/csrc/pp_loss_body.h
--- /dev/null
+++ b/poseprobe_amd/csrc/pp_loss_body.h
@@ -0,0 +1,48 @@
+#pragma once
+#include "pp_common.h"
+
+__device__ __forceinline__ float block_sum256(float v, float* sm) {
+  v = pp_wave_sum(v);
+  int lane = threadIdx.x & 63, wid = threadIdx.x >> 6;
+  __syncthreads();
+  if (lane == 0) sm[wid] = v;
+  __syncthreads();
+  return sm[0] + sm[1] + sm[2] + sm[3];
+}
+
+__device__ __forceinline__ float loss_mask_sum(const float* __restrict__ mask_px, int n_rays, float* sm) {
+  float part = 0.f;
+  for (int i = threadIdx.x; i < n_rays; i += 256) part += mask_px[i];
+  return block_sum256(part, sm);
+}
+
+struct RayLoss { float g_rgbm[3], g_last, g_cw, l_mse, l_ent, l_bce; };
+
+__device__ __forceinline__ RayLoss loss_ray_terms(const float (&rgbm)[3], const float a, const float c0, const float (&target)[3],
+                                                  const float y, const float msum, const float invN, const float w_main,
+                                                  const float w_ent, const float w_mask, const float ls) {
+  RayLoss L;
+  L.l_mse = 0.f;
+  for (int k = 0; k < 3; ++k) {
+    float d = rgbm[k] * y - target[k] * y;
+    L.l_mse += d * d;
+    L.g_rgbm[k] = ls * w_main * 2.f * d * y / (msum * 3.f);
+  }
+  float p = fminf(fmaxf(a, 1e-6f), 1.f - 1e-6f);
+  float lp = logf(p), lq = logf(1.f - p);
+  L.l_ent = -(p * lp + (1.f - p) * lq);
+  L.g_last = (a >= 1e-6f && a <= 1.f - 1e-6f) ? ls * w_ent * (-(lp - lq)) * invN : 0.f;
+  float c = fminf(fmaxf(c0, 1e-3f), 1.f - 1e-3f);
+  L.l_bce = -(y * logf(c) + (1.f - y) * logf(1.f - c));
+  L.g_cw = (c0 >= 1e-3f && c0 <= 1.f - 1e-3f) ? ls * w_mask * (-(y / c) + (1.f - y) / (1.f - c)) * invN : 0.f;
+  return L;
+}
+
+__device__ __forceinline__ void loss_rays_add(float* __restrict__ loss_out, const float l_mse, const float l_ent, const float l_bce,
+                                              const float msum, const float invN, const float w_main, const float w_ent,
+                                              const float w_mask) {
+  atomicAdd(&loss_out[0], l_mse / (msum * 3.f));
+  atomicAdd(&loss_out[1], l_ent * invN);
+  atomicAdd(&loss_out[6], l_bce * invN);
+  atomicAdd(&loss_out[7], w_main * (l_mse / (msum * 3.f)) + w_ent * (l_ent * invN) + w_mask * (l_bce * invN));
+}
diff --git a/poseprobe_amd/csrc/pp_march.hip b/poseprobe_amd/csrc/pp_march.hip
--- a/poseprobe_amd/csrc/pp_march.hip
+++ b/poseprobe_amd/csrc/pp_march.hip
@@ -1,10 +1,114 @@
 #include "pp_common.h"
+#include "pp_loss_body.h"
 
 __device__ __forceinline__ float lane_value(float v, int j) {
   return __int_as_float(__builtin_amdgcn_readlane(__float_as_int(v), j));
 }
 __device__ __forceinline__ double lane_value(double v, int j) {
   return __hiloint2double(__builtin_amdgcn_readlane(__double2hiint(v), j), __builtin_amdgcn_readlane(__double2loint(v), j));
+}
+
+struct MarchAcc {
+  float Tc = 1.f;
+  int stop;
+  bool stopped = false;
+  float rgb[3] = {0, 0, 0}, w = 0.f, d = 0.f, n[3] = {0, 0, 0};
+};
+
+template <bool FUSED, bool DVGO>
+__device__ __forceinline__ void march_fwd_chunk(MarchAcc& s, const int c0, const int e, const int lane, const float a,
+                                                const bool has_rgb, const float (&cr)[3], const bool has_sw, const float cs,
+                                                const bool has_n, const float (&cn)[3], float& myT, float& myw) {
+  myT = 1.f; myw = 0.f;
+  if (!s.stopped) {
+    int n = e - c0 < 64 ? e - c0 : 64;
+    const double omd = 1.0 - (double)a;
+    const float omf = fmaxf(1.f - a, 1e-10f);
+    bool reached = false;
+    for (int j = 0; j < n; ++j) {
+      if (lane == j) { myT = s.Tc; reached = true; }
+      if (DVGO) {
+        s.Tc = s.Tc * lane_value(omf, j);
+      } else {
+        s.Tc = (float)((double)s.Tc * lane_value(omd, j));
+        if (s.Tc < 1e-3f) { s.stop = c0 + j + 1; s.stopped = true; break; }
+      }
+    }
+    if (reached) myw = myT * a;
+  }
+  if (FUSED && c0 + lane < e) {
+    s.w += myw;
+    if (has_rgb) for (int k = 0; k < 3; ++k) s.rgb[k] += myw * cr[k];
+    if (has_sw) s.d += myw * cs;
+    if (has_n) for (int k = 0; k < 3; ++k) s.n[k] += myw * cn[k];
+  }
+}
+
+template <bool FUSED>
+__device__ __forceinline__ void march_fwd_finish(MarchAcc& s, const int r, const int lane, const float bg,
+                                                 float* __restrict__ alphainv_last, int32_t* __restrict__ i_end,
+                                                 float* __restrict__ rgb_marched, float* __restrict__ rgb_pre,
+                                                 float* __restrict__ cum_weights, float* __restrict__ depth_acc,
+                                                 float* __restrict__ normal_marched, float (&pre)[3], float (&rgbm)[3]) {
+  if (FUSED) {
+    s.w = pp_wave_sum(s.w);
+    s.d = pp_wave_sum(s.d);
+    for (int k = 0; k < 3; ++k) { s.rgb[k] = pp_wave_sum(s.rgb[k]); s.n[k] = pp_wave_sum(s.n[k]); }
+    for (int k = 0; k < 3; ++k) {
+      pre[k] = s.rgb[k] + (1.f - s.w) * bg;
+      rgbm[k] = fminf(fmaxf(pre[k], 0.f), 1.f);
+    }
+  }
+  if (lane == 0) {
+    alphainv_last[r] = s.Tc;
+    i_end[r] = s.stop;
+    if (FUSED) {
+      cum_weights[r] = s.w;
+      if (depth_acc) depth_acc[r] = s.d;
+      for (int k = 0; k < 3; ++k) {
+        if (rgb_pre) rgb_pre[r * 3 + k] = pre[k];
+        if (rgb_marched) rgb_marched[r * 3 + k] = rgbm[k];
+        if (normal_marched) normal_marched[r * 3 + k] = s.n[k];
+      }
+    }
+  }
+}
+
+__device__ __forceinline__ void march_bwd_ray(const float (&pre)[3], const float (&g)[3], const float g_cw, const float bg,
+                                              float (&gm)[3], float& gcw) {
+  for (int k = 0; k < 3; ++k) gm[k] = (pre[k] >= 0.f && pre[k] <= 1.f) ? g[k] : 0.f;
+  gcw = g_cw - bg * (gm[0] + gm[1] + gm[2]);
+}
+
+struct MarchChunk { float a, w, T, gw, v[3], sw; };
+
+template <bool FUSED>
+__device__ __forceinline__ float march_bwd_chunk(const MarchChunk& ck, const int c0, const int lane, const bool live, const int stop,
+                                                 const bool has_rgb, const bool has_sw, const float (&gm)[3], const float gcw,
+                                                 const float gd, float& back, float* __restrict__ g_rgb) {
+  const int i = c0 + lane;
+  const float a = ck.a, w = ck.w, T = ck.T;
+  float gw = ck.gw;
+  if (FUSED && live) {
+    float wr = 0.f;
+    if (has_rgb) for (int k = 0; k < 3; ++k) { wr += gm[k] * ck.v[k]; if (g_rgb) g_rgb[i * 3 + k] = w * gm[k]; }
+    gw += wr + gcw + (has_sw ? gd * ck.sw : 0.f);
+  }
+  int hi = stop - c0;
+  if (hi > 64) hi = 64;
+  const float gww = gw * w;
+  float myback = 0.f;
+  for (int j = hi - 1; j >= 0; --j) {
+    if (lane == j) myback = back;
+    back += lane_value(gww, j);
+  }
+  float ga = 0.f;
+  if (lane < hi) {
+    const float gwT = gw * T;
+    const double denom = (double)(1.f - a) + 1e-10;
+    ga = (float)((double)gwT - (double)myback / denom);
+  }
+  return ga;
 }
 
 template <bool FUSED, bool DVGO>
@@ -20,10 +124,8 @@
   int lane = threadIdx.x & 63;
   if (r >= n_rays) return;
   const int b = ray_start[r], e = ray_start[r + 1];
-  float Tc = 1.f;
-  int stop = e;
-  bool stopped = false;
-  float acc_rgb[3] = {0, 0, 0}, acc_w = 0.f, acc_d = 0.f, acc_n[3] = {0, 0, 0};
+  MarchAcc s;
+  s.stop = e;
   float a_next = (b + lane < e) ? alpha[b + lane] : 0.f;
   for (int c0 = b; c0 < e; c0 += 64) {
     int i = c0 + lane;
@@ -35,53 +137,16 @@
       if (step_w) cs = step_w[i];
       if (nrm_in) for (int k = 0; k < 3; ++k) cn[k] = nrm_in[i * 3 + k];
     }
-    float myT = 1.f, myw = 0.f;
-    if (!stopped) {
-      int n = e - c0 < 64 ? e - c0 : 64;
-      const double omd = 1.0 - (double)a;
-      const float omf = fmaxf(1.f - a, 1e-10f);
-      bool reached = false;
-      for (int j = 0; j < n; ++j) {
-        if (lane == j) { myT = Tc; reached = true; }
-        if (DVGO) {
-          Tc = Tc * lane_value(omf, j);
-        } else {
-          Tc = (float)((double)Tc * lane_value(omd, j));
-          if (Tc < 1e-3f) { stop = c0 + j + 1; stopped = true; break; }
-        }
-      }
-      if (reached) myw = myT * a;
-    }
+    float myT, myw;
+    march_fwd_chunk<FUSED, DVGO>(s, c0, e, lane, a, rgb != nullptr, cr, step_w != nullptr, cs, nrm_in != nullptr, cn, myT, myw);
     if (i < e) {
       weights[i] = myw;
       if (Tout) Tout[i] = myT;
-      if (FUSED) {
-        acc_w += myw;
-        if (rgb) for (int k = 0; k < 3; ++k) acc_rgb[k] += myw * cr[k];
-        if (step_w) acc_d += myw * cs;
-        if (nrm_in) for (int k = 0; k < 3; ++k) acc_n[k] += myw * cn[k];
-      }
-    }
-  }
-  if (FUSED) {
-    acc_w = pp_wave_sum(acc_w);
-    acc_d = pp_wave_sum(acc_d);
-    for (int k = 0; k < 3; ++k) { acc_rgb[k] = pp_wave_sum(acc_rgb[k]); acc_n[k] = pp_wave_sum(acc_n[k]); }
-  }
-  if (lane == 0) {
-    alphainv_last[r] = Tc;
-    i_end[r] = stop;
-    if (FUSED) {
-      cum_weights[r] = acc_w;
-      if (depth_acc) depth_acc[r] = acc_d;
-      for (int k = 0; k < 3; ++k) {
-        float pre = acc_rgb[k] + (1.f - acc_w) * bg;
-        if (rgb_pre) rgb_pre[r * 3 + k] = pre;
-        if (rgb_marched) rgb_marched[r * 3 + k] = fminf(fmaxf(pre, 0.f), 1.f);
-        if (normal_marched) normal_marched[r * 3 + k] = acc_n[k];
-      }
-    }
-  }
+    }
+  }
+  float pre[3], rgbm[3];
+  march_fwd_finish<FUSED>(s, r, lane, bg, alphainv_last, i_end, rgb_marched, rgb_pre, cum_weights, depth_acc, normal_marched, pre,
+                          rgbm);
 }
 
 template <bool FUSED>
@@ -100,19 +165,18 @@
   const int b = ray_start[r], e = ray_start[r + 1], stop = i_end[r];
   float gm[3] = {0, 0, 0}, gcw = 0.f, gd = 0.f;
   if (FUSED) {
+    float pre[3], g[3];
     for (int k = 0; k < 3; ++k) {
-      float pre = rgb_pre ? rgb_pre[r * 3 + k] : 0.5f;
-      float g = g_rgbm ? g_rgbm[r * 3 + k] : 0.f;
-      gm[k] = (pre >= 0.f && pre <= 1.f) ? g : 0.f;
-    }
-    gcw = (g_cw ? g_cw[r] : 0.f) - bg * (gm[0] + gm[1] + gm[2]);
+      pre[k] = rgb_pre ? rgb_pre[r * 3 + k] : 0.5f;
+      g[k] = g_rgbm ? g_rgbm[r * 3 + k] : 0.f;
+    }
+    march_bwd_ray(pre, g, g_cw ? g_cw[r] : 0.f, bg, gm, gcw);
     gd = g_depth ? g_depth[r] : 0.f;
   }
   float back = (g_last ? g_last[r] : 0.f) * alphainv_last[r];
   int nchunk = (e - b + 63) / 64;
-  struct Chunk { float a, w, T, gw, v[3], sw; };
   auto fetch = [&](int c) {
-    Chunk k;
+    MarchChunk k;
     const int i = b + c * 64 + lane;
     const bool live = i < e;
     k.a = live ? alpha[i] : 0.f;
@@ -126,35 +190,122 @@
     }
     return k;
   };
-  Chunk nx = fetch(nchunk > 0 ? nchunk - 1 : 0);
+  MarchChunk nx = fetch(nchunk > 0 ? nchunk - 1 : 0);
   for (int c = nchunk - 1; c >= 0; --c) {
     int c0 = b + c * 64;
     int i = c0 + lane;
     bool live = i < e;
-    const Chunk ck = nx;
+    const MarchChunk ck = nx;
     if (c > 0) nx = fetch(c - 1);
-    const float a = ck.a, w = ck.w, T = ck.T;
-    float gw = ck.gw;
-    if (FUSED && live) {
-      float wr = 0.f;
-      if (rgb) for (int k = 0; k < 3; ++k) { wr += gm[k] * ck.v[k]; if (g_rgb) g_rgb[i * 3 + k] = w * gm[k]; }
-      gw += wr + gcw + (step_w ? gd * ck.sw : 0.f);
-    }
-    int hi = stop - c0;
-    if (hi > 64) hi = 64;
-    const float gww = gw * w;
-    float myback = 0.f;
-    for (int j = hi - 1; j >= 0; --j) {
-      if (lane == j) myback = back;
-      back += lane_value(gww, j);
-    }
-    float ga = 0.f;
-    if (lane < hi) {
-      const float gwT = gw * T;
-      const double denom = (double)(1.f - a) + 1e-10;
-      ga = (float)((double)gwT - (double)myback / denom);
-    }
+    const float ga = march_bwd_chunk<FUSED>(ck, c0, lane, live, stop, rgb != nullptr, step_w != nullptr, gm, gcw, gd, back, g_rgb);
     if (live) g_alpha[i] = ga;
+  }
+}
+
+#define MLB_CHUNKS 3
+__global__ __launch_bounds__(256) void k_march_loss_bwd(
+    const float* __restrict__ alpha, const float* __restrict__ rgb, const float* __restrict__ step_w,
+    const int32_t* __restrict__ ray_start, int n_rays, float bg, float* __restrict__ weights, float* __restrict__ Tout,
+    float* __restrict__ alphainv_last, int32_t* __restrict__ i_end, float* __restrict__ rgb_marched, float* __restrict__ rgb_pre,
+    float* __restrict__ cum_weights, float* __restrict__ depth_acc, const float* __restrict__ target,
+    const float* __restrict__ mask_px, float* __restrict__ mask_sum, float w_main, float w_ent, float w_mask, float ls,
+    float* __restrict__ g_rgbm, float* __restrict__ g_last, float* __restrict__ g_cw, float* __restrict__ loss_out,
+    const float* __restrict__ g_depth, const float* __restrict__ g_w_in, float* __restrict__ g_alpha, float* __restrict__ g_rgb,
+    float* work) {
+  __shared__ float sm[4];
+  __shared__ float s_loss[4][3];
+  __shared__ int s_last;
+  const int wid = __builtin_amdgcn_readfirstlane(threadIdx.x >> 6);
+  const int r = blockIdx.x * 4 + wid;
+  const int lane = threadIdx.x & 63;
+  const float msum = loss_mask_sum(mask_px, n_rays, sm);
+  if (blockIdx.x == 0 && threadIdx.x == 0) mask_sum[0] = msum;
+  const float invN = 1.f / (float)n_rays;
+  float l_mse = 0.f, l_ent = 0.f, l_bce = 0.f;
+  if (r < n_rays) {
+    const int b = ray_start[r];
+    int e = ray_start[r + 1];
+    if (e - b > 64 * MLB_CHUNKS) e = b + 64 * MLB_CHUNKS;
+    const int nchunk = (e - b + 63) / 64;
+    MarchAcc s;
+    s.stop = e;
+    float ka[MLB_CHUNKS], kw[MLB_CHUNKS], kT[MLB_CHUNKS], kr[MLB_CHUNKS][3], ks[MLB_CHUNKS];
+    const float no3[3] = {0.f, 0.f, 0.f};
+    float a_next = (b + lane < e) ? alpha[b + lane] : 0.f;
+#pragma unroll
+    for (int c = 0; c < MLB_CHUNKS; ++c) {
+      ka[c] = 0.f; kw[c] = 0.f; kT[c] = 1.f; ks[c] = 0.f;
+      for (int k = 0; k < 3; ++k) kr[c][k] = 0.f;
+      if (c < nchunk) {
+        const int c0 = b + c * 64, i = c0 + lane;
+        ka[c] = a_next;
+        a_next = (i + 64 < e) ? alpha[i + 64] : 0.f;
+        if (i < e) {
+          for (int k = 0; k < 3; ++k) kr[c][k] = rgb[i * 3 + k];
+          if (step_w) ks[c] = step_w[i];
+        }
+        march_fwd_chunk<true, false>(s, c0, e, lane, ka[c], true, kr[c], step_w != nullptr, ks[c], false, no3, kT[c], kw[c]);
+        if (i < e) {
+          weights[i] = kw[c];
+          Tout[i] = kT[c];
+        }
+      }
+    }
+    float pre[3], rgbm[3];
+    march_fwd_finish<true>(s, r, lane, bg, alphainv_last, i_end, rgb_marched, rgb_pre, cum_weights, depth_acc, nullptr, pre, rgbm);
+    const float tgt[3] = {target[r * 3], target[r * 3 + 1], target[r * 3 + 2]};
+    const RayLoss L = loss_ray_terms(rgbm, s.Tc, s.w, tgt, mask_px[r], msum, invN, w_main, w_ent, w_mask, ls);
+    l_mse = L.l_mse; l_ent = L.l_ent; l_bce = L.l_bce;
+    if (lane == 0) {
+      for (int k = 0; k < 3; ++k) g_rgbm[r * 3 + k] = L.g_rgbm[k];
+      g_last[r] = L.g_last;
+      g_cw[r] = L.g_cw;
+    }
+    float gm[3], gcw;
+    march_bwd_ray(pre, L.g_rgbm, L.g_cw, bg, gm, gcw);
+    const float gd = g_depth ? g_depth[r] : 0.f;
+    float back = L.g_last * s.Tc;
+    float kg[MLB_CHUNKS];
+#pragma unroll
+    for (int c = 0; c < MLB_CHUNKS; ++c) {
+      const int i = b + c * 64 + lane;
+      kg[c] = (g_w_in && c < nchunk && i < e) ? g_w_in[i] : 0.f;
+    }
+#pragma unroll
+    for (int c = MLB_CHUNKS - 1; c >= 0; --c) {
+      if (c < nchunk) {
+        const int c0 = b + c * 64, i = c0 + lane;
+        const bool live = i < e;
+        MarchChunk ck;
+        ck.a = ka[c]; ck.w = kw[c]; ck.T = kT[c]; ck.gw = kg[c]; ck.sw = ks[c];
+        for (int k = 0; k < 3; ++k) ck.v[k] = kr[c][k];
+        const float ga = march_bwd_chunk<true>(ck, c0, lane, live, s.stop, true, step_w != nullptr, gm, gcw, gd, back, g_rgb);
+        if (live) g_alpha[i] = ga;
+      }
+    }
+  }
+  if (lane == 0) { s_loss[wid][0] = l_mse; s_loss[wid][1] = l_ent; s_loss[wid][2] = l_bce; }
+  __syncthreads();
+  unsigned* ticket = reinterpret_cast<unsigned*>(work);
+  float* rows = work + 4;
+  if (threadIdx.x == 0) {
+    for (int k = 0; k < 3; ++k) {
+      const float v = ((s_loss[0][k] + s_loss[1][k]) + s_loss[2][k]) + s_loss[3][k];
+      const float old = __hip_atomic_exchange(rows + blockIdx.x * 4 + k, v, __ATOMIC_RELAXED, __HIP_MEMORY_SCOPE_AGENT);
+      asm volatile("" ::"v"(old));
+    }
+    asm volatile("s_waitcnt vmcnt(0)" ::: "memory");
+    s_last = __hip_atomic_fetch_add(ticket, 1u, __ATOMIC_RELAXED, __HIP_MEMORY_SCOPE_AGENT) == gridDim.x - 1;
+  }
+  __syncthreads();
+  if (!s_last) return;
+  float t[3] = {0.f, 0.f, 0.f};
+  for (int g = threadIdx.x; g < (int)gridDim.x; g += 256)
+    for (int k = 0; k < 3; ++k) t[k] += __hip_atomic_load(rows + g * 4 + k, __ATOMIC_RELAXED, __HIP_MEMORY_SCOPE_AGENT);
+  for (int k = 0; k < 3; ++k) t[k] = block_sum256(t[k], sm);
+  if (threadIdx.x == 0) {
+    if (loss_out) loss_rays_add(loss_out, t[0], t[1], t[2], msum, invN, w_main, w_ent, w_mask);
+    __hip_atomic_store(ticket, 0u, __ATOMIC_RELAXED, __HIP_MEMORY_SCOPE_AGENT);
   }
 }
 
@@ -206,6 +357,36 @@
   hipLaunchKernelGGL((k_march_bwd<true>), dim3(pp_div_up(n_rays, 4)), dim3(256), 0, pp_stream(stream), alpha, rgb,
                      step_w, weights, T, alphainv_last, ray_start, i_end, n_rays, bg, rgb_pre, g_rgb_marched,
                      g_cum_weights, g_alphainv_last, g_depth_acc, g_weights, grad_alpha, grad_rgb);
+  PP_CHECK_LAUNCH();
+  return PP_OK;
+}
+
+extern "C" int pp_march_loss_workspace(int32_t n_rays, int32_t sample_cap, int64_t* bytes) {
+  PP_REQUIRE(bytes, "null pointer");
+  PP_REQUIRE(n_rays > 0, "n_rays<=0");
+  PP_REQUIRE(sample_cap > 0 && sample_cap <= 64 * MLB_CHUNKS, "sample_cap: the kernel holds at most 192 samples of a ray");
+  *bytes = (int64_t)(4 + 4 * pp_div_up(n_rays, 4)) * sizeof(float);
+  return PP_OK;
+}
+
+extern "C" int pp_march_loss_bwd(const float* alpha, const float* rgb, const float* step_w, const int32_t* ray_start,
+                                 int32_t n_rays, int32_t sample_cap, float bg, float* weights, float* T, float* alphainv_last,
+                                 int32_t* i_end, float* rgb_marched, float* rgb_pre, float* cum_weights, float* depth_acc,
+                                 const float* target, const float* mask_px, float* mask_sum, float w_main, float w_entropy,
+                                 float w_mask, float loss_scale, float* g_rgb_marched, float* g_alphainv_last,
+                                 float* g_cum_weights, float* loss_out, const float* g_depth_acc, const float* g_weights,
+                                 float* grad_alpha, float* grad_rgb, void* work, int64_t work_bytes, void* stream) {
+  PP_REQUIRE(alpha && rgb && ray_start && weights && T && alphainv_last && i_end && rgb_marched && rgb_pre && cum_weights,
+             "null pointer (compositing)");
+  PP_REQUIRE(target && mask_px && mask_sum && g_rgb_marched && g_alphainv_last && g_cum_weights, "null pointer (losses)");
+  PP_REQUIRE(grad_alpha && work, "null pointer (backward / workspace)");
+  int64_t need = 0;
+  if (int st = pp_march_loss_workspace(n_rays, sample_cap, &need)) return st;
+  PP_REQUIRE(work_bytes >= need && (reinterpret_cast<uintptr_t>(work) & 15) == 0, "workspace too small or not 16-byte aligned");
+  hipLaunchKernelGGL(k_march_loss_bwd, dim3(pp_div_up(n_rays, 4)), dim3(256), 0, pp_stream(stream), alpha, rgb, step_w, ray_start,
+                     n_rays, bg, weights, T, alphainv_last, i_end, rgb_marched, rgb_pre, cum_weights, depth_acc, target, mask_px,
+                     mask_sum, w_main, w_entropy, w_mask, loss_scale, g_rgb_marched, g_alphainv_last, g_cum_weights, loss_out,
+                     g_depth_acc, g_weights, grad_alpha, grad_rgb, static_cast<float*>(work));
   PP_CHECK_LAUNCH();
   return PP_OK;
 }
diff --git a/poseprobe_amd/csrc/pp_mlp.hip b/poseprobe_amd/csrc/pp_mlp.hip
--- a/poseprobe_amd/csrc/pp_mlp.hip
+++ b/poseprobe_amd/csrc/pp_mlp.hip
@@ -100,6 +100,37 @@
   return PP_OK;
 }
 
+extern "C" int pp_step_begin(const float* se3, const float* w2c_init, const int32_t* refine_mask, int32_t n_views, float* w2c,
+                             float* c2w, float* jac, const float* step_scalars, int32_t n_scalars, float* step_dev,
+                             float* zero_block, int32_t n_zero, const float* warp_params, const float* rgbnet_params, float* pack,
+                             void* ctx, void* stream) {
+  PP_REQUIRE(se3 && w2c_init && w2c && c2w && jac && n_views > 0, "null pointer or n_views<=0");
+  PP_REQUIRE(n_scalars >= 0 && n_scalars <= PP_STEP_SCALARS_MAX && (n_scalars == 0 || (step_scalars && step_dev)),
+             "0 <= n_scalars <= 32, with step_scalars (host) and step_dev");
+  PP_REQUIRE(n_zero >= 0 && (n_zero == 0 || zero_block), "n_zero<0 or null zero_block");
+  PP_REQUIRE(pack == nullptr || (ctx && (warp_params || rgbnet_params)), "a pack needs a context and parameters");
+  PP_REQUIRE((reinterpret_cast<uintptr_t>(pack) & 15) == 0, "pack must be 16-byte aligned");
+  PPStepScalars sv;
+  sv.n = n_scalars;
+  for (int i = 0; i < PP_STEP_SCALARS_MAX; ++i) sv.v[i] = i < n_scalars ? step_scalars[i] : 0.f;
+  bool packs = false;
+  if (ctx) {
+    pp_mlp_pack_invalidate(ctx);
+    const MlpRoute rt(ctx);
+    packs = pack && rt.pack && rt.fused && (rt.split & 15) != 0;
+  }
+  pp_launch_step_begin(se3, w2c_init, refine_mask, n_views, w2c, c2w, jac, sv, step_dev, zero_block, n_zero, warp_params,
+                       rgbnet_params, packs ? pack : nullptr, pp_stream(stream));
+  PP_CHECK_LAUNCH();
+  if (packs) {
+    PPContext* c = static_cast<PPContext*>(ctx);
+    c->pack = pack;
+    c->pack_params[0] = warp_params;
+    c->pack_params[1] = rgbnet_params;
+  }
+  return PP_OK;
+}
+
 extern "C" int pp_mlp_fwd(const float* params, const float* feat, int32_t in_ld, int32_t n_gemm, const int32_t* count,
                           int32_t capacity, const float* logit_add, int32_t logit_add_ld, float* acts, float* out,
                           void* ctx, void* stream) {
diff --git a/poseprobe_amd/csrc/pp_mlp_fused.h b/poseprobe_amd/csrc/pp_mlp_fused.h
--- a/poseprobe_amd/csrc/pp_mlp_fused.h
+++ b/poseprobe_amd/csrc/pp_mlp_fused.h
@@ -40,6 +40,11 @@
                                const int32_t* count, int capacity, float out_range, float* ybar, float* params_grad,
                                float* pts_grad, hipStream_t st, int wgs, const float* pack, float* part, bool lean);
 int pp_launch_mlp_pack(const float* warp_params, const float* rgbnet_params, float* pack, hipStream_t st);
+#define PP_STEP_SCALARS_MAX 32
+struct PPStepScalars { float v[PP_STEP_SCALARS_MAX]; int n; };
+int pp_launch_step_begin(const float* se3, const float* w2c_init, const int32_t* refine_mask, int n_views, float* w2c, float* c2w,
+                         float* jac, const PPStepScalars& sv, float* step_dev, float* zero_block, int n_zero,
+                         const float* warp_params, const float* rgbnet_params, float* pack, hipStream_t st);
 int pp_launch_wgrad_chain(const float* YA, const float* XA, float* WA, const float* YB, const float* XB, float* WB,
                           const float* YC, const float* XC, float* WC, int kxc, const int32_t* count, int rmul, int rcap,
                           hipStream_t st, int wgs, float* bA, float* bB, float* bC);
diff --git a/poseprobe_amd/csrc/pp_mlp_split.hip b/poseprobe_amd/csrc/pp_mlp_split.hip
--- a/poseprobe_amd/csrc/pp_mlp_split.hip
+++ b/poseprobe_amd/csrc/pp_mlp_split.hip
@@ -3,6 +3,7 @@
 #include "pp_gemm_split.h"
 #include "pp_split_image.h"
 #include "pp_mlp_pack.h"
+#include "pp_pose_body.h"
 #include "pp_ordered.h"
 
 typedef float f32x4 __attribute__((ext_vector_type(4)));
@@ -1264,9 +1265,8 @@
   return 0;
 }
 
-__global__ __launch_bounds__(256) void k_mlp_pack(const float* __restrict__ warp, const float* __restrict__ rgb, float* __restrict__ pack) {
-  __shared__ __attribute__((aligned(16))) float red4[32];
-  const int task = blockIdx.x;
+__device__ __forceinline__ void mlp_pack_task(const int task, const float* __restrict__ warp, const float* __restrict__ rgb,
+                                              float* __restrict__ pack, float* red4) {
   const float* __restrict__ params = task < PK_TASKS_WARP ? warp : rgb;
   if (params == nullptr) return;
   const int tid = threadIdx.x, lane = tid & 63, wid = tid >> 6;
@@ -1327,6 +1327,35 @@
   }
 }
 
+__global__ __launch_bounds__(256) void k_mlp_pack(const float* __restrict__ warp, const float* __restrict__ rgb, float* __restrict__ pack) {
+  __shared__ __attribute__((aligned(16))) float red4[32];
+  mlp_pack_task(blockIdx.x, warp, rgb, pack, red4);
+}
+
+__global__ __launch_bounds__(256) void k_step_begin(const float* __restrict__ se3, const float* __restrict__ w2c_init,
+                                                    const int32_t* __restrict__ refine_mask, int n_views, float* __restrict__ w2c,
+                                                    float* __restrict__ c2w, float* __restrict__ jac, const PPStepScalars sv,
+                                                    float* __restrict__ step_dev, float* __restrict__ zero_block, int n_zero,
+                                                    const float* __restrict__ warp, const float* __restrict__ rgb,
+                                                    float* __restrict__ pack) {
+  __shared__ __attribute__((aligned(16))) float red4[32];
+  if (blockIdx.x == 0) {
+    for (int t = threadIdx.x; t < n_views * 6; t += 256) pose_fwd_elem(t, se3, w2c_init, refine_mask, n_views, w2c, c2w, jac);
+    if ((int)threadIdx.x < sv.n) step_dev[threadIdx.x] = sv.v[threadIdx.x];
+    for (int i = threadIdx.x; i < n_zero; i += 256) zero_block[i] = 0.f;
+    return;
+  }
+  mlp_pack_task(blockIdx.x - 1, warp, rgb, pack, red4);
+}
+
+int pp_launch_step_begin(const float* se3, const float* w2c_init, const int32_t* refine_mask, int n_views, float* w2c, float* c2w,
+                         float* jac, const PPStepScalars& sv, float* step_dev, float* zero_block, int n_zero,
+                         const float* warp_params, const float* rgbnet_params, float* pack, hipStream_t st) {
+  hipLaunchKernelGGL(k_step_begin, dim3(pack ? 1 + PK_TASKS : 1), dim3(256), 0, st, se3, w2c_init, refine_mask, n_views, w2c, c2w,
+                     jac, sv, step_dev, zero_block, n_zero, warp_params, rgbnet_params, pack);
+  return 0;
+}
+
 int pp_launch_mlp_pack(const float* warp_params, const float* rgbnet_params, float* pack, hipStream_t st) {
   hipLaunchKernelGGL(k_mlp_pack, dim3(PK_TASKS), dim3(256), 0, st, warp_params, rgbnet_params, pack);
   return 0;
diff --git a/poseprobe_amd/csrc/pp_pose_body.h b/poseprobe_amd/csrc/pp_pose_body.h
--- /dev/null
+++ b/poseprobe_amd/csrc/pp_pose_body.h
@@ -0,0 +1,73 @@
+#pragma once
+#include "pp_common.h"
+
+struct D6 {
+  float v;
+  float d;
+};
+__device__ __forceinline__ D6 d6c(float c) { D6 r; r.v = c; r.d = 0.f; return r; }
+__device__ __forceinline__ D6 operator+(const D6& a, const D6& b) { D6 r; r.v = a.v + b.v; r.d = a.d + b.d; return r; }
+__device__ __forceinline__ D6 operator-(const D6& a, const D6& b) { D6 r; r.v = a.v - b.v; r.d = a.d - b.d; return r; }
+__device__ __forceinline__ D6 operator-(const D6& a) { D6 r; r.v = -a.v; r.d = -a.d; return r; }
+__device__ __forceinline__ D6 operator*(const D6& a, const D6& b) { D6 r; r.v = a.v * b.v; r.d = a.d * b.v + a.v * b.d; return r; }
+__device__ __forceinline__ D6 operator*(const D6& a, float s) { D6 r; r.v = a.v * s; r.d = a.d * s; return r; }
+
+static __device__ D6 taylor_t(const D6& t, int kind) {
+  D6 ans = d6c(0.f);
+  D6 pw = d6c(1.f);
+  double denom = 1.0;
+  for (int i = 0; i <= 10; ++i) {
+    if (kind == 0) { if (i > 0) denom *= (double)((2 * i) * (2 * i + 1)); }
+    else if (kind == 1) denom *= (double)((2 * i + 1) * (2 * i + 2));
+    else denom *= (double)((2 * i + 2) * (2 * i + 3));
+    float c = (float)(((i & 1) ? -1.0 : 1.0) / denom);
+    ans = ans + pw * c;
+    pw = pw * t;
+  }
+  return ans;
+}
+
+__device__ __forceinline__ void pose_fwd_elem(int tidx, const float* __restrict__ se3, const float* __restrict__ w2c_init,
+                                              const int32_t* __restrict__ refine_mask, int n_views, float* __restrict__ w2c,
+                                              float* __restrict__ c2w, float* __restrict__ jac) {
+  int v = tidx / 6, kd = tidx - (tidx / 6) * 6;
+  if (v >= n_views) return;
+  const float* P0 = w2c_init + v * 12;
+  D6 Rn[3][3], tn[3];
+  bool refine = (refine_mask == nullptr) || refine_mask[v] != 0;
+  if (!refine) {
+    for (int i = 0; i < 3; ++i) { for (int j = 0; j < 3; ++j) Rn[i][j] = d6c(P0[i * 4 + j]); tn[i] = d6c(P0[i * 4 + 3]); }
+  } else {
+    D6 w[3], u[3];
+    for (int k = 0; k < 3; ++k) {
+      w[k] = d6c(se3[v * 6 + k]); w[k].d = (kd == k) ? 1.f : 0.f;
+      u[k] = d6c(se3[v * 6 + 3 + k]); u[k].d = (kd == 3 + k) ? 1.f : 0.f;
+    }
+    D6 t = w[0] * w[0] + w[1] * w[1] + w[2] * w[2];
+    D6 A = taylor_t(t, 0), B = taylor_t(t, 1), C = taylor_t(t, 2);
+    D6 z = d6c(0.f);
+    D6 wx[3][3] = {{z, -w[2], w[1]}, {w[2], z, -w[0]}, {-w[1], w[0], z}};
+    D6 wx2[3][3];
+    for (int i = 0; i < 3; ++i) for (int j = 0; j < 3; ++j) wx2[i][j] = wx[i][0] * wx[0][j] + wx[i][1] * wx[1][j] + wx[i][2] * wx[2][j];
+    D6 R[3][3], Vm[3][3], tr[3];
+    for (int i = 0; i < 3; ++i) for (int j = 0; j < 3; ++j) {
+      D6 eye = d6c(i == j ? 1.f : 0.f);
+      R[i][j] = eye + A * wx[i][j] + B * wx2[i][j];
+      Vm[i][j] = eye + B * wx[i][j] + C * wx2[i][j];
+    }
+    for (int i = 0; i < 3; ++i) tr[i] = Vm[i][0] * u[0] + Vm[i][1] * u[1] + Vm[i][2] * u[2];
+    for (int i = 0; i < 3; ++i) {
+      for (int j = 0; j < 3; ++j) Rn[i][j] = R[0][j] * P0[i * 4 + 0] + R[1][j] * P0[i * 4 + 1] + R[2][j] * P0[i * 4 + 2];
+      tn[i] = tr[0] * P0[i * 4 + 0] + tr[1] * P0[i * 4 + 1] + tr[2] * P0[i * 4 + 2] + d6c(P0[i * 4 + 3]);
+    }
+  }
+  for (int i = 0; i < 3; ++i) {
+    for (int j = 0; j < 3; ++j) {
+      if (kd == 0) { w2c[v * 12 + i * 4 + j] = Rn[i][j].v; c2w[v * 12 + i * 4 + j] = Rn[j][i].v; }
+      jac[(v * 12 + i * 4 + j) * 6 + kd] = Rn[j][i].d;
+    }
+    D6 ti = -(Rn[0][i] * tn[0] + Rn[1][i] * tn[1] + Rn[2][i] * tn[2]);
+    if (kd == 0) { w2c[v * 12 + i * 4 + 3] = tn[i].v; c2w[v * 12 + i * 4 + 3] = ti.v; }
+    jac[(v * 12 + i * 4 + 3) * 6 + kd] = ti.d;
+  }
+}
diff --git a/poseprobe_amd/csrc/pp_rays.hip b/poseprobe_amd/csrc/pp_rays.hip
--- a/poseprobe_amd/csrc/pp_rays.hip
+++ b/poseprobe_amd/csrc/pp_rays.hip
@@ -1,77 +1,12 @@
 #include "pp_common.h"
 #include "pp_ordered.h"
 #include "pp_ray_bwd.h"
-
-struct D6 {
-  float v;
-  float d;
-};
-__device__ __forceinline__ D6 d6c(float c) { D6 r; r.v = c; r.d = 0.f; return r; }
-__device__ __forceinline__ D6 operator+(const D6& a, const D6& b) { D6 r; r.v = a.v + b.v; r.d = a.d + b.d; return r; }
-__device__ __forceinline__ D6 operator-(const D6& a, const D6& b) { D6 r; r.v = a.v - b.v; r.d = a.d - b.d; return r; }
-__device__ __forceinline__ D6 operator-(const D6& a) { D6 r; r.v = -a.v; r.d = -a.d; return r; }
-__device__ __forceinline__ D6 operator*(const D6& a, const D6& b) { D6 r; r.v = a.v * b.v; r.d = a.d * b.v + a.v * b.d; return r; }
-__device__ __forceinline__ D6 operator*(const D6& a, float s) { D6 r; r.v = a.v * s; r.d = a.d * s; return r; }
-
-__device__ D6 taylor_t(const D6& t, int kind) {
-  D6 ans = d6c(0.f);
-  D6 pw = d6c(1.f);
-  double denom = 1.0;
-  for (int i = 0; i <= 10; ++i) {
-    if (kind == 0) { if (i > 0) denom *= (double)((2 * i) * (2 * i + 1)); }
-    else if (kind == 1) denom *= (double)((2 * i + 1) * (2 * i + 2));
-    else denom *= (double)((2 * i + 2) * (2 * i + 3));
-    float c = (float)(((i & 1) ? -1.0 : 1.0) / denom);
-    ans = ans + pw * c;
-    pw = pw * t;
-  }
-  return ans;
-}
+#include "pp_pose_body.h"
 
 __global__ void k_pose_fwd(const float* __restrict__ se3, const float* __restrict__ w2c_init,
                            const int32_t* __restrict__ refine_mask, int n_views, float* __restrict__ w2c,
                            float* __restrict__ c2w, float* __restrict__ jac) {
-  int tidx = blockIdx.x * blockDim.x + threadIdx.x;
-  int v = tidx / 6, kd = tidx - (tidx / 6) * 6;
-  if (v >= n_views) return;
-  const float* P0 = w2c_init + v * 12;
-  D6 Rn[3][3], tn[3];
-  bool refine = (refine_mask == nullptr) || refine_mask[v] != 0;
-  if (!refine) {
-    for (int i = 0; i < 3; ++i) { for (int j = 0; j < 3; ++j) Rn[i][j] = d6c(P0[i * 4 + j]); tn[i] = d6c(P0[i * 4 + 3]); }
-  } else {
-    D6 w[3], u[3];
-    for (int k = 0; k < 3; ++k) {
-      w[k] = d6c(se3[v * 6 + k]); w[k].d = (kd == k) ? 1.f : 0.f;
-      u[k] = d6c(se3[v * 6 + 3 + k]); u[k].d = (kd == 3 + k) ? 1.f : 0.f;
-    }
-    D6 t = w[0] * w[0] + w[1] * w[1] + w[2] * w[2];
-    D6 A = taylor_t(t, 0), B = taylor_t(t, 1), C = taylor_t(t, 2);
-    D6 z = d6c(0.f);
-    D6 wx[3][3] = {{z, -w[2], w[1]}, {w[2], z, -w[0]}, {-w[1], w[0], z}};
-    D6 wx2[3][3];
-    for (int i = 0; i < 3; ++i) for (int j = 0; j < 3; ++j) wx2[i][j] = wx[i][0] * wx[0][j] + wx[i][1] * wx[1][j] + wx[i][2] * wx[2][j];
-    D6 R[3][3], Vm[3][3], tr[3];
-    for (int i = 0; i < 3; ++i) for (int j = 0; j < 3; ++j) {
-      D6 eye = d6c(i == j ? 1.f : 0.f);
-      R[i][j] = eye + A * wx[i][j] + B * wx2[i][j];
-      Vm[i][j] = eye + B * wx[i][j] + C * wx2[i][j];
-    }
-    for (int i = 0; i < 3; ++i) tr[i] = Vm[i][0] * u[0] + Vm[i][1] * u[1] + Vm[i][2] * u[2];
-    for (int i = 0; i < 3; ++i) {
-      for (int j = 0; j < 3; ++j) Rn[i][j] = R[0][j] * P0[i * 4 + 0] + R[1][j] * P0[i * 4 + 1] + R[2][j] * P0[i * 4 + 2];
-      tn[i] = tr[0] * P0[i * 4 + 0] + tr[1] * P0[i * 4 + 1] + tr[2] * P0[i * 4 + 2] + d6c(P0[i * 4 + 3]);
-    }
-  }
-  for (int i = 0; i < 3; ++i) {
-    for (int j = 0; j < 3; ++j) {
-      if (kd == 0) { w2c[v * 12 + i * 4 + j] = Rn[i][j].v; c2w[v * 12 + i * 4 + j] = Rn[j][i].v; }
-      jac[(v * 12 + i * 4 + j) * 6 + kd] = Rn[j][i].d;
-    }
-    D6 ti = -(Rn[0][i] * tn[0] + Rn[1][i] * tn[1] + Rn[2][i] * tn[2]);
-    if (kd == 0) { w2c[v * 12 + i * 4 + 3] = tn[i].v; c2w[v * 12 + i * 4 + 3] = ti.v; }
-    jac[(v * 12 + i * 4 + 3) * 6 + kd] = ti.d;
-  }
+  pose_fwd_elem(blockIdx.x * blockDim.x + threadIdx.x, se3, w2c_init, refine_mask, n_views, w2c, c2w, jac);
 }
 
 __global__ void k_pose_bwd(const float* __restrict__ jac, const float* __restrict__ c2w_grad, int n_views,
diff --git a/poseprobe_amd/engine.py b/poseprobe_amd/engine.py
--- a/poseprobe_amd/engine.py
+++ b/poseprobe_amd/engine.py
@@ -1,5 +1,6 @@
 import contextlib
 import math
+import warnings
 from dataclasses import dataclass
 
 import numpy as np
@@ -215,10 +216,13 @@
             raise ValueError('an ordered RenderCore needs its own context (the workspace is attached to it)')
 
     @contextlib.contextmanager
-    def pass_scope(self, flat, pack, lean_ws=None):
+    def pass_scope(self, flat, pack, lean_ws=None, pack_with=None):
         lean = lean_ws is not None and lean_ws.warp_acts is not None
         try:
-            ops.mlp_pack(flat.view('warp'), flat.view('rgbnet'), pack, self.ctx)
+            if pack_with is not None:
+                pack_with()
+            else:
+                ops.mlp_pack(flat.view('warp'), flat.view('rgbnet'), pack, self.ctx)
             if lean:
                 ops.warp_lean_begin(lean_ws.warp_acts, lean_ws.scratch, flat.view('warp'), self.ctx)
             yield
@@ -232,7 +236,7 @@
                          ws.pts, ws.ray_id, ws.step_k, ws.step)
 
     def forward(self, ws, k0_cl, sdf, sdf_ab, rgbnet_p, warp_p, inv_s, pe_w, step_w=None, before_k0_use=None, normals=None,
-                side_by_side=False):
+                side_by_side=False, composite=True):
         cfg, sc = self.cfg, self.cfg.pp
         nrm, normal_marched = (None, None) if normals is None else normals
         ops.warp_fwd(warp_p, ws.pts, ws.count, ws.cap, cfg.out_range, ws.warp_acts, ws.warp_out, self.ctx)
@@ -248,16 +252,24 @@
         ops.rgbnet_fwd(rgbnet_p, ws.feat, ws.count, ws.cap, ws.rgb_acts, ws.rgb, self.ctx)
         if nrm is not None:
             torch.div(ws.gradient, ws.gradient.norm(2, -1, keepdim=True) + 1e-6, out=nrm)
+        if not composite:
+            if normals is not None or step_w is not None:
+                raise ValueError('composite=False: the fused ray launch composites neither normals nor a step_w of the caller')
+            return
         ops.march_fwd(ws.alpha, ws.rgb, ws.step if step_w is None else step_w, nrm, ws.ray_start, ws.N, cfg.bg,
                       ws.weights, ws.T, ws.alphainv_last, ws.i_end, ws.rgb_marched, ws.rgb_pre, ws.cum_weights,
                       ws.depth_acc, normal_marched)
 
     def backward(self, ws, k0_cl, sdf, sdf_ab, rgbnet_p, warp_p, inv_s, pe_w, k0_grad_cl, sdf_ab_grad, rgbnet_grad,
                  warp_grad, g_depth=None, g_weights=None, g_gradient_ext=None, g_sdf_deform=None, g_grad_deform=None,
-                 g_correction=None, g_alpha_ext=None, g_rgb_ext=None, after_k0_grad=None, priors=None):
+                 g_correction=None, g_alpha_ext=None, g_rgb_ext=None, after_k0_grad=None, priors=None, march_done=False):
         cfg, sc = self.cfg, self.cfg.pp
-        ops.march_bwd(ws.alpha, ws.rgb, ws.step, ws.weights, ws.T, ws.alphainv_last, ws.ray_start, ws.i_end, ws.N, cfg.bg,
-                      ws.rgb_pre, ws.g_rgbm, ws.g_cw, ws.g_last, g_depth, g_weights, ws.g_alpha, ws.g_rgb)
+        if march_done:
+            if not (g_depth is None and g_weights is None and g_alpha_ext is None and g_rgb_ext is None):
+                raise ValueError('march_done: the fused ray launch takes no upstream gradients beside the ray losses')
+        else:
+            ops.march_bwd(ws.alpha, ws.rgb, ws.step, ws.weights, ws.T, ws.alphainv_last, ws.ray_start, ws.i_end, ws.N, cfg.bg,
+                          ws.rgb_pre, ws.g_rgbm, ws.g_cw, ws.g_last, g_depth, g_weights, ws.g_alpha, ws.g_rgb)
         if g_alpha_ext is not None:
             ws.g_alpha.add_(g_alpha_ext)
         if g_rgb_ext is not None:
@@ -299,7 +311,7 @@
     def __init__(self, cfg: SceneConfig, n_views, H, W, n_rand, device='cuda', lr_pose=1e-3, lr_pose_end=1e-4,
                  pose_iters=1, lrate_decay=10, loss_scale=0.1, weight_main=1.0, weight_tv_k0=0.01, weight_mask=0.1,
                  fix_first=True, capacity=None, x_slab=None, dist_ctx=None, deterministic_scatter=False, options=None,
-                 deterministic=False, reproj_rows=0):
+                 deterministic=False, reproj_rows=0, fuse_head=True, fuse_rays=True):
         self.cfg, self.dev = cfg, torch.device(device)
         self.deterministic = bool(deterministic)
         if self.deterministic:
@@ -339,6 +351,13 @@
         self.jac = torch.zeros(n_views, 12, 6, **f)
         self.c2w_grad = torch.zeros(n_views, 3, 4, **f)
         self.tail_arrive = torch.zeros(1, dtype=torch.int32, device=self.dev)
+        self.fuse_head, self.fuse_rays = bool(fuse_head), bool(fuse_rays)
+        self.ray_work = None
+        if cfg.n_samples <= ops.MARCH_LOSS_MAX_SAMPLES:
+            self.ray_work = torch.zeros(ops.march_loss_workspace(n_rand, cfg.n_samples), dtype=torch.uint8, device=self.dev)
+        elif self.fuse_rays:
+            warnings.warn(f'{cfg.n_samples} samples per ray: more than the fused ray launch holds ({ops.MARCH_LOSS_MAX_SAMPLES}); '
+                          'the step composites, takes the ray losses and differentiates in separate launches')
         self._c2w_clean = True
         self._deferred_rays = None
         mask = torch.ones(n_views, dtype=torch.int32)
@@ -364,6 +383,9 @@
             self.step_host = self.step_host.pin_memory()
         self._slot = 0
         self.step_dev = torch.zeros(self.npe + 4, **f)
+        if self.npe + 4 > ops.STEP_SCALARS_MAX and self.fuse_head:
+            warnings.warn(f'{self.npe} position-encoding bands: the step keeps its separate head launches')
+            self.fuse_head = False
         self.pe_w = self.step_dev[:self.npe]
         self.seg_lr = self.step_dev[self.npe:self.npe + 3]
         self.pose_seg_lr = self.step_dev[self.npe + 3:self.npe + 4]
@@ -450,26 +472,41 @@
         cfg, ws, sc = self.cfg, self.ws, self.cfg.pp
         if self.deterministic:
             self.ordered_work()
-        ops.pose_fwd(self.se3, self.w2c_init, self.refine_mask, self.w2c, self.c2w, self.jac)
-        ops.raygen_select_fwd(sc, ray_idx, self.c2w, self.intr, self.H, self.W, cfg.inverse_y, True, self.images, self.masks,
-                              ws.rays_o, ws.rays_d, ws.viewdirs, ws.target, ws.mask_px)
-        self.core.sample(ws, jitter)
-        if self.dist is not None:
-            self.dist.start_batch_stats(ws.count, ws.mask_px)
         progress = global_step / cfg.N_iters
-        self._upload_step_scalars(progress)
+        P = self.flat
+        head = None
+        if self.side_by_side and self.fuse_head:
+            head = lambda: ops.step_begin(self.se3, self.w2c_init, self.refine_mask, self.w2c, self.c2w, self.jac,
+                                          self._step_scalars(progress), self.step_dev, ws.zero_block, P.view('warp'),
+                                          P.view('rgbnet'), self.mlp_pack, self.ctx)
+        fused_rays = self.side_by_side and self.fuse_rays and self.ray_work is not None
         s_val, inv_s = cfg.s_val(global_step), cfg.inv_s(global_step)
-        P = self.flat
-        with self.core.pass_scope(P, self.mlp_pack, ws):
+        w_dyn = dynamic_weight(1e-1, 1e-3, global_step, cfg.N_iters)
+        ls = self.loss_scale
+
+        def rays_and_samples():
+            ops.raygen_select_fwd(sc, ray_idx, self.c2w, self.intr, self.H, self.W, cfg.inverse_y, True, self.images, self.masks,
+                                  ws.rays_o, ws.rays_d, ws.viewdirs, ws.target, ws.mask_px)
+            self.core.sample(ws, jitter)
+            if self.dist is not None:
+                self.dist.start_batch_stats(ws.count, ws.mask_px)
+        if head is None:
+            ops.pose_fwd(self.se3, self.w2c_init, self.refine_mask, self.w2c, self.c2w, self.jac)
+            rays_and_samples()
+            self._upload_step_scalars(progress)
+        with self.core.pass_scope(P, self.mlp_pack, ws, pack_with=head):
+            if head is not None:
+                rays_and_samples()
             self.core.forward(ws, self.k0_cl, self.sdf, P.view('sdf_ab'), P.view('rgbnet'), P.view('warp'), inv_s, self.pe_w,
                               before_k0_use=None if self.dist is None else (lambda: self.dist.wait_parameters(self)),
-                              side_by_side=self.side_by_side)
-            ws.zero_block.zero_()
-            w_dyn = dynamic_weight(1e-1, 1e-3, global_step, cfg.N_iters)
-            ls = self.loss_scale
+                              side_by_side=self.side_by_side, composite=not fused_rays)
+            if head is None:
+                ws.zero_block.zero_()
             batch_norm = None if self.dist is None else self.dist.wait_batch_stats()
+            march = (ws.alpha, ws.rgb, ws.step, ws.ray_start, cfg.n_samples, cfg.bg, ws.weights, ws.T, ws.i_end, ws.rgb_pre,
+                     ws.depth_acc, ws.g_alpha, ws.g_rgb, self.ray_work) if fused_rays else None
             ops.loss_rays(ws.rgb_marched, ws.alphainv_last, ws.cum_weights, ws.target, ws.mask_px, ws.mask_sum, self.w_main,
-                          0.01, self.w_mask, ls, ws.g_rgbm, ws.g_last, ws.g_cw, ws.loss_out, batch_norm)
+                          0.01, self.w_mask, ls, ws.g_rgbm, ws.g_last, ws.g_cw, ws.loss_out, batch_norm, march=march)
 
             dense_exchange = self.dist is not None and self.dist.local_scatter
             k0_grad = self.k0_grad if dense_exchange else None
@@ -487,7 +524,7 @@
             self.core.backward(ws, self.k0_cl, self.sdf, P.view('sdf_ab'), P.view('rgbnet'), P.view('warp'), inv_s, self.pe_w,
                                k0_grad, P.view('sdf_ab', 'grad'), P.view('rgbnet', 'grad'), P.view('warp', 'grad'),
                                priors=(1.0, w_dyn, ls, ws.loss_out, batch_norm),
-                               after_k0_grad=after_k0)
+                               after_k0_grad=after_k0, march_done=fused_rays)
             if defer_pose_bwd:
                 self._deferred_rays = ray_idx
             elif self.deterministic:
@@ -569,11 +606,13 @@
     def _upload_step_scalars(self, progress):
         h = self.step_host[self._slot]
         self._slot = (self._slot + 1) % self.step_host.shape[0]
-        h[:self.npe] = torch.from_numpy(self.cfg.pe_weights(progress))
+        h.copy_(torch.from_numpy(self._step_scalars(progress)))
+        self.step_dev.copy_(h, non_blocking=True)
+
+    def _step_scalars(self, progress):
         d = self.decay
-        h[self.npe + 0], h[self.npe + 1], h[self.npe + 2] = self.lr['sdf_ab'] * d, self.lr['rgbnet'] * d, self.lr['warp'] * d
-        h[self.npe + 3] = self.lr_pose
-        self.step_dev.copy_(h, non_blocking=True)
+        lrs = np.array([self.lr['sdf_ab'] * d, self.lr['rgbnet'] * d, self.lr['warp'] * d, self.lr_pose], dtype=np.float32)
+        return np.concatenate([self.cfg.pe_weights(progress), lrs])
 
     def optimizer_step(self, optimize_pose=True, grad_scale=1.0):
         cfg = self.cfg
diff --git a/poseprobe_amd/ops.py b/poseprobe_amd/ops.py
--- a/poseprobe_amd/ops.py
+++ b/poseprobe_amd/ops.py
@@ -69,6 +69,16 @@
     _lib.call('pp_pose_fwd', _f(se3), _f(w2c_init), _i(refine_mask), V, _f(w2c), _f(c2w), _f(jac), _stream())
 
 
+def step_begin(se3, w2c_init, refine_mask, w2c, c2w, jac, scalars, step_dev, zero_block, warp_params=None, rgbnet_params=None,
+               pack=None, ctx=None):
+    vals = np.ascontiguousarray(scalars, dtype=np.float32)
+    n = vals.shape[0]
+    host = (ctypes.c_float * max(n, 1)).from_buffer_copy(vals.tobytes() if n else bytes(4))
+    _lib.call('pp_step_begin', _f(se3), _f(w2c_init), _i(refine_mask), se3.shape[0], _f(w2c), _f(c2w), _f(jac),
+              ctypes.cast(host, ctypes.c_void_p), n, _f(step_dev), _f(zero_block), 0 if zero_block is None else zero_block.numel(),
+              _f(warp_params), _f(rgbnet_params), _f(pack), _h(ctx), _stream())
+
+
 def pose_bwd(jac, c2w_grad, se3_grad):
     _lib.call('pp_pose_bwd', _f(jac), _f(c2w_grad), se3_grad.shape[0], _f(se3_grad), _stream())
 
@@ -125,6 +135,25 @@
               _f(g_weights), _f(grad_alpha), _f(grad_rgb), _stream())
 
 
+MARCH_LOSS_MAX_SAMPLES = 192
+STEP_SCALARS_MAX = 32
+
+
+def march_loss_workspace(n_rays, sample_cap):
+    b = ctypes.c_int64()
+    _lib.call('pp_march_loss_workspace', int(n_rays), int(sample_cap), ctypes.byref(b))
+    return b.value
+
+
+def march_loss_bwd(alpha, rgb, step_w, ray_start, n_rays, sample_cap, bg, weights, T, alphainv_last, i_end, rgb_marched, rgb_pre,
+                   cum_weights, depth_acc, target, mask_px, mask_sum, w_main, w_entropy, w_mask, loss_scale, g_rgbm, g_last, g_cw,
+                   loss_out, g_depth, g_weights, grad_alpha, grad_rgb, work):
+    _lib.call('pp_march_loss_bwd', _f(alpha), _f(rgb), _f(step_w), _i(ray_start), n_rays, int(sample_cap), float(bg), _f(weights),
+              _f(T), _f(alphainv_last), _i(i_end), _f(rgb_marched), _f(rgb_pre), _f(cum_weights), _f(depth_acc), _f(target),
+              _f(mask_px), _f(mask_sum), float(w_main), float(w_entropy), float(w_mask), float(loss_scale), _f(g_rgbm), _f(g_last),
+              _f(g_cw), _f(loss_out), _f(g_depth), _f(g_weights), _f(grad_alpha), _f(grad_rgb), _u8(work), work.numel(), _stream())
+
+
 def geometry_fwd(sc, sdf_grid, sdf_ab, pts, warp_out, viewdirs, ray_id, count, capacity, inv_s, alpha, gradient,
                  sdf_final, sdf_deform, grad_deform):
     _lib.call('pp_geometry_fwd', ctypes.byref(sc), _f(sdf_grid), _f(sdf_ab), _f(pts), _f(warp_out), _f(viewdirs),
@@ -306,7 +335,15 @@
 
 
 def loss_rays(rgb_marched, alphainv_last, cum_weights, target, mask_px, mask_sum, w_main, w_entropy, w_mask,
-              loss_scale, g_rgbm, g_last, g_cw, loss_out, batch_norm=None):
+              loss_scale, g_rgbm, g_last, g_cw, loss_out, batch_norm=None, march=None):
+    if march is not None:
+        if batch_norm is not None:
+            raise ValueError('loss_rays(march=...) has no batch_norm: composite and differentiate with the separate calls')
+        alpha, rgb, step_w, ray_start, sample_cap, bg, weights, T, i_end, rgb_pre, depth_acc, grad_alpha, grad_rgb, work = march
+        march_loss_bwd(alpha, rgb, step_w, ray_start, rgb_marched.shape[0], sample_cap, bg, weights, T, alphainv_last, i_end,
+                       rgb_marched, rgb_pre, cum_weights, depth_acc, target, mask_px, mask_sum, w_main, w_entropy, w_mask,
+                       loss_scale, g_rgbm, g_last, g_cw, loss_out, None, None, grad_alpha, grad_rgb, work)
+        return
     _lib.call('pp_loss_rays', _f(rgb_marched), _f(alphainv_last), _f(cum_weights), _f(target), _f(mask_px),
               _f(mask_sum), rgb_marched.shape[0], float(w_main), float(w_entropy), float(w_mask), float(loss_scale),
               _f(g_rgbm), _f(g_last), _f(g_cw), _f(loss_out), _f(batch_norm), _stream())
```

Result: faster. 1.072 million rays/s (median of 6 runs) (+1.6%).
